# shoeffner/ann3depth

Hardware: AMD Instinct MI355X
Metric: images/sec (640x480->55x74 MSDN train step) (higher is better)
Workload: dtype f32

## Files before the change

ann3depth_amd/_lib.py:

```python
import ctypes
import os
from ctypes import c_char_p, c_float, c_int, c_int32, c_int64, c_size_t, c_uint8, c_uint32, c_void_p, POINTER

LIB_PATH = os.environ.get('A3D_LIB') or os.path.join(os.path.dirname(os.path.abspath(__file__)), 'liba3d.so')


class A3dError(RuntimeError):
    pass


class ConvDesc(ctypes.Structure):
    _fields_ = [(n, c_int32) for n in ('n', 'h', 'w', 'c', 'k', 'r', 's', 'stride', 'pad_t', 'pad_l', 'ho', 'wo',
                                       'ldx', 'ldy', 'precision', 'storage', 'hints')]


class SecondOutput(ctypes.Structure):
    _fields_ = [('ptr', c_void_p), ('ld', c_int32), ('step', c_int32), ('offset', c_int32), ('bf16', c_int32), ('cols', c_int32)]


class ExampleView(ctypes.Structure):
    _fields_ = [('image_height', c_int64), ('image_width', c_int64), ('image_channels', c_int64),
                ('depth_height', c_int64), ('depth_width', c_int64), ('depth_channels', c_int64),
                ('image', c_void_p), ('image_bytes', c_size_t), ('depth', c_void_p), ('depth_bytes', c_size_t)]


class TimingRecord(ctypes.Structure):
    _fields_ = [(n, c_int32) for n in ('mode', 'bm', 'bn', 'waves_m', 'nwaves', 'bk', 'avec', 'bvec', 'prec', 'lds_dma', 'splitk', 'm', 'n', 'k')] + \
               [('ms', c_float), ('flops', ctypes.c_double)]


_P = c_void_p
_D = POINTER(ConvDesc)

SIGNATURES = {
    'a3d_version': (c_char_p, []),
    'a3d_last_error': (c_int, [c_char_p, c_size_t]),
    'a3d_conv2d_fwd_ws_bytes': (c_size_t, [_D]),
    'a3d_conv2d_fwd': (c_int, [_D, _P, _P, _P, _P, c_int, _P, c_size_t, _P]),
    'a3d_conv2d_bwd_data_ws_bytes': (c_size_t, [_D]),
    'a3d_conv2d_bwd_data': (c_int, [_D, _P, _P, _P, _P, _P, c_size_t, _P]),
    'a3d_conv2d_bwd_filter_ws_bytes': (c_size_t, [_D]),
    'a3d_conv2d_bwd_filter': (c_int, [_D, _P, _P, _P, _P, _P, c_size_t, _P]),
    'a3d_conv2d_fwd_prepared_filter_bytes': (c_size_t, [_D]),
    'a3d_conv2d_fwd_prepare_filter': (c_int, [_D, _P, _P, c_size_t, _P]),
    'a3d_conv2d_bwd_filter_pooled_ws_bytes': (c_size_t, [_D]),
    'a3d_conv2d_bwd_filter_pooled': (c_int, [_D, _P, _P, c_int, _P, _P, c_int, c_int, _P, _P, _P, c_size_t, _P]),
    'a3d_conv2d_bwd_both_supported': (c_int, [_D]),
    'a3d_conv2d_bwd_both_ws_bytes': (c_size_t, [_D]),
    'a3d_conv2d_bwd_both': (c_int, [_D, _P, _P, _P, _P, _P, _P, c_int, c_int, c_int, _P, _P, c_size_t, _P]),
    'a3d_dense_fwd_ws_bytes': (c_size_t, [c_int, c_int, c_int]),
    'a3d_dense_fwd': (c_int, [c_int, c_int, c_int, _P, _P, _P, _P, c_int, _P, _P, c_size_t, _P]),
    'a3d_dense_bwd_data_ws_bytes': (c_size_t, [c_int, c_int, c_int]),
    'a3d_dense_bwd_data': (c_int, [c_int, c_int, c_int, _P, _P, _P, _P, c_int, c_float, _P, c_size_t, _P]),
    'a3d_dense_bwd_filter_ws_bytes': (c_size_t, [c_int, c_int, c_int]),
    'a3d_dense_bwd_filter': (c_int, [c_int, c_int, c_int, _P, _P, _P, _P, _P, c_size_t, _P]),
    'a3d_maxpool2x2_fwd': (c_int, [c_int, c_int, c_int, c_int, _P, _P, c_int, _P, _P]),
    'a3d_maxpool2x2_bwd': (c_int, [c_int, c_int, c_int, c_int, _P, _P, c_int, _P, c_int, _P]),
    'a3d_resize_bilinear_tf1': (c_int, [c_int, c_int, c_int, c_int, _P, c_int, c_int, _P, _P]),
    'a3d_resize_bilinear_tf1_pair': (c_int, [c_int, c_int, c_int, c_int, _P, c_int, c_int, _P, c_int, _P, c_int, c_int, _P, _P]),
    'a3d_resize_bilinear_tf1_ex': (c_int, [c_int, c_int, c_int, c_int, _P, c_int, c_int, c_int, _P, c_int, _P, c_int, c_int, c_int,
                                           _P, _P]),
    'a3d_warp_bilinear_pair': (c_int, [c_int, c_int, c_int, c_int, _P, c_int, c_int, c_int, _P, c_int, _P, c_int, c_int, c_int,
                                       _P, _P, _P]),
    'a3d_extract_patches': (c_int, [c_int, c_int, c_int, c_int, _P, c_int, c_int, _P, _P]),
    'a3d_silog_loss_fwd': (c_int, [c_int, c_int, _P, _P, _P, _P, _P]),
    'a3d_silog_loss_bwd': (c_int, [c_int, c_int, _P, _P, _P, _P, _P]),
    'a3d_dropout_keep_mask': (c_int, [c_size_t, ctypes.c_uint64, ctypes.c_uint64, c_float, _P, _P]),
    'a3d_adam_apply_tf1': (c_int, [c_size_t, _P, _P, _P, _P, c_float, c_float, c_float, c_float, c_float, c_float,
                                   c_float, _P]),
    'a3d_adam_apply_tf1_flag': (c_int, [c_size_t, _P, _P, _P, _P, c_float, c_float, c_float, c_float, c_float, c_float,
                                        c_float, _P, _P]),
    'a3d_dense_fwd_ex': (c_int, [c_int, c_int, c_int, _P, _P, _P, _P, c_int, _P, c_int, c_int, _P, c_size_t, _P]),
    'a3d_dense_bwd_data_ex': (c_int, [c_int, c_int, c_int, _P, _P, _P, _P, c_int, c_float, c_int, c_int, _P, c_size_t, _P]),
    'a3d_dense_fwd_ex2': (c_int, [c_int, c_int, c_int, _P, _P, _P, _P, c_int, c_int, c_int, _P, c_int, c_int, POINTER(SecondOutput), _P,
                                  c_size_t, _P]),
    'a3d_dense_bwd_data_ex2': (c_int, [c_int, c_int, c_int, _P, _P, _P, _P, c_int, c_float, c_int, c_int, POINTER(SecondOutput), _P,
                                       c_size_t, _P]),
    'a3d_conv2d_fwd_ex2': (c_int, [_D, _P, _P, _P, _P, c_int, POINTER(SecondOutput), _P, c_size_t, _P]),
    'a3d_silog_loss_bwd_ex': (c_int, [c_int, c_int, _P, _P, _P, _P, _P, c_int, _P]),
    'a3d_depth_metrics_ws_bytes': (c_size_t, [c_int, c_int, c_int]),
    'a3d_depth_metrics': (c_int, [c_int, c_int, c_int, _P, c_int, c_int, _P, c_int, c_float, c_float, c_float, c_float, _P, _P,
                                  c_size_t, _P]),
    'a3d_cast_bf16': (c_int, [c_size_t, _P, _P, c_int, _P]),
    'a3d_cast_rows': (c_int, [c_size_t, c_int, _P, c_int, c_int, _P, c_int, c_int, _P]),
    'a3d_pad_channels_bf16': (c_int, [c_size_t, c_int, _P, c_int, _P, _P]),
    'a3d_stream_create': (c_int, [c_int, ctypes.POINTER(ctypes.c_void_p)]),
    'a3d_stream_destroy': (c_int, [_P]),
    'a3d_maxpool2x2_fwd_bf16': (c_int, [c_int, c_int, c_int, c_int, _P, c_int, _P, c_int, _P, _P]),
    'a3d_maxpool2x2_bwd_bf16': (c_int, [c_int, c_int, c_int, c_int, _P, c_int, _P, c_int, _P, c_int, _P]),
    'a3d_copy_channel_bf16': (c_int, [c_size_t, _P, c_int, c_int, _P, c_int, c_int, _P]),
    'a3d_maxpool2x2_bwd_idx_bf16': (c_int, [c_int, c_int, c_int, c_int, _P, _P, c_int, _P, c_int, _P, c_int, _P]),
    'a3d_maxpool2x2_bwd_idx_bf16s': (c_int, [c_int, c_int, c_int, c_int, _P, _P, c_int, _P, c_int, _P, c_int, _P]),
    'a3d_dense_bwd_filter_adam_tf1': (c_int, [c_int, c_int, c_int, _P, _P, _P, _P, _P, _P, _P, _P, c_float, c_float, c_float,
                                              c_float, c_float, c_float, _P]),
    'a3d_dense_bwd_filter_adam_tf1_ex': (c_int, [c_int, c_int, c_int, _P, _P, _P, _P, _P, _P, _P, _P, c_float, c_float, c_float,
                                                 c_float, c_float, c_float, c_int, _P]),
    'a3d_superpixel_mean': (c_int, [c_int, c_int, c_int, c_int, _P, c_int, _P, _P]),
    'a3d_superpixel_hist': (c_int, [c_int, c_int, c_int, _P, c_int, _P, _P]),
    'a3d_pair_similarity': (c_int, [c_int, c_int, c_int, _P, c_int, _P, _P, _P, c_int, _P, _P, c_float, _P, _P, _P]),
    'a3d_crf_loss': (c_int, [c_int, c_int, _P, _P, _P, _P, _P, c_int, c_float, _P, _P, _P, _P]),
    'a3d_crf_map': (c_int, [c_int, c_int, _P, _P, _P, _P, c_int, _P, _P, _P]),
    'a3d_sgd_apply': (c_int, [c_size_t, _P, _P, c_float, _P]),
    'a3d_conv2d_pool_fwd': (c_int, [_D, _P, _P, _P, _P, c_int, _P, c_int, _P, c_size_t, _P]),
    'a3d_maxpool2x2_bwd_idx': (c_int, [c_int, c_int, c_int, c_int, _P, _P, c_int, _P, c_int, _P, c_int, _P]),
    'a3d_copy_channel': (c_int, [c_size_t, _P, c_int, c_int, _P, c_int, c_int, _P]),
    'a3d_comm_standin': (c_int, [_P, c_size_t, _P, c_size_t, c_int, c_float, _P]),
    'a3d_timing_enable': (c_int, [c_int]),
    'a3d_timing_collect': (c_int, [POINTER(TimingRecord), c_int]),
    'a3d_timing_select': (c_int, [POINTER(TimingRecord)]),
    'a3d_crc32c': (c_uint32, [_P, c_size_t]),
    'a3d_masked_crc32c': (c_uint32, [_P, c_size_t]),
    'a3d_tfrecord_next': (c_int, [_P, c_size_t, c_int, POINTER(c_size_t), POINTER(c_size_t), POINTER(c_size_t)]),
    'a3d_example_parse': (c_int, [_P, c_size_t, POINTER(ExampleView)]),
    'a3d_decode_raw_plus_half': (c_int, [_P, c_size_t, _P]),
    'a3d_record_decode': (c_int, [_P, c_size_t, c_int, _P, c_size_t, _P, c_size_t, POINTER(ExampleView)]),
    'a3d_record_decode_u8': (c_int, [_P, c_size_t, c_int, _P, _P, c_size_t, _P, _P, c_size_t, POINTER(ExampleView),
                                     POINTER(c_int)]),
    'a3d_records_decode': (c_int, [POINTER(c_void_p), POINTER(c_size_t), c_int, c_int, POINTER(c_int64), _P, _P, _P, _P,
                                   POINTER(c_int32), c_int, POINTER(c_int32)]),
    'a3d_h2d_gather': (c_int, [_P, _P, POINTER(c_int32), c_int, c_int, c_size_t, _P]),
    'a3d_sizeof_conv_desc': (c_size_t, []),
    'a3d_example_write': (c_int64, [_P, c_int, c_int, c_int, _P, c_int, c_int, c_int, _P, c_size_t]),
}

EXT_SIGNATURES = {
    'a3dx_resize_bilinear_tf1_valid': (c_int, [c_int, c_int, c_int, c_int, _P, c_int, c_int, c_int, _P, c_int, _P, c_int, c_int,
                                               c_int, _P, c_float, c_float, _P]),
    'a3dx_warp_bilinear_pair_valid': (c_int, [c_int, c_int, c_int, c_int, _P, c_int, c_int, c_int, _P, c_int, _P, c_int, c_int,
                                              c_int, _P, _P, c_float, c_float, _P]),
    'a3dx_silog_masked_loss_fwd': (c_int, [c_int, c_int, _P, _P, _P, _P, _P]),
    'a3dx_silog_masked_loss_bwd_ex': (c_int, [c_int, c_int, _P, _P, _P, _P, _P, c_int, _P]),
}

PAIR_SIGNATURES = {
    'a3dp_crf_loss_grad': (c_int, [c_int, c_int, _P, _P, _P, _P, _P, c_int, c_float, _P, _P, _P, _P, _P]),
    'a3dp_pair_dense_bwd': (c_int, [c_int, c_int, c_int, _P, _P, _P, _P, _P]),
    'a3dp_sgd_apply_floor': (c_int, [c_size_t, _P, _P, c_float, c_float, _P]),
}

TEXTURE_SIGNATURES = {
    'a3dt_superpixel_lbp_hist': (c_int, [c_int, c_int, c_int, _P, c_int, _P, _P]),
    'a3dt_pair_similarity3': (c_int, [c_int, c_int, c_int, _P, c_int, _P, _P, _P, _P, c_int, _P, _P, c_float, _P, _P, _P]),
}

GRADLOSS_SIGNATURES = {
    'a3dg_silog_grad_loss_fwd': (c_int, [c_int, c_int, c_int, _P, _P, c_int, c_float, _P, _P, _P]),
    'a3dg_silog_grad_loss_bwd_ex': (c_int, [c_int, c_int, c_int, _P, _P, c_int, c_float, _P, _P, _P, c_int, _P]),
}

CRF_VALID_SIGNATURES = {
    'a3dv_superpixel_mean_valid': (c_int, [c_int, c_int, c_int, _P, c_int, c_int, _P, _P, _P]),
    'a3dv_crf_loss_observed': (c_int, [c_int, c_int, _P, _P, _P, _P, _P, c_int, _P, _P, _P, _P, _P, _P, _P]),
}

FCSP_SIGNATURES = {
    'a3df_superpixel_pool_fwd': (c_int, [c_int, c_int, c_int, c_int, _P, c_int, c_int, c_int, c_int, _P, _P, _P, c_int, _P]),
    'a3df_superpixel_pool_bwd': (c_int, [c_int, c_int, c_int, c_int, _P, c_int, c_int, c_int, c_int, _P, _P, _P, c_int, _P]),
}

CRF_BAND_SIGNATURES = {
    'a3db_crf_band_nll': (c_int, [c_int, c_int, c_int, _P, _P, _P, _P, _P, c_int, _P, _P, _P, _P, _P, _P, _P]),
    'a3db_crf_band_map': (c_int, [c_int, c_int, c_int, _P, _P, _P, _P, c_int, _P, _P, _P]),
}

WINO_SIGNATURES = {
    'a3dw_conv2d_bwd_data_prepared_filter_bytes': (c_size_t, [_D]),
    'a3dw_conv2d_bwd_data_prepare_filter': (c_int, [_D, _P, _P, c_size_t, _P]),
}

WINO_GRAD_SIGNATURES = {
    'a3dwg_conv2d_bwd_filter_ws_bytes': (c_size_t, [_D]),
    'a3dwg_conv2d_bwd_filter': (c_int, [_D, _P, _P, _P, _P, _P, c_size_t, _P]),
}

UPSAMPLE_SIGNATURES = {
    'a3du_joint_bilateral_upsample': (c_int, [c_int, c_int, c_int, _P, c_int, c_int, _P, c_int, _P, _P, _P, _P, c_int, c_float,
                                              c_float, _P, _P]),
}

POSTERIOR_SIGNATURES = {
    'a3dc_crf_band_posterior': (c_int, [c_int, c_int, c_int, _P, _P, _P, _P, _P, c_int, _P, _P, _P, _P, _P]),
}

SLIC_SIGNATURES = {
    'a3ds_label_mean': (c_int, [c_int, c_int, c_int, c_int, _P, c_int, _P, _P, _P, _P]),
    'a3ds_label_hist': (c_int, [c_int, c_int, c_int, _P, c_int, _P, _P, _P]),
    'a3ds_slic_update': (c_int, [c_int, c_int, c_int, _P, c_int, _P, _P, _P, _P]),
    'a3ds_slic_assign': (c_int, [c_int, c_int, c_int, _P, c_int, _P, c_float, _P, _P]),
    'a3ds_slic_segment': (c_int, [c_int, c_int, c_int, _P, c_int, c_int, c_float, _P, _P, _P, _P]),
    'a3ds_pair_similarity': (c_int, [c_int, c_int, _P, _P, _P, _P, _P, c_int, _P, _P, c_float, _P, _P, _P]),
    'a3ds_label_pool_fwd': (c_int, [c_int, c_int, c_int, c_int, _P, c_int, c_int, c_int, c_int, _P, _P, _P, _P, _P, c_int, _P]),
    'a3ds_label_pool_bwd': (c_int, [c_int, c_int, c_int, c_int, _P, c_int, c_int, c_int, c_int, _P, _P, _P, _P, _P, c_int, _P]),
}

_lib = None


def load():
    global _lib
    if _lib is not None:
        return _lib
    if not os.path.exists(LIB_PATH):
        raise A3dError(f'{LIB_PATH} not found: build it with `python -c "import __graft_entry__ as g; g.build()"` '
                       f'or `make -C ann3depth_amd/csrc` (there is no fallback path)')
    import torch
    lib = ctypes.CDLL(LIB_PATH)
    for name, (res, args) in (list(SIGNATURES.items()) + list(EXT_SIGNATURES.items()) + list(PAIR_SIGNATURES.items())
                              + list(TEXTURE_SIGNATURES.items()) + list(GRADLOSS_SIGNATURES.items())
                              + list(CRF_VALID_SIGNATURES.items()) + list(FCSP_SIGNATURES.items())
                              + list(CRF_BAND_SIGNATURES.items()) + list(WINO_SIGNATURES.items())
                              + list(UPSAMPLE_SIGNATURES.items()) + list(POSTERIOR_SIGNATURES.items())
                              + list(WINO_GRAD_SIGNATURES.items()) + list(SLIC_SIGNATURES.items())):
        try:
            fn = getattr(lib, name)
        except AttributeError as e:
            raise A3dError(f'liba3d.so lacks symbol {name}: stale build?') from e
        fn.restype = res
        fn.argtypes = args
    if lib.a3d_sizeof_conv_desc() != ctypes.sizeof(ConvDesc):
        raise A3dError(f'liba3d.so reads a {lib.a3d_sizeof_conv_desc()}-byte a3d_conv_desc, this binding passes '
                       f'{ctypes.sizeof(ConvDesc)} bytes: stale build?')
    _lib = lib
    return lib


def last_error():
    buf = ctypes.create_string_buffer(512)
    load().a3d_last_error(buf, 512)
    return buf.value.decode(errors='replace')


def check(rc, what):
    if rc != 0:
        raise A3dError(f'{what} failed ({rc}): {last_error()}')
```

ann3depth_amd/csrc/a3d_internal.h:

```cpp
#pragma once
#include <hip/hip_runtime.h>
#include <stddef.h>
#include <stdint.h>

#include <algorithm>

#include "../../include/a3d.h"
#include "igemm_plan.h"

namespace a3d {

int set_error(int code, const char* fmt, ...);

#define A3D_CHECK_ARG(cond, ...)                                 \
  do {                                                           \
    if (!(cond)) return ::a3d::set_error(A3D_EINVAL, __VA_ARGS__); \
  } while (0)

inline void clear_stale_error() { (void)hipGetLastError(); }

inline int check_launch(const char* what) {
  hipError_t e = hipGetLastError();
  if (e != hipSuccess) return set_error(A3D_ELAUNCH, "%s: %s", what, hipGetErrorString(e));
  return A3D_OK;
}

inline unsigned grid_for(size_t total, int per_block = 256, unsigned cap = 8192) {
  size_t g = (total + per_block - 1) / per_block;
  return (unsigned)std::min<size_t>(std::max<size_t>(g, 1), cap);
}

inline bool aligned16(const void* p) { return (reinterpret_cast<uintptr_t>(p) & 15) == 0; }

struct IgemmParams;
int launch_igemm(int mode, const GemmPlan& plan, int avec, int bvec, IgemmParams& p, void* ws, hipStream_t st);
int take_second_output(IgemmParams& p, const a3d_second_output* o);

struct TimingSlot {
  hipEvent_t start, stop;
  a3d_timing_record rec;
};
bool timing_wanted(const a3d_timing_record& r);
int timing_begin(TimingSlot& slot, hipStream_t st);
void timing_end(TimingSlot& slot, hipStream_t st);
a3d_timing_record timing_record(int mode, int prec, int bm, int bn, int waves_m, int nwaves, int bk, int avec, int bvec, int lds_dma,
                                int m, int n, int k);
template <typename Launch>
int timed_launch(const a3d_timing_record& rec, hipStream_t st, Launch&& launch) {
  if (!timing_wanted(rec)) return launch();
  TimingSlot slot{};
  slot.rec = rec;
  int rc = timing_begin(slot, st);
  if (rc != A3D_OK) return rc;
  rc = launch();
  timing_end(slot, st);
  return rc;
}

bool dense_dw_applicable(int m, int k, int n);
bool dense_stream_applicable(int m, int k, int n);
size_t dense_stream_ws_bytes(int m, int k, int n);
int dense_fwd_stream(int m, int k, int n, const float* x, const float* w, const float* bias, float* y, int act,
                     const uint8_t* keep, float keep_scale, void* ws, size_t ws_bytes, hipStream_t st);
struct ReduceParams;
int launch_splitk_reduce(const ReduceParams& r, hipStream_t st);
int dense_dw_launch(int m, int k, int n, const float* x, const float* dz, float* dw, float* db, hipStream_t st);

size_t colsum_bf16_ws_bytes(int n);
bool colsum_bf16_ok(int n);
int colsum_bf16(const void* dz, int rows, int n, int ld, float* out, void* ws, int* nparts, hipStream_t st);

bool stencil1_applicable(const a3d_conv_desc* d);
size_t stencil1_bwdf_ws_bytes(const a3d_conv_desc* d);
int stencil1_fwd(const a3d_conv_desc* d, const float* x, const float* w, const float* bias, float* y, int act,
                 hipStream_t st);
int stencil1_bwd_filter(const a3d_conv_desc* d, const float* x, const float* dz, float* dw, float* db, void* ws,
                        hipStream_t st);
bool stencil1_bwd_both_applicable(const a3d_conv_desc* d);
size_t stencil1_bwd_both_ws_bytes(const a3d_conv_desc* d);
int stencil1_bwd_both(const a3d_conv_desc* d, const float* x, const float* dz, const float* w, float* dw, float* db,
                      void* dx, int lddx, int dx_bf16, int relu_mask, unsigned* state, void* ws, hipStream_t st);

bool fewch_bwdf_applicable(const a3d_conv_desc* d, bool pooled);
size_t fewch_bwdf_ws_bytes(const a3d_conv_desc* d, bool pooled);
bool fewch_extents_ok(const a3d_conv_desc* d, bool pooled, int ldz, int esz, int ld_arg);
int fewch_bwd_filter(const a3d_conv_desc* d, const float* x, int src, const void* dz, int ldz, const void* pooled_act,
                     const uint8_t* argmax, int ld_arg, float* dw, float* db, void* ws, hipStream_t st);

int fewch_reduce_launch(const float* slabs, int splits, int Mp, int NP, int M, int N, float* dw, float* db, hipStream_t st);
bool fewch16_bwdf_applicable(const a3d_conv_desc* d, bool pooled);
size_t fewch16_bwdf_ws_bytes(const a3d_conv_desc* d, bool pooled);
int fewch16_bwd_filter(const a3d_conv_desc* d, const float* x, bool pooled, const void* dz, int ldz, const void* pooled_act,
                       const uint8_t* argmax, int ld_arg, float* dw, float* db, void* ws, hipStream_t st);

bool conv3_applicable(const a3d_conv_desc* d, unsigned x_off);
size_t conv3_ws_bytes(const a3d_conv_desc* d);
int conv3_pack(const a3d_conv_desc* d, const float* w, float* wp, hipStream_t st);
int conv3_fwd(const a3d_conv_desc* d, const float* x, const float* w, const float* bias, float* y, int act, int pool,
              int ld_out, uint8_t* argmax, void* ws, size_t ws_bytes, hipStream_t st, bool prepared = false);

bool conv3b_applicable(const a3d_conv_desc* d);
size_t conv3b_filter_bytes(const a3d_conv_desc* d);
int conv3b_pack(const a3d_conv_desc* d, const float* w, void* wp, hipStream_t st);
int conv3b_fwd(const a3d_conv_desc* d, const void* x, const float* w, const float* bias, void* y, int act, int pool, int ld_out,
               uint8_t* argmax, void* ws, size_t ws_bytes, hipStream_t st, bool prepared);

struct WinoGeom {
  int oh, ow, th, tw;
  size_t T;
  int K, N, Kp, Np;
  size_t v_bytes, m_bytes, u_bytes;
};
WinoGeom wino_geom(const a3d_conv_desc* d, bool bwd);
bool wino_applicable(const a3d_conv_desc* d);
int wino_filter(const a3d_conv_desc* d, bool bwd, const float* w, float* U, hipStream_t st);
int wino_input(const a3d_conv_desc* d, bool bwd, const float* src, float* V, hipStream_t st);
int wino_output(const a3d_conv_desc* d, bool bwd, const float* M, float* out, const float* bias, const float* mask, int act,
                hipStream_t st);
a3d_timing_record wino_record(int mode, const WinoGeom& g);
int wino_gemm(IgemmParams& p, const WinoGeom& g, hipStream_t st);

struct WinoGradGeom {
  size_t T;
  int Cp, Kp;
  int splits;
  size_t v_bytes, z_bytes;
  size_t slab_bytes, bias_bytes;
};
int wino_grad_splits(int C, int K, size_t T);
WinoGradGeom wino_grad_geom(const a3d_conv_desc* d);
bool wino_grad_applicable(const a3d_conv_desc* d);
int wino_dz(const a3d_conv_desc* d, const float* dz, float* Z, hipStream_t st);
int wino_dw(const a3d_conv_desc* d, const WinoGradGeom& g, const float* slabs, const float* bparts, float* dw, float* db, hipStream_t st);
a3d_timing_record wino_grad_record(const a3d_conv_desc* d, const WinoGradGeom& g);
int wino_grad_gemm(IgemmParams& p, const WinoGradGeom& g, hipStream_t st);

}
```

ann3depth_amd/csrc/igemm_host.hip:

```cpp
#include <algorithm>

#include "../../include/a3d_wino.h"
#include "../../include/a3d_wino_grad.h"
#include "a3d_internal.h"
#include "igemm.h"
#include "igemm_cfgs.h"

namespace a3d {

int launch_igemm_multi_bwd_d(int avec, int bvec, IgemmMulti& ps, unsigned grid_x, unsigned count, hipStream_t st);
int launch_igemm_bf16_multi_bwd_d(int bn, IgemmMulti& ps, unsigned grid_x, unsigned count, hipStream_t st);


struct RunForm {
  int vec;
  int rl, rlp;
  int kp;
  int np;
  size_t bytes;
};
static bool run_form_ok(const a3d_conv_desc* d, unsigned x_off, RunForm* rf, bool bwd_filter = false) {
  if (d->pad_t || d->pad_l || d->ldx != d->c || d->c % 4 == 0 || d->c > 4) return false;
  const int step = d->stride * d->c, row = d->w * d->c;
  int vec = 0;
  bool anywhere = false;
  if (step % 4 == 0 && row % 4 == 0 && x_off == 0) vec = 4;
  else if (step % 2 == 0 && row % 2 == 0 && (x_off & 7) == 0) vec = 2;
  else if (bwd_filter && d->precision == A3D_PREC_F32 && !d->storage && (x_off & 3) == 0) {
    vec = 2;
    anywhere = true;
  }
  if (vec == 4 && d->precision == A3D_PREC_F32) {
    const int rl = d->s * d->c;
    const int kp4 = d->r * ((rl + 3) / 4 * 4), kp2 = d->r * ((rl + 1) / 2 * 2);
    if ((kp2 + 127) / 128 < (kp4 + 127) / 128) vec = 2;
  }
  if (!vec) return false;
  rf->vec = vec;
  rf->rl = d->s * d->c;
  rf->rlp = (rf->rl + vec - 1) / vec * vec;
  rf->kp = d->r * rf->rlp;
  rf->np = (d->k + 3) / 4 * 4;
  rf->bytes = ((size_t)rf->kp * rf->np * 4 + 255) / 256 * 256;
  if (anywhere) return (d->wo - 1) * step + rf->rl <= row && (d->ho - 1) * d->stride + d->r <= d->h;
  return (d->wo - 1) * step + rf->rlp <= row;
}

__global__ __launch_bounds__(256) void pad_filter_kernel(const float* w, float* wp, int r, int rl, int rlp, int n, int np) {
  const int total = r * rlp * np;
  for (int i = blockIdx.x * 256 + threadIdx.x; i < total; i += gridDim.x * 256) {
    const int col = i % np, row = i / np;
    const int q = row % rlp, rr = row / rlp;
    wp[i] = (q < rl && col < n) ? w[(size_t)(rr * rl + q) * n + col] : 0.f;
  }
}
__global__ __launch_bounds__(256) void unpad_filter_kernel(const float* wp, float* w, int r, int rl, int rlp, int n) {
  const int total = r * rl * n;
  for (int i = blockIdx.x * 256 + threadIdx.x; i < total; i += gridDim.x * 256) {
    const int col = i % n, row = i / n;
    const int q = row % rl, rr = row / rl;
    w[i] = wp[(size_t)(rr * rlp + q) * n + col];
  }
}

struct Operands {
  bool known = false;
  unsigned x = 0, w = 0, y = 0;
  unsigned aux = 0;
  int act = A3D_ACT_NONE, pool = 0, ld_out = 0;
  bool argmax = false, prepared = false;
  bool db = true;
};
static const Operands kOnGrid{};
static Operands launch_operands(const void* x, const void* w, const void* y, const void* aux) {
  auto off16 = [](const void* p) { return (unsigned)(reinterpret_cast<uintptr_t>(p) & 15); };
  Operands o;
  o.known = true;
  o.x = off16(x); o.w = off16(w); o.y = off16(y); o.aux = off16(aux);
  return o;
}

enum GemmForm { kAsStored, kLdsDma, kRunForm, kBf16Image };
struct Route {
  bool ok = false;
  RunForm rf{};
  GemmProblem g{};
  GemmPlan plan{};
  size_t repack = 0;
  size_t bytes = 0;
};
static size_t upto(size_t need, const Route& r) { return r.ok ? std::max(need, r.bytes) : need; }
static void fit_workspace(Route& r, const Operands& o, size_t ws_bytes, size_t per_split = 0) {
  if (r.bytes <= ws_bytes || !(o.x | o.w | o.y | o.aux) || r.repack > ws_bytes) return;
  r.plan = plan_within(r.g, r.plan, ws_bytes - r.repack, per_split);
  r.bytes = r.repack + r.plan.ws_bytes + (r.plan.splitk > 1 ? (size_t)r.plan.splitk * per_split : 0);
}
#define A3D_CHECK_WS(ws, who) A3D_CHECK_ARG(aligned16(ws), who ": ws must be 16-byte aligned")

static const int kAll16 = A3D_STORE_X_BF16 | A3D_STORE_W_BF16 | A3D_STORE_Y_BF16;
static bool stored16(const a3d_conv_desc* d, int bits) { return (d->storage & bits) == bits; }
static bool ring_ok(const a3d_conv_desc* d, const Operands& o, int both, unsigned out_off, int taps) {
  if (d->precision != A3D_PREC_BF16 || !stored16(d, both) || d->c % 8 || d->k % 8) return false;
  return !o.known || (d->ldx % 8 == 0 && d->ldy % 8 == 0 && taps <= 128 && !out_off);
}

static int ilog2_exact(int v) {
  for (int l = 0; l < 8; ++l)
    if ((1 << l) == v) return l;
  return -1;
}

static int check_desc(const a3d_conv_desc* d) {
  A3D_CHECK_ARG(d != nullptr, "conv: null descriptor");
  A3D_CHECK_ARG(d->n > 0 && d->h > 0 && d->w > 0 && d->c > 0 && d->k > 0 && d->r > 0 && d->s > 0, "conv: bad dims");
  A3D_CHECK_ARG(ilog2_exact(d->stride) >= 0 && d->stride <= 4, "conv: stride %d unsupported (1, 2 or 4)", d->stride);
  A3D_CHECK_ARG(d->pad_t >= 0 && d->pad_l >= 0 && d->pad_t < d->r && d->pad_l < d->s, "conv: bad padding");
  A3D_CHECK_ARG(d->ho > 0 && d->wo > 0, "conv: bad output size");
  A3D_CHECK_ARG((d->ho - 1) * d->stride - d->pad_t < d->h && (d->wo - 1) * d->stride - d->pad_l < d->w,
                "conv: output size inconsistent with input");
  A3D_CHECK_ARG(d->ldx >= d->c && d->ldy >= d->k, "conv: pixel strides smaller than channel counts");
  A3D_CHECK_ARG(d->precision >= A3D_PREC_F32 && d->precision <= A3D_PREC_F32_WINOGRAD, "conv: unknown precision %d", d->precision);
  const double lim = 2147483647.0;
  A3D_CHECK_ARG((double)d->n * d->h * d->w * d->ldx < lim && (double)d->n * d->ho * d->wo * d->ldy < lim &&
                    (double)d->r * d->s * d->c * d->k < lim,
                "conv: tensor too large for 31-bit indexing");
  return A3D_OK;
}

#define A3D_AS_F32(d)                                          \
  a3d_conv_desc d##_f32;                                       \
  if ((d) && (d)->precision == A3D_PREC_F32_WINOGRAD) {        \
    d##_f32 = *(d);                                            \
    d##_f32.precision = A3D_PREC_F32;                          \
    (d) = &d##_f32;                                            \
  }

static GemmProblem fwd_problem(const a3d_conv_desc* d) {
  GemmProblem g;
  g.mode = MODE_FWD;
  g.M = d->n * d->ho * d->wo; g.N = d->k; g.K = d->r * d->s * d->c;
  g.avec = (d->c % 4 == 0 && d->ldx % 4 == 0) ? 4 : 1;
  g.bvec = (d->k % 4 == 0) ? 4 : 1;
  return g;
}
static GemmProblem bwd_d_problem(const a3d_conv_desc* d) {
  GemmProblem g;
  g.mode = MODE_BWD_D;
  g.M = d->n * d->h * d->w; g.N = d->c; g.K = d->r * d->s * d->k;
  g.avec = (d->k % 4 == 0 && d->ldy % 4 == 0) ? 4 : 1;
  g.bvec = (d->k % 4 == 0) ? 4 : 1;
  return g;
}
static GemmProblem bwd_f_problem(const a3d_conv_desc* d) {
  GemmProblem g;
  g.mode = MODE_BWD_F;
  g.M = d->r * d->s * d->c; g.N = d->k; g.K = d->n * d->ho * d->wo;
  g.avec = (d->c % 4 == 0 && d->ldx % 4 == 0) ? 4 : 1;
  g.bvec = (d->k % 4 == 0 && d->ldy % 4 == 0) ? 4 : 1;
  return g;
}

static void storage_vecs(GemmProblem& g, bool a16, bool b16, bool c16) {
  if (c16) g.no_glds = 1;
  if (a16) g.avec = 4;
  if (b16) g.bvec = 4;
}
static int apply_storage(IgemmParams& p, int precision, bool a16, bool b16, bool c16, int a_c, int a_ld, int b_c, int b_ld,
                         const void* a, const void* b, const void* c, const char* an, const char* bn, const char* cn) {
  if (!a16 && !b16 && !c16) return A3D_OK;
  A3D_CHECK_ARG(precision == A3D_PREC_BF16 || (precision == A3D_PREC_F32 && !a16 && !b16),
                "bf16 operands need precision A3D_PREC_BF16");
  A3D_CHECK_ARG(!a16 || (a_c % 8 == 0 && a_ld % 8 == 0 && aligned16(a)), "bf16 %s: channels / stride must be multiples of 8, base 16-byte aligned", an);
  A3D_CHECK_ARG(!b16 || ((b_c < 0 || b_c % 8 == 0) && b_ld % 8 == 0 && aligned16(b)), "bf16 %s: channels / stride must be multiples of 8, base 16-byte aligned", bn);
  A3D_CHECK_ARG(!c16 || aligned16(c), "bf16 %s: base must be 16-byte aligned", cn);
  p.a16 = a16; p.b16 = b16; p.c16 = c16;
  return A3D_OK;
}

static void fill_common(IgemmParams& p, const GemmProblem& g) {
  p = IgemmParams{};
  p.M = g.M; p.N = g.N; p.K = g.K;
  p.mask_scale = 1.f;
  p.mask_act = EPI_RELU;
  p.sub_step = 1;
}

static void fill_staging(IgemmParams& p, int mode, unsigned long long a_elems, unsigned long long b_elems, int taps_r,
                         int taps_s) {
  p.a_elems = a_elems;
  p.b_elems = b_elems;
  p.ntaps = std::max(1, taps_r * taps_s);
  p.cpt = std::max(1, p.Cg / 32);
  p.uni = (mode != MODE_BWD_F) && p.Cg % 32 == 0 && p.K == p.ntaps * p.Cg;
  p.kperm = p.uni && p.ntaps > 1 && p.cpt > 1;
  p.div_cpt = make_fastdiv(p.cpt);
  p.div_taps = make_fastdiv(p.ntaps);
  p.cpt64 = std::max(1, p.Cg / 64);
  p.uni64 = p.uni && p.Cg % 64 == 0;
  p.kperm64 = p.uni64 && p.ntaps > 1 && p.cpt64 > 1;
  p.div_cpt64 = make_fastdiv(p.cpt64);
}

static void fill_gather(IgemmParams& p, const a3d_conv_desc* d, int ld, int S, int Cg) {
  p.H = d->h; p.W = d->w; p.ld = ld; p.pHW = d->h * d->w;
  p.stride = d->stride; p.lstride = ilog2_exact(d->stride); p.pad_t = d->pad_t; p.pad_l = d->pad_l;
  p.S = S; p.Cg = Cg;
  p.div_phw = make_fastdiv(d->ho * d->wo); p.div_pw = make_fastdiv(d->wo);
  p.div_c = make_fastdiv(Cg); p.div_s = make_fastdiv(S);
  p.div_c_half = make_fastdiv(std::max(1, Cg / 2));
}
static void fill_pool(IgemmParams& p, const a3d_conv_desc* d, uint8_t* argmax, int ld_out) {
  const int ph = d->ho / 2, pw = d->wo / 2;
  p.pool = 1;
  p.argmax = argmax;
  p.div_phw = make_fastdiv(ph * pw * 4); p.div_pw = make_fastdiv(pw);
  p.ldc = ld_out;
}

static int fwd_rows(const a3d_conv_desc* d, int pool) {
  return pool ? d->n * (d->ho / 2) * (d->wo / 2) * 4 : d->n * d->ho * d->wo;
}

static a3d_timing_record conv3_record(const a3d_conv_desc* d, int m) {
  return timing_record(MODE_FWD, A3D_PREC_F32, 64, d->k > 64 ? 96 : 64, 1, 1, 8, 4, 4, 2, m, d->k, d->r * d->s * d->c);
}
static a3d_timing_record conv3b_record(const a3d_conv_desc* d, int m) {
  return timing_record(MODE_FWD, A3D_PREC_BF16, 64, d->k > 64 ? 96 : 64, 1, 1, 16, 4, 4, 2, m, d->k, d->r * d->s * 3);
}
static a3d_timing_record fewch_record(const a3d_conv_desc* d) {
  return timing_record(MODE_BWD_F, A3D_PREC_F32, 128, (d->k + 31) / 32 * 32, 4, 4, 2, 1, 1, 4, d->r * d->s * d->c, d->k, d->n * d->ho * d->wo);
}
static a3d_timing_record fewch16_record(const a3d_conv_desc* d) {
  return timing_record(MODE_BWD_F, A3D_PREC_BF16, 128, (d->k + 31) / 32 * 32, 4, 4, 16, 1, 1, 4, d->r * d->s * d->c, d->k, d->n * d->ho * d->wo);
}

static bool bf16_image_form_ok(const a3d_conv_desc* d, const Operands& o, RunForm* rf) {
  rf->vec = 4;
  rf->rl = d->s * 4;
  rf->rlp = (d->s * 2 + 3) / 4 * 4 * 2;
  rf->kp = d->r * rf->rlp;
  rf->np = (d->k + 7) / 8 * 8;
  rf->bytes = ((size_t)rf->kp * rf->np * 2 + 255) / 256 * 256;
  if (!(d->storage & A3D_STORE_X_BF16) || d->c != 4 || d->ldx != 4) return false;
  if (!o.known) return true;
  if ((d->storage & A3D_STORE_W_BF16) || d->precision != A3D_PREC_BF16) return false;
  if (d->pad_t || d->pad_l || d->stride % 2 || (d->w * 2) % 4 || o.x) return false;
  return (d->wo - 1) * d->stride * 2 + rf->rlp / 2 <= d->w * 2;
}
__global__ __launch_bounds__(256) void pad_filter_bf16_kernel(const float* w, __bf16* wp, int r, int rl, int rlp, int n, int np) {
  const int total = r * rlp * np;
  for (int i = blockIdx.x * 256 + threadIdx.x; i < total; i += gridDim.x * 256) {
    const int col = i % np, row = i / np;
    const int q = row % rlp, rr = row / rlp;
    wp[i] = (__bf16)((q < rl && col < n) ? w[(size_t)(rr * rl + q) * n + col] : 0.f);
  }
}
static int pad_filter(const a3d_conv_desc* d, const RunForm& rf, bool bf16, const float* w, void* wp, hipStream_t st) {
  const dim3 grid((rf.kp * rf.np + 255) / 256), block(256);
  clear_stale_error();
  if (bf16)
    hipLaunchKernelGGL(pad_filter_bf16_kernel, grid, block, 0, st, w, static_cast<__bf16*>(wp), d->r, rf.rl, rf.rlp, d->k, rf.np);
  else
    hipLaunchKernelGGL(pad_filter_kernel, grid, block, 0, st, w, static_cast<float*>(wp), d->r, rf.rl, rf.rlp, d->k, rf.np);
  return check_launch(bf16 ? "pad_filter_bf16" : "pad_filter");
}

static bool fwd_form_ok(const a3d_conv_desc* d, const Operands& o, GemmForm form, RunForm* rf) {
  if (form == kRunForm) return run_form_ok(d, o.x, rf);
  if (form == kBf16Image) return bf16_image_form_ok(d, o, rf);
  if (form == kAsStored || !ring_ok(d, o, A3D_STORE_X_BF16 | A3D_STORE_W_BF16, o.y, d->r * d->s)) return form == kAsStored;
  return !o.known || (o.act != A3D_ACT_SIGMOID && (!o.pool || ((d->storage & A3D_STORE_Y_BF16) && o.ld_out % 8 == 0 &&
                                                               (!o.argmax || (d->k % 16 == 0 && !o.aux)))));
}
static Route fwd_gemm(const a3d_conv_desc* d, const Operands& o, GemmForm form) {
  Route r;
  if (!(r.ok = fwd_form_ok(d, o, form, &r.rf))) return r;
  GemmProblem& g = r.g;
  g = fwd_problem(d);
  g.M = fwd_rows(d, o.pool); g.plain = o.pool ? 1 : 0;
  if (o.x) g.avec = 1;
  if (o.w) g.bvec = 1;
  if (form == kRunForm || form == kBf16Image) {
    g.K = r.rf.kp; g.avec = r.rf.vec;
    if (!o.prepared) r.repack = r.rf.bytes;
  }
  if (form == kBf16Image) { g.bvec = 4; g.no_glds = 1; }
  if (form == kLdsDma) { g.ring_ok = 1; g.avec = g.bvec = 4; }
  if (o.known) {
    if (d->hints & A3D_HINT_SHARE_CU) g.no_glds = 1;
    if (form == kRunForm) g.bvec = 4;
    storage_vecs(g, d->storage & A3D_STORE_X_BF16, d->storage & A3D_STORE_W_BF16, d->storage & A3D_STORE_Y_BF16);
  }
  r.plan = plan_gemm(g, d->precision);
  r.bytes = r.repack + r.plan.ws_bytes;
  return r;
}

}

using namespace a3d;

extern "C" {

static size_t wino_bytes(const a3d_conv_desc* d, bool bwd, bool prepared) {
  const WinoGeom g = wino_geom(d, bwd);
  return (prepared ? 0 : g.u_bytes) + g.v_bytes + g.m_bytes;
}
static int wino_conv(const a3d_conv_desc* d, bool bwd, const float* src, const float* w, float* out, const float* bias, const float* mask,
                     int act, bool prepared, void* ws, size_t ws_bytes, hipStream_t st) {
  const WinoGeom g = wino_geom(d, bwd);
  const size_t need = wino_bytes(d, bwd, prepared);
  if (!ws || need > ws_bytes) return set_error(A3D_EWORKSPACE, "conv2d (Winograd): need %zu workspace bytes", need);
  A3D_CHECK_ARG(!prepared || aligned16(w), "conv2d (Winograd): the prepared filter must be 16-byte aligned");
  char* base = static_cast<char*>(ws);
  const float* U = w;
  int rc;
  if (!prepared) {
    rc = wino_filter(d, bwd, w, reinterpret_cast<float*>(base), st);
    if (rc != A3D_OK) return rc;
    U = reinterpret_cast<const float*>(base);
    base += g.u_bytes;
  }
  float* V = reinterpret_cast<float*>(base);
  float* M = reinterpret_cast<float*>(base + g.v_bytes);
  rc = wino_input(d, bwd, src, V, st);
  if (rc != A3D_OK) return rc;
  a3d_conv_desc e{};
  e.n = (int)g.T; e.h = e.w = e.ho = e.wo = 1; e.c = g.Kp; e.k = g.Np; e.r = e.s = 1; e.stride = 1; e.ldx = g.Kp; e.ldy = g.Np;
  GemmProblem gp = fwd_problem(&e);
  IgemmParams p;
  fill_common(p, gp);
  p.A = V; p.B = U; p.C = M;
  p.npix = gp.M; p.nrsc = gp.K;
  fill_gather(p, &e, g.Kp, 1, g.Kp);
  p.ldb = g.Np; p.ldc = g.Np;
  fill_staging(p, MODE_FWD, (unsigned long long)g.T * g.Kp, (unsigned long long)g.Kp * g.Np, 1, 1);
  rc = timed_launch(wino_record(bwd ? MODE_BWD_D : MODE_FWD, g), st, [&] { return wino_gemm(p, g, st); });
  if (rc != A3D_OK) return rc;
  return wino_output(d, bwd, M, out, bias, mask, act, st);
}

size_t a3d_conv2d_fwd_ws_bytes(const a3d_conv_desc* d) {
  if (check_desc(d) != A3D_OK) return 0;
  const size_t wino = wino_applicable(d) ? wino_bytes(d, false, (d->hints & A3D_HINT_W_PREPARED) != 0) : 0;
  A3D_AS_F32(d);
  if (stencil1_applicable(d)) return 0;
  if (wino) return std::max(wino, a3d_conv2d_fwd_ws_bytes(d));
  size_t need = 0;
  for (GemmForm form : {kAsStored, kLdsDma, kRunForm, kBf16Image}) need = upto(need, fwd_gemm(d, kOnGrid, form));
  RunForm rf;
  if (bf16_image_form_ok(d, kOnGrid, &rf)) need = std::max(need, conv3b_filter_bytes(d));
  if (conv3_applicable(d, kOnGrid.x)) need = std::max(need, conv3_ws_bytes(d));
  return need;
}

static int conv_fwd_impl(const a3d_conv_desc* d, const float* x, const float* w, const float* bias, float* y, int act,
                         int pool, int ld_out, uint8_t* argmax, void* ws, size_t ws_bytes, void* stream,
                         const a3d_second_output* out2 = nullptr) {
  int rc = check_desc(d);
  if (rc != A3D_OK) return rc;
  if (!ws) ws_bytes = 0;
  if (wino_applicable(d) && !pool && !(out2 && out2->ptr)) {
    A3D_CHECK_ARG(x && w && y, "conv2d_fwd: null tensor");
    A3D_CHECK_WS(ws, "conv2d_fwd");
    A3D_CHECK_ARG(act == A3D_ACT_NONE || act == A3D_ACT_RELU || act == A3D_ACT_SIGMOID, "conv2d_fwd: bad act");
    return wino_conv(d, false, x, w, y, bias, nullptr, act, (d->hints & A3D_HINT_W_PREPARED) != 0, ws, ws_bytes,
                     static_cast<hipStream_t>(stream));
  }
  A3D_CHECK_ARG(!(wino_applicable(d) && (d->hints & A3D_HINT_W_PREPARED)),
                "conv2d_fwd: A3D_HINT_W_PREPARED with A3D_PREC_F32_WINOGRAD is for the plain forward only (no fused pool, no second output)");
  A3D_AS_F32(d);
  Operands o = launch_operands(x, w, y, argmax);
  o.act = act; o.pool = pool; o.ld_out = ld_out; o.argmax = argmax != nullptr;
  o.prepared = (d->hints & A3D_HINT_W_PREPARED) != 0;
  RunForm rf;
  const bool image = fwd_form_ok(d, o, kBf16Image, &rf);
  A3D_CHECK_ARG(!(out2 && out2->ptr) || (!pool && !stencil1_applicable(d) && !image && !conv3_applicable(d, o.x)),
                "conv2d_fwd_ex2: a second output on the implicit-GEMM forwards only (no fused pool, no few-channel / one-filter kernels)");
  A3D_CHECK_ARG(x && w && y, "conv2d_fwd: null tensor");
  A3D_CHECK_WS(ws, "conv2d_fwd");
  A3D_CHECK_ARG(act == A3D_ACT_NONE || act == A3D_ACT_RELU || act == A3D_ACT_SIGMOID, "conv2d_fwd: bad act");
  if (pool) {
    A3D_CHECK_ARG(d->precision == A3D_PREC_F32 || image ||
                      (d->precision == A3D_PREC_BF16 && (stored16(d, kAll16) || d->storage == A3D_STORE_Y_BF16)),
                  "conv2d_pool_fwd: fp32, the bf16 image form (4-channel bf16 image, a3d_pad_channels_bf16), or bf16 arithmetic on "
                  "bf16 x, w and y (LDS-DMA kernel)");
    A3D_CHECK_ARG(d->ho >= 2 && d->wo >= 2 && ld_out >= d->k, "conv2d_pool_fwd: output smaller than one pool window");
    A3D_CHECK_ARG(!stencil1_applicable(d), "conv2d_pool_fwd: single-output-channel convs are not supported");
  } else if (stencil1_applicable(d)) {
    A3D_CHECK_ARG(!d->storage, "conv2d_fwd: single-output-channel convs take float32 tensors");
    return stencil1_fwd(d, x, w, bias, y, act, static_cast<hipStream_t>(stream));
  }
  hipStream_t st = static_cast<hipStream_t>(stream);
  if (image && conv3b_applicable(d))
    return timed_launch(conv3b_record(d, fwd_rows(d, pool)), st,
                        [&] { return conv3b_fwd(d, x, w, bias, y, act, pool, ld_out, argmax, ws, ws_bytes, st, o.prepared); });
  if (!image && conv3_applicable(d, o.x))
    return timed_launch(conv3_record(d, fwd_rows(d, pool)), st,
                        [&] { return conv3_fwd(d, x, w, bias, y, act, pool, ld_out, argmax, ws, ws_bytes, st, o.prepared); });
  const bool run = !image && fwd_form_ok(d, o, kRunForm, &rf) && (o.prepared || rf.bytes <= ws_bytes), padded = run || image;
  Route r = fwd_gemm(d, o, image ? kBf16Image : run ? kRunForm : fwd_form_ok(d, o, kLdsDma, &rf) ? kLdsDma : kAsStored);
  fit_workspace(r, o, ws_bytes);
  A3D_CHECK_ARG(!o.prepared || (padded && !o.w && !o.x),
                "conv2d_fwd: A3D_HINT_W_PREPARED on a launch that reads the filter as stored, or with x off the 16-byte grid");
  IgemmParams p;
  fill_common(p, r.g);
  const int sb = d->storage;
  if (image) {
    p.a16 = 1; p.b16 = 1; p.c16 = (sb & A3D_STORE_Y_BF16) ? 1 : 0;
  } else {
    A3D_CHECK_ARG(!sb || ((!pool || sb == A3D_STORE_Y_BF16 || (sb == kAll16 && d->precision == A3D_PREC_BF16)) &&
                          !(run && (sb & A3D_STORE_W_BF16))),
                  "conv2d_fwd: the fused pool takes float32 inputs (its output may be bf16) or bf16 x, w and y; 3-channel filters stay float32");
    rc = apply_storage(p, d->precision, sb & A3D_STORE_X_BF16, sb & A3D_STORE_W_BF16, sb & A3D_STORE_Y_BF16, d->c, d->ldx, d->k, d->k,
                       x, w, y, "x", "w", "y");
    if (rc != A3D_OK) return rc;
    A3D_CHECK_ARG(!(pool && (p.a16 || p.b16)) || r.plan.ring,
                  "conv2d_pool_fwd: on bf16 inputs the fused pool is the LDS-DMA kernel's (channels and strides in whole 16-byte pieces, k %% 16 == 0)");
  }
  if (r.bytes > ws_bytes) return set_error(A3D_EWORKSPACE, "conv2d_fwd: need %zu workspace bytes", r.bytes);
  A3D_CHECK_ARG(!image || (r.plan.prec == A3D_PREC_BF16 && !o.y), "conv2d_fwd: bf16 image form needs the bf16 kernel");
  A3D_CHECK_ARG(!(p.a16 || p.b16) || r.plan.prec == A3D_PREC_BF16, "conv2d_fwd: bf16 operands need vectorisable tensors");
  A3D_CHECK_ARG(!p.c16 || r.plan.prec == A3D_PREC_BF16 || !is_glds_cfg(r.plan.cfg), "conv2d_fwd: no bf16 output from the LDS-DMA kernels");
  const float* filter = w;
  if (padded && !o.prepared) {
    rc = pad_filter(d, r.rf, image, w, ws, st);
    if (rc != A3D_OK) return rc;
    filter = static_cast<const float*>(ws);
  }
  const int ldb = padded ? r.rf.np : d->k;
  p.A = x; p.B = filter; p.C = y; p.bias = bias; p.act = act;
  p.share = (d->hints & A3D_HINT_SHARE_CU) ? 1 : 0;
  p.npix = r.g.M; p.nrsc = r.g.K;
  fill_gather(p, d, d->ldx, padded ? 1 : d->s, padded ? r.rf.rlp : d->c);
  p.ldb = ldb; p.ldc = d->ldy;
  if (pool) fill_pool(p, d, argmax, ld_out);
  fill_staging(p, MODE_FWD, (unsigned long long)d->n * d->h * d->w * d->ldx, (unsigned long long)r.g.K * ldb, d->r, padded ? 1 : d->s);
  rc = take_second_output(p, out2);
  if (rc != A3D_OK) return rc;
  return launch_igemm(MODE_FWD, r.plan, r.g.avec, r.g.bvec, p, static_cast<char*>(ws) + r.repack, st);
}

int a3d_conv2d_fwd(const a3d_conv_desc* d, const float* x, const float* w, const float* bias, float* y, int act,
                   void* ws, size_t ws_bytes, void* stream) {
  return conv_fwd_impl(d, x, w, bias, y, act, 0, 0, nullptr, ws, ws_bytes, stream);
}

static int fwd_filter_form(const a3d_conv_desc* d, RunForm* rf) {
  if (check_desc(d) != A3D_OK || stencil1_applicable(d)) return 0;
  const Operands o = launch_operands(nullptr, nullptr, nullptr, nullptr);
  if (bf16_image_form_ok(d, o, rf)) return 1;
  if (conv3_applicable(d, o.x)) return 2;
  if (run_form_ok(d, o.x, rf)) return 3;
  return 0;
}

size_t a3d_conv2d_fwd_prepared_filter_bytes(const a3d_conv_desc* d) {
  if (check_desc(d) == A3D_OK && wino_applicable(d)) return wino_geom(d, false).u_bytes;
  A3D_AS_F32(d);
  RunForm rf{};
  switch (fwd_filter_form(d, &rf)) {
    case 1: return conv3b_applicable(d) ? conv3b_filter_bytes(d) : rf.bytes;
    case 2: return conv3_ws_bytes(d);
    case 3: return rf.bytes;
    default: return 0;
  }
}

int a3d_conv2d_fwd_prepare_filter(const a3d_conv_desc* d, const float* w, void* prepared, size_t prepared_bytes, void* stream) {
  int rc = check_desc(d);
  if (rc != A3D_OK) return rc;
  A3D_CHECK_ARG(w && prepared && aligned16(prepared), "conv2d_fwd_prepare_filter: null or misaligned buffer");
  const size_t need = a3d_conv2d_fwd_prepared_filter_bytes(d);
  A3D_CHECK_ARG(need > 0, "conv2d_fwd_prepare_filter: this forward reads the filter as stored");
  if (prepared_bytes < need) return set_error(A3D_EWORKSPACE, "conv2d_fwd_prepare_filter: need %zu bytes", need);
  hipStream_t st = static_cast<hipStream_t>(stream);
  if (wino_applicable(d)) return wino_filter(d, false, w, static_cast<float*>(prepared), st);
  A3D_AS_F32(d);
  RunForm rf{};
  switch (fwd_filter_form(d, &rf)) {
    case 1: return conv3b_applicable(d) ? conv3b_pack(d, w, prepared, st) : pad_filter(d, rf, true, w, prepared, st);
    case 2: return conv3_pack(d, w, static_cast<float*>(prepared), st);
    default: return pad_filter(d, rf, false, w, prepared, st);
  }
}

int a3d_conv2d_fwd_ex2(const a3d_conv_desc* d, const float* x, const float* w, const float* bias, float* y, int act,
                       const a3d_second_output* out2, void* ws, size_t ws_bytes, void* stream) {
  return conv_fwd_impl(d, x, w, bias, y, act, 0, 0, nullptr, ws, ws_bytes, stream, out2);
// ... 182 lines not shown
  r.plan = plan_gemm(g, d->precision);
  if (r.plan.ring) r.bytes = r.plan.ws_bytes + (o.db ? colsum_bf16_ws_bytes(d->k) : 0);
  else r.bytes = r.repack + r.plan.ws_bytes + (r.plan.splitk > 1 && o.db ? (size_t)r.plan.splitk * g.N * 4 : 0);
  return r;
}

int a3d_conv2d_bwd_both_supported(const a3d_conv_desc* d) {
  A3D_AS_F32(d);
  return check_desc(d) == A3D_OK && !d->storage && stencil1_bwd_both_applicable(d);
}

size_t a3d_conv2d_bwd_both_ws_bytes(const a3d_conv_desc* d) {
  return a3d_conv2d_bwd_both_supported(d) ? stencil1_bwd_both_ws_bytes(d) : 0;
}

int a3d_conv2d_bwd_both(const a3d_conv_desc* d, const float* x, const float* dz, const float* w, float* dw, float* db,
                        void* dx, int lddx, int dx_bf16, int relu_mask, uint32_t* state, void* ws, size_t ws_bytes,
                        void* stream) {
  A3D_AS_F32(d);
  int rc = check_desc(d);
  if (rc != A3D_OK) return rc;
  A3D_CHECK_ARG(x && dz && w && dw && dx && state, "conv2d_bwd_both: null tensor");
  A3D_CHECK_ARG(a3d_conv2d_bwd_both_supported(d),
                "conv2d_bwd_both: one output channel, 5x5, stride 1, an even channel count <= 64, float32 tensors, x below 1 GiB");
  A3D_CHECK_ARG(lddx >= d->c && lddx % 2 == 0, "conv2d_bwd_both: lddx must be even and >= c");
  A3D_CHECK_ARG((reinterpret_cast<uintptr_t>(x) & 7) == 0 && (reinterpret_cast<uintptr_t>(w) & 7) == 0 &&
                    (reinterpret_cast<uintptr_t>(dx) & (dx_bf16 ? 3 : 7)) == 0 && (reinterpret_cast<uintptr_t>(ws) & 3) == 0,
                "conv2d_bwd_both: x, w and dx must be aligned to a channel pair");
  if (stencil1_bwd_both_ws_bytes(d) > ws_bytes) return set_error(A3D_EWORKSPACE, "conv2d_bwd_both: workspace too small");
  return stencil1_bwd_both(d, x, dz, w, dw, db, dx, lddx, dx_bf16, relu_mask, state, ws, static_cast<hipStream_t>(stream));
}

static bool fewch_wanted(const a3d_conv_desc* d, bool pooled) {
  return !d->storage && fewch_bwdf_applicable(d, pooled) && tune_int("A3D_FEWCH", 1) != 0;
}

static int fewch_timed(const a3d_conv_desc* d, const float* x, int src, const void* dz, int ldz, const void* pooled_act,
                       const uint8_t* argmax, int ld_arg, float* dw, float* db, void* ws, hipStream_t st) {
  return timed_launch(fewch_record(d), st, [&] { return fewch_bwd_filter(d, x, src, dz, ldz, pooled_act, argmax, ld_arg, dw, db, ws, st); });
}

static bool fewch16_wanted(const a3d_conv_desc* d, bool pooled) {
  return !d->storage && fewch16_bwdf_applicable(d, pooled) && tune_int("A3D_FEWCH16", 1) != 0;
}

static bool fewch_pooled_ok(const a3d_conv_desc* d) { return !d->storage && fewch_bwdf_applicable(d, true); }

size_t a3d_conv2d_bwd_filter_pooled_ws_bytes(const a3d_conv_desc* d) {
  A3D_AS_F32(d);
  if (check_desc(d) != A3D_OK) return 0;
  if (fewch16_wanted(d, true)) return fewch16_bwdf_ws_bytes(d, true);
  return fewch_pooled_ok(d) ? fewch_bwdf_ws_bytes(d, true) : 0;
}

int a3d_conv2d_bwd_filter_pooled(const a3d_conv_desc* d, const float* x, const void* dpool, int ld_dpool, const void* pooled,
                                 const uint8_t* argmax, int ld_argmax, int pooled_bf16, float* dw, float* db, void* ws,
                                 size_t ws_bytes, void* stream) {
  A3D_AS_F32(d);
  int rc = check_desc(d);
  if (rc != A3D_OK) return rc;
  A3D_CHECK_ARG(x && dpool && argmax && dw, "conv2d_bwd_filter_pooled: null tensor");
  A3D_CHECK_WS(ws, "conv2d_bwd_filter_pooled");
  if (fewch16_wanted(d, true)) {
    A3D_CHECK_ARG(pooled_bf16 && ld_dpool >= d->k && ld_argmax >= d->k && ld_dpool % 4 == 0 &&
                      (reinterpret_cast<uintptr_t>(dpool) & 7) == 0 && (reinterpret_cast<uintptr_t>(pooled) & 7) == 0 &&
                      (reinterpret_cast<uintptr_t>(x) & 15) == 0,
                  "conv2d_bwd_filter_pooled: bf16 arithmetic takes bf16 pooled tensors in whole aligned 4-channel groups");
    A3D_CHECK_ARG(fewch_extents_ok(d, true, ld_dpool, 2, ld_argmax), "conv2d_bwd_filter_pooled: pooled tensors of 2 GiB or more");
    if (fewch16_bwdf_ws_bytes(d, true) > ws_bytes) return set_error(A3D_EWORKSPACE, "conv2d_bwd_filter_pooled: workspace too small");
    hipStream_t st = static_cast<hipStream_t>(stream);
    return timed_launch(fewch16_record(d), st,
                        [&] { return fewch16_bwd_filter(d, x, true, dpool, ld_dpool, pooled, argmax, ld_argmax, dw, db, ws, st); });
  }
  A3D_CHECK_ARG(fewch_pooled_ok(d),
                "conv2d_bwd_filter_pooled: an unpadded conv of <= 4 densely packed float32 input channels and 33..96 filters (fp32 "
                "arithmetic; or bf16 arithmetic with bf16 pooled tensors)");
  A3D_CHECK_ARG(ld_dpool >= d->k && ld_argmax >= d->k, "conv2d_bwd_filter_pooled: pixel strides below the filter count");
  A3D_CHECK_ARG(ld_dpool % 4 == 0 && aligned16(x) && (reinterpret_cast<uintptr_t>(dpool) & (pooled_bf16 ? 7 : 15)) == 0 &&
                    (reinterpret_cast<uintptr_t>(pooled) & (pooled_bf16 ? 7 : 15)) == 0,
                "conv2d_bwd_filter_pooled: x, dpool and pooled in whole aligned 4-channel groups (ld_dpool % 4 == 0)");
  A3D_CHECK_ARG(fewch_extents_ok(d, true, ld_dpool, pooled_bf16 ? 2 : 4, ld_argmax), "conv2d_bwd_filter_pooled: pooled tensors of 2 GiB or more");
  if (fewch_bwdf_ws_bytes(d, true) > ws_bytes) return set_error(A3D_EWORKSPACE, "conv2d_bwd_filter_pooled: workspace too small");
  return fewch_timed(d, x, pooled_bf16 ? 2 : 1, dpool, ld_dpool, pooled, argmax, ld_argmax, dw, db, ws,
                     static_cast<hipStream_t>(stream));
}

size_t a3d_conv2d_bwd_filter_ws_bytes(const a3d_conv_desc* d) {
  A3D_AS_F32(d);
  if (check_desc(d) != A3D_OK) return 0;
  if (stencil1_applicable(d)) return stencil1_bwdf_ws_bytes(d);
  size_t need = fewch_wanted(d, false) ? fewch_bwdf_ws_bytes(d, false) : 0;
  for (GemmForm form : {kAsStored, kLdsDma, kRunForm}) need = upto(need, bwd_f_gemm(d, kOnGrid, form));
  return need;
}

int a3d_conv2d_bwd_filter(const a3d_conv_desc* d, const float* x, const float* dz, float* dw, float* db, void* ws,
                          size_t ws_bytes, void* stream) {
  A3D_AS_F32(d);
  int rc = check_desc(d);
  if (rc != A3D_OK) return rc;
  A3D_CHECK_ARG(x && dz && dw, "conv2d_bwd_filter: null tensor");
  A3D_CHECK_WS(ws, "conv2d_bwd_filter");
  if (!ws) ws_bytes = 0;
  if (stencil1_applicable(d)) {
    A3D_CHECK_ARG(!d->storage, "conv2d_bwd_filter: single-output-channel convs take float32 tensors");
    if (stencil1_bwdf_ws_bytes(d) > ws_bytes) return set_error(A3D_EWORKSPACE, "conv2d_bwd_filter: workspace too small");
    return stencil1_bwd_filter(d, x, dz, dw, db, ws, static_cast<hipStream_t>(stream));
  }
  if (fewch_wanted(d, false) && aligned16(x) && fewch_extents_ok(d, false, d->ldy, 4, 0)) {
    if (fewch_bwdf_ws_bytes(d, false) > ws_bytes) return set_error(A3D_EWORKSPACE, "conv2d_bwd_filter: workspace too small");
    return fewch_timed(d, x, 0, dz, d->ldy, nullptr, nullptr, 0, dw, db, ws, static_cast<hipStream_t>(stream));
  }
  Operands o = launch_operands(x, dw, dz, nullptr);
  o.db = db != nullptr;
  RunForm rf;
  const bool run = run_form_ok(d, o.x, &rf, true) && rf.bytes <= ws_bytes;
  Route r = bwd_f_gemm(d, o, run ? kRunForm : bwd_f_ring_ok(d, o) ? kLdsDma : kAsStored);
  fit_workspace(r, o, ws_bytes, o.db ? (size_t)r.g.N * 4 : 0);
  const GemmPlan& plan = r.plan;
  float* out = run ? static_cast<float*>(ws) : dw;
  IgemmParams p;
  fill_common(p, r.g);
  rc = apply_storage(p, d->precision, d->storage & A3D_STORE_X_BF16, d->storage & A3D_STORE_Y_BF16, false, d->c, d->ldx, -1, d->ldy,
                     x, dz, dw, "x", "dz", "dw");
  if (rc != A3D_OK) return rc;
  A3D_CHECK_ARG(!d->storage || plan.prec == A3D_PREC_BF16, "conv2d_bwd_filter: bf16 storage needs vectorisable operands");
  if (r.bytes > ws_bytes) return set_error(A3D_EWORKSPACE, "conv2d_bwd_filter: need %zu workspace bytes", r.bytes);
  hipStream_t st = static_cast<hipStream_t>(stream);
  if (plan.ring && db) {
    float* parts = reinterpret_cast<float*>(static_cast<char*>(ws) + plan.ws_bytes);
    int nparts = 0;
    rc = colsum_bf16(dz, r.g.K, d->k, d->ldy, plan.splitk > 1 ? nullptr : db, parts, &nparts, st);
    if (rc != A3D_OK) return rc;
    if (plan.splitk > 1) { p.dbias_parts = parts; p.dbias_parts_out = db; p.dbias_parts_n = nparts; }
    db = nullptr;
  }
  p.A = x; p.B = dz; p.C = out; p.dbias = db;
  p.npix = r.g.K; p.nrsc = r.g.M;
  fill_gather(p, d, d->ldx, run ? 1 : d->s, run ? rf.rlp : d->c);
  p.ldb = d->ldy; p.ldc = d->k;
  fill_staging(p, MODE_BWD_F, (unsigned long long)d->n * d->h * d->w * d->ldx, (unsigned long long)d->n * d->ho * d->wo * d->ldy, d->r,
               run ? 1 : d->s);
  if (run) { p.unpad_dst = dw; p.unpad_rl = rf.rl; p.unpad_rlp = rf.rlp; }
  rc = launch_igemm(MODE_BWD_F, plan, r.g.avec, r.g.bvec, p, static_cast<char*>(ws) + r.repack, st);
  if (rc != A3D_OK || !run || p.unpad_done) return rc;
  clear_stale_error();
  hipLaunchKernelGGL(unpad_filter_kernel, dim3((d->r * rf.rl * d->k + 255) / 256), dim3(256), 0, st, out, dw, d->r,
                     rf.rl, rf.rlp, d->k);
  return check_launch("unpad_filter");
}

static bool wino_grad_takes(const a3d_conv_desc* d) { return check_desc(d) == A3D_OK && wino_grad_applicable(d); }

size_t a3dwg_conv2d_bwd_filter_ws_bytes(const a3d_conv_desc* d) {
  if (!wino_grad_takes(d)) return a3d_conv2d_bwd_filter_ws_bytes(d);
  const WinoGradGeom g = wino_grad_geom(d);
  return g.v_bytes + g.z_bytes + g.slab_bytes + g.bias_bytes;
}

int a3dwg_conv2d_bwd_filter(const a3d_conv_desc* d, const float* x, const float* dz, float* dw, float* db, void* ws,
                            size_t ws_bytes, void* stream) {
  if (!wino_grad_takes(d)) return a3d_conv2d_bwd_filter(d, x, dz, dw, db, ws, ws_bytes, stream);
  A3D_CHECK_ARG(x && dz && dw, "conv2d_bwd_filter (Winograd): null tensor");
  A3D_CHECK_WS(ws, "conv2d_bwd_filter (Winograd)");
  const WinoGradGeom g = wino_grad_geom(d);
  const size_t need = g.v_bytes + g.z_bytes + g.slab_bytes + g.bias_bytes;
  if (!ws || need > ws_bytes) return set_error(A3D_EWORKSPACE, "conv2d_bwd_filter (Winograd): need %zu workspace bytes", need);
  hipStream_t st = static_cast<hipStream_t>(stream);
  char* base = static_cast<char*>(ws);
  float* V = reinterpret_cast<float*>(base);
  float* Z = reinterpret_cast<float*>(base + g.v_bytes);
  float* slabs = reinterpret_cast<float*>(base + g.v_bytes + g.z_bytes);
  float* bparts = reinterpret_cast<float*>(base + g.v_bytes + g.z_bytes + g.slab_bytes);
  int rc = wino_input(d, false, x, V, st);
  if (rc != A3D_OK) return rc;
  rc = wino_dz(d, dz, Z, st);
  if (rc != A3D_OK) return rc;
  a3d_conv_desc e{};
  e.n = (int)g.T; e.h = e.w = e.ho = e.wo = 1; e.c = g.Cp; e.k = g.Kp; e.r = e.s = 1; e.stride = 1; e.ldx = g.Cp; e.ldy = g.Kp;
  GemmProblem gp = bwd_f_problem(&e);
  IgemmParams p;
  fill_common(p, gp);
  p.A = V; p.B = Z; p.C = slabs; p.dbias = db ? bparts : nullptr;
  p.npix = gp.K; p.nrsc = gp.M;
  fill_gather(p, &e, g.Cp, 1, g.Cp);
  p.ldb = g.Kp; p.ldc = g.Kp;
  fill_staging(p, MODE_BWD_F, (unsigned long long)g.T * g.Cp, (unsigned long long)g.T * g.Kp, 1, 1);
  rc = timed_launch(wino_grad_record(d, g), st, [&] { return wino_grad_gemm(p, g, st); });
  if (rc != A3D_OK) return rc;
  return wino_dw(d, g, slabs, bparts, dw, db, st);
}

static a3d_conv_desc dense_desc(int m, int k, int n) {
  a3d_conv_desc d{};
  d.n = m; d.h = 1; d.w = 1; d.c = k; d.k = n; d.r = 1; d.s = 1; d.stride = 1; d.ho = 1; d.wo = 1;
  d.ldx = k; d.ldy = n;
  return d;
}

size_t a3d_dense_fwd_ws_bytes(int m, int k, int n) {
  a3d_conv_desc d = dense_desc(m, k, n);
  if (check_desc(&d) != A3D_OK) return 0;
  return std::max(plan_gemm(fwd_problem(&d), A3D_PREC_F32).ws_bytes, dense_stream_ws_bytes(m, k, n));
}

int a3d_dense_fwd(int m, int k, int n, const float* x, const float* w, const float* bias, float* y, int act,
                  const uint8_t* drop_keep, void* ws, size_t ws_bytes, void* stream) {
  return a3d_dense_fwd_ex(m, k, n, x, w, bias, y, act, drop_keep, A3D_PREC_F32, 0, ws, ws_bytes, stream);
}

int a3d_dense_fwd_ex(int m, int k, int n, const float* x, const float* w, const float* bias, float* y, int act,
                     const uint8_t* drop_keep, int precision, int storage, void* ws, size_t ws_bytes, void* stream) {
  return a3d_dense_fwd_ex2(m, k, n, x, w, bias, y, n, n, act, drop_keep, precision, storage, nullptr, ws, ws_bytes, stream);
}

int a3d_dense_fwd_ex2(int m, int k, int n, const float* x, const float* w, const float* bias, float* y, int ldy, int ncols_y, int act,
                      const uint8_t* drop_keep, int precision, int storage, const a3d_second_output* out2, void* ws,
                      size_t ws_bytes, void* stream) {
  A3D_CHECK_ARG(m > 0 && k > 0 && n > 0, "dense_fwd: bad dims");
  A3D_CHECK_ARG(ncols_y > 0 && ncols_y <= n && ldy >= ncols_y, "dense_fwd: y rows of %d columns at pitch %d from a GEMM of %d", ncols_y, ldy, n);
  A3D_CHECK_ARG((storage & ~(A3D_STORE_W_BF16 | A3D_STORE_X_BF16)) == 0, "dense_fwd: the weights and x may be bf16, y is float32");
  if (precision == A3D_PREC_F32_WINOGRAD) precision = A3D_PREC_F32;
  a3d_conv_desc d = dense_desc(m, k, n);
  d.precision = precision;
  int rc = check_desc(&d);
  if (rc != A3D_OK) return rc;
  A3D_CHECK_ARG(x && w && y, "dense_fwd: null tensor");
  A3D_CHECK_WS(ws, "dense_fwd");
  if (precision == A3D_PREC_F32 && !storage && dense_stream_applicable(m, k, n) && aligned16(x) && !out2 && ldy == n && ncols_y == n &&
      !tune_int("A3D_NO_DENSE_KERNELS", 0))
    return dense_fwd_stream(m, k, n, x, w, bias, y, act, drop_keep, 2.f, ws, ws_bytes, static_cast<hipStream_t>(stream));
  GemmProblem g = fwd_problem(&d);
  if (!aligned16(x)) g.avec = 1;
  if (!aligned16(w)) g.bvec = 1;
  IgemmParams p;
  fill_common(p, g);
  rc = apply_storage(p, precision, storage & A3D_STORE_X_BF16, storage & A3D_STORE_W_BF16, false, k, k, n, n, x, w, y, "x", "w", "y");
  if (rc != A3D_OK) return rc;
  A3D_CHECK_ARG(!p.a16 || aligned16(y), "dense_fwd: beside a bf16 x, y must be 16-byte aligned (the LDS-DMA kernel alone reads a bf16 x)");
  storage_vecs(g, p.a16, p.b16, p.c16);
  g.ring_ok = p.a16 && p.b16 && precision == A3D_PREC_BF16 && k % 8 == 0 && n % 8 == 0 && aligned16(y) && act != A3D_ACT_SIGMOID;
  g.need_reduce = ncols_y != n;
  GemmPlan plan = plan_gemm(g, precision);
  if (!aligned16(x) || !aligned16(w) || !aligned16(y)) plan = plan_within(g, plan, ws ? ws_bytes : 0, 0);
  A3D_CHECK_ARG(!storage || plan.prec == A3D_PREC_BF16, "dense_fwd: bf16 weights need vectorisable operands");
  A3D_CHECK_ARG(!p.a16 || plan.ring, "dense_fwd: a bf16 x is taken by the LDS-DMA kernel only (bf16 weights, k and n multiples of 8)");
  if (plan.ws_bytes > ws_bytes) return set_error(A3D_EWORKSPACE, "dense_fwd: need %zu workspace bytes", plan.ws_bytes);
  p.A = x; p.B = w; p.C = y; p.bias = bias; p.act = act; p.keep = drop_keep; p.mask_scale = 2.f;
  p.npix = m; p.nrsc = k;
  fill_gather(p, &d, k, 1, k);
  p.ldb = n; p.ldc = ldy; p.c_cols = ncols_y == n ? 0 : ncols_y;
  rc = take_second_output(p, out2);
  if (rc != A3D_OK) return rc;
  fill_staging(p, MODE_FWD, (unsigned long long)m * k, (unsigned long long)k * n, 1, 1);
  return launch_igemm(MODE_FWD, plan, g.avec, g.bvec, p, ws, static_cast<hipStream_t>(stream));
}

size_t a3d_dense_bwd_data_ws_bytes(int m, int k, int n) {
  a3d_conv_desc d = dense_desc(m, k, n);
  return a3d_conv2d_bwd_data_ws_bytes(&d);
}

int a3d_dense_bwd_data(int m, int k, int n, const float* dz, const float* w, float* dx, const float* mask,
                       int mask_act, float scale, void* ws, size_t ws_bytes, void* stream) {
  return a3d_dense_bwd_data_ex(m, k, n, dz, w, dx, mask, mask_act, scale, A3D_PREC_F32, 0, ws, ws_bytes, stream);
}

int a3d_dense_bwd_data_ex(int m, int k, int n, const float* dz, const float* w, float* dx, const float* mask, int mask_act,
                          float scale, int precision, int storage, void* ws, size_t ws_bytes, void* stream) {
  return a3d_dense_bwd_data_ex2(m, k, n, dz, w, dx, mask, mask_act, scale, precision, storage, nullptr, ws, ws_bytes, stream);
}

int a3d_dense_bwd_data_ex2(int m, int k, int n, const float* dz, const float* w, float* dx, const float* mask, int mask_act,
                           float scale, int precision, int storage, const a3d_second_output* out2, void* ws, size_t ws_bytes,
                           void* stream) {
  A3D_CHECK_ARG(m > 0 && k > 0 && n > 0, "dense_bwd_data: bad dims");
  if (precision == A3D_PREC_F32_WINOGRAD) precision = A3D_PREC_F32;
  A3D_CHECK_ARG(precision >= A3D_PREC_F32 && precision <= A3D_PREC_BF16, "dense_bwd_data: unknown precision %d", precision);
  A3D_CHECK_ARG(!mask || mask_act == A3D_ACT_RELU || mask_act == A3D_ACT_SIGMOID, "dense_bwd_data: bad mask_act");
  a3d_conv_desc d = dense_desc(m, k, n);
  int rc = check_desc(&d);
  if (rc != A3D_OK) return rc;
  A3D_CHECK_ARG(dz && w && dx, "dense_bwd_data: null tensor");
  A3D_CHECK_WS(ws, "dense_bwd_data");
  GemmProblem g = bwd_d_problem(&d);
  if (!aligned16(dz)) g.avec = 1;
  if (!aligned16(w)) g.bvec = 1;
  IgemmParams p;
  fill_common(p, g);
  rc = apply_storage(p, precision, storage & A3D_STORE_Y_BF16, storage & A3D_STORE_W_BF16, storage & A3D_STORE_X_BF16, n, n, n, n, dz, w,
                     dx, "dz", "w", "dx");
  if (rc != A3D_OK) return rc;
  A3D_CHECK_ARG(!p.c16 || aligned16(mask), "dense_bwd_data: bf16 mask must be 16-byte aligned");
  storage_vecs(g, p.a16, p.b16, p.c16);
  g.ring_ok = p.a16 && p.b16 && precision == A3D_PREC_BF16 && k % 8 == 0 && n % 8 == 0 && aligned16(dx) &&
              (!mask || (aligned16(mask) && mask_act == A3D_ACT_RELU));
  GemmPlan plan = plan_gemm(g, precision);
  if (!aligned16(dz) || !aligned16(w) || !aligned16(dx) || !aligned16(mask)) plan = plan_within(g, plan, ws ? ws_bytes : 0, 0);
  A3D_CHECK_ARG(!storage || plan.prec == A3D_PREC_BF16, "dense_bwd_data: bf16 weights need vectorisable operands");
  A3D_CHECK_ARG(!(p.a16 || p.c16) || plan.ring, "dense_bwd_data: bf16 dz / dx are taken by the LDS-DMA kernel only (bf16 weights, k and n multiples of 8, ReLU mask)");
  if (plan.ws_bytes > ws_bytes) return set_error(A3D_EWORKSPACE, "dense_bwd_data: need %zu workspace bytes", plan.ws_bytes);
  p.A = dz; p.B = w; p.C = dx; p.mask = mask; p.mask_scale = scale; p.mask_act = mask_act;
  p.npix = m; p.nrsc = n;
  fill_gather(p, &d, n, 1, n);
  p.Cn = k;
  p.ldc = k;
  p.S_full = 1;
  rc = take_second_output(p, out2);
  if (rc != A3D_OK) return rc;
  fill_staging(p, MODE_BWD_D, (unsigned long long)m * n, (unsigned long long)k * n, 1, 1);
  return launch_igemm(MODE_BWD_D, plan, g.avec, g.bvec, p, ws, static_cast<hipStream_t>(stream));
}

size_t a3d_dense_bwd_filter_ws_bytes(int m, int k, int n) {
  a3d_conv_desc d = dense_desc(m, k, n);
  return a3d_conv2d_bwd_filter_ws_bytes(&d);
}

int a3d_dense_bwd_filter(int m, int k, int n, const float* x, const float* dz, float* dw, float* db, void* ws,
                         size_t ws_bytes, void* stream) {
  A3D_CHECK_ARG(m > 0 && k > 0 && n > 0, "dense_bwd_filter: bad dims");
  A3D_CHECK_WS(ws, "dense_bwd_filter");
  if (dense_dw_applicable(m, k, n) && (long)k * n >= (1L << 16) && !tune_int("A3D_NO_DENSE_KERNELS", 0)) {
    A3D_CHECK_ARG(x && dz && dw, "dense_bwd_filter: null tensor");
    return dense_dw_launch(m, k, n, x, dz, dw, db, static_cast<hipStream_t>(stream));
  }
  a3d_conv_desc d = dense_desc(m, k, n);
  return a3d_conv2d_bwd_filter(&d, x, dz, dw, db, ws, ws_bytes, stream);
}

}
```

ann3depth_amd/csrc/wino.hip:

```cpp
#include "a3d_internal.h"
#include "igemm.h"
#include "igemm_cfgs.h"

namespace a3d {

typedef float f4 __attribute__((ext_vector_type(4)));

__global__ __launch_bounds__(256) void wino_filter_kernel(const float* w, float* U, int c, int k, int Rp, int Cp, int bwd) {
  const int total = Rp * Cp;
  for (int i = blockIdx.x * 256 + threadIdx.x; i < total; i += gridDim.x * 256) {
    const int col = i % Cp, row = i / Cp;
    const int rows = bwd ? k : c, cols = bwd ? c : k;
    float g[3][3];
#pragma unroll
    for (int r = 0; r < 3; ++r)
#pragma unroll
      for (int s = 0; s < 3; ++s) {
        float v = 0.f;
        if (row < rows && col < cols)
          v = bwd ? w[((size_t)((2 - r) * 3 + (2 - s)) * c + col) * k + row] : w[((size_t)(r * 3 + s) * c + row) * k + col];
        g[r][s] = v;
      }
    float t[4][3];
#pragma unroll
    for (int s = 0; s < 3; ++s) {
      const float a = g[0][s] + g[2][s];
      t[0][s] = g[0][s];
      t[1][s] = (a + g[1][s]) * 0.5f;
      t[2][s] = (a - g[1][s]) * 0.5f;
      t[3][s] = g[2][s];
    }
#pragma unroll
    for (int a4 = 0; a4 < 4; ++a4) {
      const float a = t[a4][0] + t[a4][2];
      const float u[4] = {t[a4][0], (a + t[a4][1]) * 0.5f, (a - t[a4][1]) * 0.5f, t[a4][2]};
#pragma unroll
      for (int b4 = 0; b4 < 4; ++b4) U[(size_t)(a4 * 4 + b4) * total + i] = u[b4];
    }
  }
}

template <bool VEC>
__global__ __launch_bounds__(256) void wino_input_kernel(const float* __restrict__ x, float* __restrict__ V, int h, int w, int c, int ld,
                                                         int th, int tw, int pad_t, int pad_l, int Cp, size_t T) {
  const int cqn = Cp / 4;
  const size_t total = T * (size_t)cqn;
  for (size_t i = (size_t)blockIdx.x * 256 + threadIdx.x; i < total; i += (size_t)gridDim.x * 256) {
    const int cq = (int)(i % cqn);
    const size_t t = i / cqn;
    const int tj = (int)(t % tw), ti = (int)((t / tw) % th);
    const size_t img = t / ((size_t)tw * th);
    const int y0 = 2 * ti - pad_t, x0 = 2 * tj - pad_l;
    f4 d[4][4];
#pragma unroll
    for (int a = 0; a < 4; ++a)
#pragma unroll
      for (int b = 0; b < 4; ++b) {
        f4 v = f4(0.f);
        const int yy = y0 + a, xx = x0 + b;
        if (yy >= 0 && yy < h && xx >= 0 && xx < w) {
          const float* src = x + ((img * h + yy) * w + xx) * (size_t)ld + cq * 4;
          if (VEC) {
            v = *reinterpret_cast<const f4*>(src);
          } else {
#pragma unroll
            for (int e = 0; e < 4; ++e)
              if (cq * 4 + e < c) v[e] = src[e];
          }
        }
        d[a][b] = v;
      }
    f4 r[4][4];
#pragma unroll
    for (int b = 0; b < 4; ++b) {
      r[0][b] = d[0][b] - d[2][b];
      r[1][b] = d[1][b] + d[2][b];
      r[2][b] = d[2][b] - d[1][b];
      r[3][b] = d[1][b] - d[3][b];
    }
#pragma unroll
    for (int a = 0; a < 4; ++a) {
      const f4 v[4] = {r[a][0] - r[a][2], r[a][1] + r[a][2], r[a][2] - r[a][1], r[a][1] - r[a][3]};
#pragma unroll
      for (int b = 0; b < 4; ++b) *reinterpret_cast<f4*>(V + ((size_t)(a * 4 + b) * T + t) * Cp + cq * 4) = v[b];
    }
  }
}

template <bool VEC>
__global__ __launch_bounds__(256) void wino_output_kernel(const float* __restrict__ M, float* __restrict__ out, const float* __restrict__ bias,
                                                          const float* __restrict__ mask, int act, int oh, int ow, int ncols, int ld,
                                                          int th, int tw, int Np, size_t T) {
  const int cqn = Np / 4;
  const size_t total = T * (size_t)cqn;
  for (size_t i = (size_t)blockIdx.x * 256 + threadIdx.x; i < total; i += (size_t)gridDim.x * 256) {
    const int cq = (int)(i % cqn);
    const size_t t = i / cqn;
    const int tj = (int)(t % tw), ti = (int)((t / tw) % th);
    const size_t img = t / ((size_t)tw * th);
    f4 m[4][4];
#pragma unroll
    for (int a = 0; a < 4; ++a)
#pragma unroll
      for (int b = 0; b < 4; ++b) m[a][b] = *reinterpret_cast<const f4*>(M + ((size_t)(a * 4 + b) * T + t) * Np + cq * 4);
    f4 r[2][4];
#pragma unroll
    for (int b = 0; b < 4; ++b) {
      r[0][b] = (m[0][b] + m[1][b]) + m[2][b];
      r[1][b] = (m[1][b] - m[2][b]) - m[3][b];
    }
    f4 bv = f4(0.f);
    if (bias) {
#pragma unroll
      for (int e = 0; e < 4; ++e)
        if (cq * 4 + e < ncols) bv[e] = bias[cq * 4 + e];
    }
#pragma unroll
    for (int a = 0; a < 2; ++a) {
      const f4 y2[2] = {(r[a][0] + r[a][1]) + r[a][2], (r[a][1] - r[a][2]) - r[a][3]};
#pragma unroll
      for (int b = 0; b < 2; ++b) {
        const int oy = 2 * ti + a, ox = 2 * tj + b;
        if (oy >= oh || ox >= ow) continue;
        const size_t o = ((img * oh + oy) * ow + ox) * (size_t)ld + cq * 4;
        f4 v = y2[b] + bv;
        if (act == EPI_RELU) {
#pragma unroll
          for (int e = 0; e < 4; ++e) v[e] = fmaxf(v[e], 0.f);
        } else if (act == EPI_SIGMOID) {
#pragma unroll
          for (int e = 0; e < 4; ++e) v[e] = 1.f / (1.f + expf(-v[e]));
        }
        if (VEC) {
          if (mask) {
            const f4 y = *reinterpret_cast<const f4*>(mask + o);
#pragma unroll
            for (int e = 0; e < 4; ++e) v[e] = apply_act_grad(v[e], y[e], EPI_RELU, 1.f);
          }
          *reinterpret_cast<f4*>(out + o) = v;
        } else {
#pragma unroll
          for (int e = 0; e < 4; ++e)
            if (cq * 4 + e < ncols) out[o + e] = mask ? apply_act_grad(v[e], mask[o + e], EPI_RELU, 1.f) : v[e];
        }
      }
    }
  }
}

constexpr int kBM = 128, kBN = 128, kWavesM = 4, kNWaves = 8, kBK = 32;
__global__ __launch_bounds__(64 * kNWaves, 2 * kNWaves / 4) void wino_gemm_kernel(const IgemmParams p, const size_t batch_a,
                                                                                   const size_t batch_b, const size_t batch_c) {
  IgemmParams q = p;
  q.A = p.A + (size_t)blockIdx.y * batch_a;
  q.B = p.B + (size_t)blockIdx.y * batch_b;
  q.C = p.C + (size_t)blockIdx.y * batch_c;
  igemm_body<MODE_FWD, kBM, kBN, kWavesM, kNWaves, kBK, 4, 4>(q, gridDim.x, blockIdx.x);
}

WinoGeom wino_geom(const a3d_conv_desc* d, bool bwd) {
  WinoGeom g{};
  g.oh = bwd ? d->h : d->ho;
  g.ow = bwd ? d->w : d->wo;
  g.th = (g.oh + 1) / 2;
  g.tw = (g.ow + 1) / 2;
  g.T = (size_t)d->n * g.th * g.tw;
  g.K = bwd ? d->k : d->c;
  g.N = bwd ? d->c : d->k;
  g.Kp = (g.K + 3) / 4 * 4;
  g.Np = (g.N + 3) / 4 * 4;
  auto up = [](size_t b) { return (b + 255) / 256 * 256; };
  g.v_bytes = up((size_t)16 * g.T * g.Kp * 4);
  g.m_bytes = up((size_t)16 * g.T * g.Np * 4);
  g.u_bytes = up((size_t)16 * g.Kp * g.Np * 4);
  return g;
}

bool wino_applicable(const a3d_conv_desc* d) {
  if (d->precision != A3D_PREC_F32_WINOGRAD || d->storage || d->r != 3 || d->s != 3 || d->stride != 1 || d->pad_t > 1 || d->pad_l > 1)
    return false;
  for (bool bwd : {false, true}) {
    const WinoGeom g = wino_geom(d, bwd);
    if ((double)g.T * std::max(g.Kp, g.Np) * 4.0 >= 2147483647.0 || g.T >= ((size_t)1 << 30)) return false;
  }
  return true;
}

int wino_filter(const a3d_conv_desc* d, bool bwd, const float* w, float* U, hipStream_t st) {
  const WinoGeom g = wino_geom(d, bwd);
  clear_stale_error();
  hipLaunchKernelGGL(wino_filter_kernel, dim3(grid_for((size_t)g.Kp * g.Np)), dim3(256), 0, st, w, U, d->c, d->k, g.Kp, g.Np, bwd ? 1 : 0);
  return check_launch("wino_filter");
}

int wino_input(const a3d_conv_desc* d, bool bwd, const float* src, float* V, hipStream_t st) {
  const WinoGeom g = wino_geom(d, bwd);
  const int h = bwd ? d->ho : d->h, w = bwd ? d->wo : d->w, ld = bwd ? d->ldy : d->ldx;
  const int pad_t = bwd ? 2 - d->pad_t : d->pad_t, pad_l = bwd ? 2 - d->pad_l : d->pad_l;
  const bool vec = g.K % 4 == 0 && ld % 4 == 0 && aligned16(src);
  const dim3 grid(grid_for(g.T * (size_t)(g.Kp / 4), 256, 1u << 20)), block(256);
  clear_stale_error();
  if (vec) hipLaunchKernelGGL(wino_input_kernel<true>, grid, block, 0, st, src, V, h, w, g.K, ld, g.th, g.tw, pad_t, pad_l, g.Kp, g.T);
  else hipLaunchKernelGGL(wino_input_kernel<false>, grid, block, 0, st, src, V, h, w, g.K, ld, g.th, g.tw, pad_t, pad_l, g.Kp, g.T);
  return check_launch("wino_input");
}

int wino_output(const a3d_conv_desc* d, bool bwd, const float* M, float* out, const float* bias, const float* mask, int act,
                hipStream_t st) {
  const WinoGeom g = wino_geom(d, bwd);
  const int ld = bwd ? d->ldx : d->ldy;
  const bool vec = g.N % 4 == 0 && ld % 4 == 0 && aligned16(out) && aligned16(mask);
  const dim3 grid(grid_for(g.T * (size_t)(g.Np / 4), 256, 1u << 20)), block(256);
  clear_stale_error();
  if (vec) hipLaunchKernelGGL(wino_output_kernel<true>, grid, block, 0, st, M, out, bias, mask, act, g.oh, g.ow, g.N, ld, g.th, g.tw, g.Np, g.T);
  else hipLaunchKernelGGL(wino_output_kernel<false>, grid, block, 0, st, M, out, bias, mask, act, g.oh, g.ow, g.N, ld, g.th, g.tw, g.Np, g.T);
  return check_launch("wino_output");
}

a3d_timing_record wino_record(int mode, const WinoGeom& g) {
  return timing_record(mode, A3D_PREC_F32, kBM, kBN, kWavesM, kNWaves, kBK, 4, 4, 0, (int)(16 * g.T), g.N, g.K);
}

int wino_gemm(IgemmParams& p, const WinoGeom& g, hipStream_t st) {
  using Cfg = IgemmCfg<MODE_FWD, kBM, kBN, kWavesM, kNWaves, kBK, 4, 4>;
  static bool attr_done[64] = {};
  int dev = 0;
  (void)hipGetDevice(&dev);
  if (dev < 0 || dev >= 64 || !attr_done[dev]) {
    hipError_t e = hipFuncSetAttribute(reinterpret_cast<const void*>(wino_gemm_kernel), hipFuncAttributeMaxDynamicSharedMemorySize,
                                       (int)Cfg::LDS_BYTES);
    if (e != hipSuccess) return set_error(A3D_ELAUNCH, "hipFuncSetAttribute: %s", hipGetErrorString(e));
    if (dev >= 0 && dev < 64) attr_done[dev] = true;
  }
  p.splitk = 1;
  p.ktiles_per_split = (p.K + kBK - 1) / kBK;
  p.tiles_m = (p.M + kBM - 1) / kBM;
  p.tiles_n = (p.N + kBN - 1) / kBN;
  p.slab = (size_t)p.M * p.N;
  clear_stale_error();
  hipLaunchKernelGGL(wino_gemm_kernel, dim3((unsigned)(p.tiles_m * p.tiles_n), 16), dim3(Cfg::NT), Cfg::LDS_BYTES, st, p,
                     g.T * (size_t)g.Kp, (size_t)g.Kp * g.Np, g.T * (size_t)g.Np);
  return check_launch("wino_gemm");
}


template <bool VEC>
__global__ __launch_bounds__(256) void wino_dz_kernel(const float* __restrict__ dz, float* __restrict__ Z, int ho, int wo, int k, int ld,
                                                      int th, int tw, int Kp, size_t T) {
  const int cqn = Kp / 4;
  const size_t total = T * (size_t)cqn;
  for (size_t i = (size_t)blockIdx.x * 256 + threadIdx.x; i < total; i += (size_t)gridDim.x * 256) {
    const int cq = (int)(i % cqn);
    const size_t t = i / cqn;
    const int tj = (int)(t % tw), ti = (int)((t / tw) % th);
    const size_t img = t / ((size_t)tw * th);
    f4 y[2][2];
#pragma unroll
    for (int a = 0; a < 2; ++a)
#pragma unroll
      for (int b = 0; b < 2; ++b) {
        f4 v = f4(0.f);
        const int yy = 2 * ti + a, xx = 2 * tj + b;
        if (yy < ho && xx < wo) {
          const float* src = dz + ((img * ho + yy) * wo + xx) * (size_t)ld + cq * 4;
          if (VEC) {
            v = *reinterpret_cast<const f4*>(src);
          } else {
#pragma unroll
            for (int e = 0; e < 4; ++e)
              if (cq * 4 + e < k) v[e] = src[e];
          }
        }
        y[a][b] = v;
      }
    const f4 r[4][2] = {{y[0][0], y[0][1]}, {y[0][0] + y[1][0], y[0][1] + y[1][1]}, {y[0][0] - y[1][0], y[0][1] - y[1][1]},
                        {-y[1][0], -y[1][1]}};
#pragma unroll
    for (int a = 0; a < 4; ++a) {
      const f4 z[4] = {r[a][0], r[a][0] + r[a][1], r[a][0] - r[a][1], -r[a][1]};
#pragma unroll
      for (int b = 0; b < 4; ++b) *reinterpret_cast<f4*>(Z + ((size_t)(a * 4 + b) * T + t) * Kp + cq * 4) = z[b];
    }
  }
}

__global__ __launch_bounds__(256) void wino_dw_kernel(const float* __restrict__ slabs, const float* __restrict__ bparts, float* __restrict__ dw,
                                                      float* __restrict__ db, int c, int k, int Cp, int Kp, int splits) {
  const size_t total = (size_t)c * k, plane = (size_t)Cp * Kp;
  for (size_t i = (size_t)blockIdx.x * 256 + threadIdx.x; i < total; i += (size_t)gridDim.x * 256) {
    const int col = (int)(i % k), row = (int)(i / k);
    const size_t at = (size_t)row * Kp + col;
    float m[4][4];
#pragma unroll
    for (int xi = 0; xi < 16; ++xi) m[xi / 4][xi % 4] = slabs[(size_t)xi * splits * plane + at];
    for (int z = 1; z < splits; ++z) {
      float v[16];
#pragma unroll
      for (int xi = 0; xi < 16; ++xi) v[xi] = slabs[((size_t)xi * splits + z) * plane + at];
#pragma unroll
      for (int xi = 0; xi < 16; ++xi) m[xi / 4][xi % 4] += v[xi];
    }
    float t[3][4];
#pragma unroll
    for (int b = 0; b < 4; ++b) {
      const float hs = (m[1][b] + m[2][b]) * 0.5f;
      t[0][b] = m[0][b] + hs;
      t[1][b] = (m[1][b] - m[2][b]) * 0.5f;
      t[2][b] = hs + m[3][b];
    }
#pragma unroll
    for (int a = 0; a < 3; ++a) {
      const float hs = (t[a][1] + t[a][2]) * 0.5f;
      const float g[3] = {t[a][0] + hs, (t[a][1] - t[a][2]) * 0.5f, hs + t[a][3]};
#pragma unroll
      for (int b = 0; b < 3; ++b) dw[((size_t)(a * 3 + b) * c + row) * k + col] = g[b];
    }
    if (db && row == 0) {
      float s = bparts[col];
      for (int z = 1; z < splits; ++z) s += bparts[(size_t)z * Kp + col];
      db[col] = s;
    }
  }
}

constexpr int kBiasPlane = 1 * 4 + 1;
__global__ __launch_bounds__(64 * kNWaves, 2 * kNWaves / 4) void wino_grad_gemm_kernel(const IgemmParams p, const size_t batch_a,
                                                                                        const size_t batch_b, const size_t batch_c) {
  IgemmParams q = p;
  q.A = p.A + (size_t)blockIdx.y * batch_a;
  q.B = p.B + (size_t)blockIdx.y * batch_b;
  q.C = p.C + (size_t)blockIdx.y * batch_c;
  if (blockIdx.y != kBiasPlane) q.dbias = nullptr;
  igemm_body<MODE_BWD_F, kBM, kBN, kWavesM, kNWaves, kBK, 4, 4>(q, gridDim.x, blockIdx.x);
}

constexpr int kBlockSlots = 512, kCUs = 256, kMinKTiles = 5;
int wino_grad_splits(int C, int K, size_t T) {
  const long blocks1 = 16L * ((C + kBM - 1) / kBM) * ((K + kBN - 1) / kBN);
  const long nk = (long)((T + kBK - 1) / kBK);
  const long smax = std::max(1L, std::min(kBlockSlots / blocks1, nk / kMinKTiles));
  long s = 1, load = (blocks1 + kCUs - 1) / kCUs;
  for (long t = 2; t <= smax; ++t) {
    const long l = (blocks1 * t + kCUs - 1) / kCUs;
    if (l * s < load * t) { s = t; load = l; }
  }
  const int forced = tune_int("A3D_WINO_GRAD_SPLIT", 0);
  if (forced > 0) s = std::min((long)forced, nk);
  const long per = (nk + s - 1) / s;
  return (int)((nk + per - 1) / per);
}

WinoGradGeom wino_grad_geom(const a3d_conv_desc* d) {
  const WinoGeom w = wino_geom(d, false);
  WinoGradGeom g{};
  g.T = w.T; g.Cp = w.Kp; g.Kp = w.Np;
  g.splits = wino_grad_splits(d->c, d->k, w.T);
  auto up = [](size_t b) { return (b + 255) / 256 * 256; };
  g.v_bytes = w.v_bytes;
  g.z_bytes = w.m_bytes;
  g.slab_bytes = up((size_t)16 * g.splits * g.Cp * g.Kp * 4);
  g.bias_bytes = up((size_t)g.splits * g.Kp * 4);
  return g;
}

bool wino_grad_applicable(const a3d_conv_desc* d) {
  if (d->precision != A3D_PREC_F32 && d->precision != A3D_PREC_F32_WINOGRAD) return false;
  a3d_conv_desc e = *d;
  e.precision = A3D_PREC_F32_WINOGRAD;
  return wino_applicable(&e);
}

int wino_dz(const a3d_conv_desc* d, const float* dz, float* Z, hipStream_t st) {
  const WinoGeom g = wino_geom(d, false);
  const bool vec = d->k % 4 == 0 && d->ldy % 4 == 0 && aligned16(dz);
  const dim3 grid(grid_for(g.T * (size_t)(g.Np / 4), 256, 1u << 20)), block(256);
  clear_stale_error();
  if (vec) hipLaunchKernelGGL(wino_dz_kernel<true>, grid, block, 0, st, dz, Z, d->ho, d->wo, d->k, d->ldy, g.th, g.tw, g.Np, g.T);
  else hipLaunchKernelGGL(wino_dz_kernel<false>, grid, block, 0, st, dz, Z, d->ho, d->wo, d->k, d->ldy, g.th, g.tw, g.Np, g.T);
  return check_launch("wino_dz");
}

int wino_dw(const a3d_conv_desc* d, const WinoGradGeom& g, const float* slabs, const float* bparts, float* dw, float* db, hipStream_t st) {
  clear_stale_error();
  hipLaunchKernelGGL(wino_dw_kernel, dim3(grid_for((size_t)d->c * d->k, 256, 1u << 20)), dim3(256), 0, st, slabs, bparts, dw, db, d->c, d->k,
                     g.Cp, g.Kp, g.splits);
  return check_launch("wino_dw");
}

a3d_timing_record wino_grad_record(const a3d_conv_desc* d, const WinoGradGeom& g) {
  a3d_timing_record r = timing_record(MODE_BWD_F, A3D_PREC_F32, kBM, kBN, kWavesM, kNWaves, kBK, 4, 4, 0, d->c, d->k, (int)(16 * g.T));
  r.splitk = g.splits;
  return r;
}

int wino_grad_gemm(IgemmParams& p, const WinoGradGeom& g, hipStream_t st) {
  using Cfg = IgemmCfg<MODE_BWD_F, kBM, kBN, kWavesM, kNWaves, kBK, 4, 4>;
  static bool attr_done[64] = {};
  int dev = 0;
  (void)hipGetDevice(&dev);
  if (dev < 0 || dev >= 64 || !attr_done[dev]) {
    hipError_t e = hipFuncSetAttribute(reinterpret_cast<const void*>(wino_grad_gemm_kernel), hipFuncAttributeMaxDynamicSharedMemorySize,
                                       (int)Cfg::LDS_BYTES);
    if (e != hipSuccess) return set_error(A3D_ELAUNCH, "hipFuncSetAttribute: %s", hipGetErrorString(e));
    if (dev >= 0 && dev < 64) attr_done[dev] = true;
  }
  const int nk = (p.K + kBK - 1) / kBK;
  p.splitk = g.splits;
  p.ktiles_per_split = (nk + g.splits - 1) / g.splits;
  p.tiles_m = (p.M + kBM - 1) / kBM;
  p.tiles_n = (p.N + kBN - 1) / kBN;
  p.slab = (size_t)p.M * p.N;
  clear_stale_error();
  hipLaunchKernelGGL(wino_grad_gemm_kernel, dim3((unsigned)(p.tiles_m * p.tiles_n * p.splitk), 16), dim3(Cfg::NT), Cfg::LDS_BYTES, st, p,
                     g.T * (size_t)g.Cp, g.T * (size_t)g.Kp, (size_t)g.splits * g.Cp * g.Kp);
  return check_launch("wino_grad_gemm");
}

}
```

ann3depth_amd/models.py:

```python
import collections
import contextlib
import ctypes
import math
import os

import numpy as np
import torch

from . import _lib, augment as augment_, ops
from ._lib import ConvDesc
from .feed import DeviceFeed

NET_H, NET_W = 228, 304
OUT_H, OUT_W = 55, 74
SAMPLES_COARSE = 2000000
SAMPLES_FINE = 1500000

ConvSpec = collections.namedtuple('ConvSpec', 'name cin cout k stride padding relu')

MSDN_CONVS = [
    ConvSpec('coarse/conv/conv2d_0', 3, 96, 11, 4, 'VALID', True),
    ConvSpec('coarse/conv/conv2d_1', 96, 256, 5, 1, 'SAME', True),
    ConvSpec('coarse/conv/conv2d_2', 256, 384, 3, 1, 'SAME', True),
    ConvSpec('coarse/conv/conv2d_3', 384, 384, 3, 1, 'SAME', True),
# ... 146 lines not shown
        self._poison_seen = []
        self.fuse_pool = precision == 'fp32'
        self.side = None
        if self.overlap and dev.type == 'cuda':
            handle = ctypes.c_void_p()
            with torch.cuda.device(dev):
                ops.check(_lib.load().a3d_stream_create(1, ctypes.byref(handle)), 'a3d_stream_create')
            self.side = torch.cuda.ExternalStream(handle.value, device=dev)
            self._side_handle = handle.value
        shapes = collections.OrderedDict()
        for c in MSDN_CONVS:
            shapes[c.name + '/kernel'] = (c.k, c.k, c.cin, c.cout)
            shapes[c.name + '/bias'] = (c.cout,)
        for n, i, o in MSDN_DENSES:
            shapes[n + '/kernel'] = (i, o)
            shapes[n + '/bias'] = (o,)
        self.shapes = shapes
        self.groups = collections.OrderedDict()
        self.group_of = {}
        for gname, (lr, scopes) in MSDN_OPTIMIZERS.items():
            gshapes = collections.OrderedDict((n, s) for n, s in shapes.items()
                                              if any(n.startswith(sc + '/') for sc in scopes))
            world = reducer.world_size if (reducer is not None and gname == 'CoarseDense') else 1
            self.groups[gname] = ParamGroup(gname, lr, gshapes, dev, beta2=beta2, multiple=world)
            for n in gshapes:
                self.group_of[n] = gname
        if params is None:
            rng = np.random.default_rng(seed)
            params = {n: (glorot_uniform(rng, s) if n.endswith('/kernel') else np.zeros(s, np.float32))
                      for n, s in shapes.items()}
        self.load_params(params)

        def buf(*shape):
            return torch.empty(shape, device=dev)

        def abuf(*shape):
            return torch.empty(shape, device=dev, dtype=torch.bfloat16 if self.bf16s else torch.float32)
        self.conv = {c.name: c for c in MSDN_CONVS}
        self.x = buf(B, NET_H, NET_W, 3)
        self.t = buf(B, OUT_H, OUT_W, 1)
        self.c0 = None if self.bf16s else buf(B, 55, 74, 96)
        self.c1 = None if self.bf16s else buf(B, 27, 37, 256)
        self.p0 = abuf(B, 27, 37, 96); self.p1 = abuf(B, 13, 18, 256)
        self.c2 = abuf(B, 13, 18, 384); self.c3 = abuf(B, 13, 18, 384); self.c4 = abuf(B, 6, 8, 256)
        self.drop = buf(B, 4096)
        self.coarse = buf(B, OUT_H, OUT_W, 1)
        self.f1 = buf(B, 110, 148, 63) if not self.bf16s else None
        self.cat = abuf(B, OUT_H, OUT_W, 64)
        self.f2 = buf(B, OUT_H, OUT_W, 64)
        self.fine = buf(B, OUT_H, OUT_W, 1)
        self.loss_coarse = buf(1); self.loss_fine = buf(1)
        if grad_weight > 0:
            self.loss_quad_c = buf(4); self.loss_quad_f = buf(4)
            self.loss_pair_c = self.loss_quad_c[:2]; self.loss_pair_f = self.loss_quad_f[:2]
            self.loss_coarse = self.loss_pair_c[:1]; self.loss_fine = self.loss_pair_f[:1]
        elif valid_range is not None:
            self.loss_pair_c = buf(2); self.loss_pair_f = buf(2)
            self.loss_coarse = self.loss_pair_c[:1]; self.loss_fine = self.loss_pair_f[:1]
        self.loss_out_c, self.loss_out_f = ((self.loss_quad_c, self.loss_quad_f) if grad_weight > 0 else
                                            (self.loss_pair_c, self.loss_pair_f) if valid_range is not None else
                                            (self.loss_coarse, self.loss_fine))
        self.a0 = torch.empty((B, 27, 37, 96), dtype=torch.uint8, device=dev)
        self.a1 = torch.empty((B, 13, 18, 256), dtype=torch.uint8, device=dev)
        self.af1 = torch.empty((B, OUT_H, OUT_W, 63), dtype=torch.uint8, device=dev)
        self.pooled_fwd = None
        silog_ws = ops.silog_grad_ws if grad_weight > 0 else ops.silog_ws if valid_range is None else ops.silog_masked_ws
        self.ws_c = silog_ws(B, dev); self.ws_f = silog_ws(B, dev)
        self.t_one = buf(B, 1, 1, 1) if valid_range is not None else None
        self.dz1 = buf(B, OUT_H * OUT_W); self.dz0 = buf(B, 4096)
        self.dc4 = abuf(B, 6, 8, 256); self.dc3 = abuf(B, 13, 18, 384); self.dc2 = abuf(B, 13, 18, 384)
        self.dp1 = abuf(B, 13, 18, 256); self.dc1 = abuf(B, 27, 37, 256)
        self.dp0 = abuf(B, 27, 37, 96); self.dc0 = None
        self.dfine = buf(B, OUT_H, OUT_W, 1); self.df2 = abuf(B, OUT_H, OUT_W, 64)
        self.dcat = abuf(B, OUT_H, OUT_W, 64); self.df1 = None
        if self.bf16s:
            self.c4_32 = buf(B, 6, 8, 256)
            self.dz0_16 = torch.empty((B, 4096), device=dev, dtype=torch.bfloat16)
            self.dense_bf16_x = B <= 64
            if not self.dense_bf16_x:
                self.dc4_32 = buf(B, 6, 8, 256)
            NP = (OUT_H * OUT_W + 7) // 8 * 8
            self.w1pad = torch.zeros((4096, NP), device=dev, dtype=torch.bfloat16)
            self.b1pad = torch.zeros((1, NP), device=dev)
            self.drop16 = torch.empty((B, 4096), device=dev, dtype=torch.bfloat16)
            self.dz1_16 = torch.zeros((B, NP), device=dev, dtype=torch.bfloat16)
        def D(*a):
            return ops.conv_desc(*a, precision=precision)
        self.d = {
            'coarse/conv/conv2d_0': D(B, NET_H, NET_W, 3, 96, 11, 11, 4, 'VALID'),
            'coarse/conv/conv2d_1': D(B, 27, 37, 96, 256, 5, 5, 1, 'SAME'),
            'coarse/conv/conv2d_2': D(B, 13, 18, 256, 384, 3, 3, 1, 'SAME'),
            'coarse/conv/conv2d_3': D(B, 13, 18, 384, 384, 3, 3, 1, 'SAME'),
            'coarse/conv/conv2d_4': D(B, 13, 18, 384, 256, 3, 3, 2, 'VALID'),
            'fine/first/conv2d': D(B, NET_H, NET_W, 3, 63, 9, 9, 2, 'VALID'),
            'fine/second/conv2d': D(B, OUT_H, OUT_W, 64, 64, 5, 5, 1, 'SAME'),
            'fine/third': D(B, OUT_H, OUT_W, 64, 1, 5, 5, 1, 'SAME'),
        }
        self.d_wino = {}
        if precision == 'fp32' and dev.type == 'cuda':
            for n in self.WINO_LAYERS:
                d = self.d[n]
                if d.n * -(-d.ho // 2) * -(-d.wo // 2) >= self.WINO_MIN_TILES:
                    e = self.d_wino[n] = ConvDesc.from_buffer_copy(d)
                    e.precision = ops.PREC['fp32w']
        self.wino_grad = set()
        if precision == 'fp32' and dev.type == 'cuda':
            for n in self.WINO_GRAD_LAYERS:
                d = self.d[n]
                if d.n * -(-d.ho // 2) * -(-d.wo // 2) >= self.WINO_GRAD_MIN_TILES:
                    self.wino_grad.add(n)
        self.d_few = {}
        if dev.type == 'cuda':
            few_prec = 'bf16' if self.bf16s else 'fp32'
            for n, dd in (('coarse/conv/conv2d_0', ops.conv_desc(B, NET_H, NET_W, 3, 96, 11, 11, 4, 'VALID', precision=few_prec)),
                          ('fine/first/conv2d', ops.conv_desc(B, NET_H, NET_W, 3, 63, 9, 9, 2, 'VALID', precision=few_prec))):
                if ops.conv2d_bwd_filter_pooled_supported(dd):
                    self.d_few[n] = dd
        self.store = {}
        self.wcopy = {}
        if self.bf16s:
            X, W, Y = ops.STORE_X, ops.STORE_W, ops.STORE_Y
            for n in ('coarse/conv/conv2d_1', 'coarse/conv/conv2d_2', 'coarse/conv/conv2d_3', 'coarse/conv/conv2d_4'):
                self.store[n] = {'fwd': X | W | Y, 'bwd_d': X | W | Y, 'bwd_f': X | Y}
            self.store['coarse/conv/conv2d_0'] = {'bwd_f': Y}
            self.d['fine/first/conv2d'].precision = ops.PREC['fp32']
            self.store['fine/second/conv2d'] = {'fwd': X | W, 'bwd_d': W | X | Y, 'bwd_f': X | Y}
            self.x4 = torch.empty((B, NET_H, NET_W, 4), device=dev, dtype=torch.bfloat16)
            self.w0_4 = torch.zeros((11, 11, 4, 96), device=dev)
            self.d0_4 = ops.with_storage(ops.conv_desc(B, NET_H, NET_W, 4, 96, 11, 11, 4, 'VALID', ldy=96, precision='bf16'),
                                         X | Y)
            self.w4 = torch.zeros((9, 9, 4, 63), device=dev)
            self.d4 = ops.with_storage(ops.conv_desc(B, NET_H, NET_W, 4, 63, 9, 9, 2, 'VALID', ldy=64, precision='bf16'),
                                       X | Y)
            for n in list(self.store) + ['coarse/dense/dense_0']:
                if n == 'coarse/dense/dense_0' or self.store[n].get('fwd', 0) & W:
                    self.wcopy[n] = torch.empty(self.shapes[n + '/kernel'], device=dev, dtype=torch.bfloat16)
            self.refresh_weight_copies()

    def __del__(self):
        handle, self._side_handle = getattr(self, '_side_handle', None), None
        if handle:
            try:
                torch.cuda.synchronize(self.device)
                ops.drop_workspace(handle)
                _lib.load().a3d_stream_destroy(handle)
            except Exception:
                pass

    SHARE_CU = ('fine/first/conv2d', 'fine/second/conv2d')
    WINO_LAYERS = ('coarse/conv/conv2d_2', 'coarse/conv/conv2d_3')
    WINO_MIN_TILES = 504
    WINO_GRAD_LAYERS = WINO_LAYERS
    WINO_GRAD_MIN_TILES = 504

    def _desc(self, name, which):
        d = self.d[name]
        bits = self.store.get(name, {}).get(which, 0)
        if which == 'fwd' and self.side is not None and name in self.SHARE_CU and name not in self._alone:
            key = (name, bits)
            if key not in self._shared_desc:
                e = ops.with_storage(d, bits)
                e.hints = ops.HINT_SHARE_CU
                self._shared_desc[key] = e
            return self._shared_desc[key]
        return ops.with_storage(d, bits) if bits else d

    def _w(self, name, which='fwd'):
        if name in self.wcopy and (name not in self.store or self.store[name][which] & ops.STORE_W):
            return self.wcopy[name]
        return self._v(name + '/kernel')

    def _prepared(self, key, desc, w, which='fwd'):
        if self.device.type != 'cuda':
            return desc, w
        pf = self._prep.get(key)
        if pf is None:
            pf = self._prep[key] = ops.PreparedFilter(desc, self.device, which)
            pf.source = w
            if pf.ok:
                pf.refresh(w)
        return (pf.desc_prepared, pf.buf) if pf.ok else (desc, w)

    def _refresh_prepared(self):
        for pf in self._prep.values():
            if pf.ok:
                pf.refresh(pf.source)

    def refresh_weight_copies(self):
        for n, c in self.wcopy.items():
            ops.cast_bf16(self._v(n + '/kernel'), c)
        if self.bf16s:
            self.w4[:, :, :3, :] = self._v('fine/first/conv2d/kernel')
            self.w0_4[:, :, :3, :] = self._v('coarse/conv/conv2d_0/kernel')
            n = 'coarse/dense/dense_1'
            ops.cast_rows(self._v(n + '/kernel'), self.w1pad)
            ops.cast_rows(self._v(n + '/bias').view(1, -1), self.b1pad)

    def _weights_moved(self, *groups):
        if not all(g.frozen() for g in groups):
            if self.wcopy:
                self.refresh_weight_copies()
            self._refresh_prepared()

    def settle(self):
        if self._deferred is not None:
            works, group, scale = self._deferred
            self._deferred = None
            if works and isinstance(works[0], tuple):
                self._poll_poison()
                for work, a, b in works:
                    self.reducer.wait(work)
                    group.apply_slice(a, b, scale, poisoned=self._poison)
                group.advance()
                self._m_sharded = True
                self._watch_poison()
                return
            for work in works:
                self.reducer.wait(work)
            group.apply(scale)
            self._weights_moved(group)

    def _dense_buckets(self):
        if self._dense_pieces is None:
            gd = self.groups['CoarseDense']
            q = self.reducer.world_size * ParamGroup.ALIGN
            c = -(-gd.offsets['coarse/dense/dense_1/kernel'][0] // q) * q
            third = -(-(c // 3) // q) * q
            self._dense_pieces = ([(c, gd.count)], [(0, third), (third, 2 * third), (2 * third, c)])
        return self._dense_pieces

    def _my_slice(self, a, b):
        n = (b - a) // self.reducer.world_size
        return a + self.reducer.rank * n, a + (self.reducer.rank + 1) * n

    def _watch_poison(self):
        red = self.reducer
        work = red.any(self._poison)
        red.wait(work)
        if not hasattr(self, '_poison_ring'):
            ring = torch.empty(4, dtype=torch.int32)
            self._poison_ring = (ring.pin_memory() if self.device.type == 'cuda' else ring, 0)
        ring, nxt = self._poison_ring
        self._poison_ring = (ring, (nxt + 1) % 4)
        host = ring[nxt:nxt + 1]
        host.copy_(self._poison, non_blocking=True)
        ev = None
        if self.device.type == 'cuda':
            ev = torch.cuda.Event()
            ev.record()
        self._poison_seen.append((ev, host))

    def _poll_poison(self, block=False):
        while self._poison_seen and (block or len(self._poison_seen) >= 2):
            ev, host = self._poison_seen.pop(0)
            if ev is not None:
                ev.synchronize()
            if int(host.item()):
                self._resync()

    def _resync(self):
        gd = self.groups['CoarseDense']
        early, late = self._dense_buckets()
        for a, b in early + late:
            for buf in (gd.var, gd.v, gd.m):
                self.reducer.all_gather(buf[a:b])
        self._poison.zero_()
        self._poison_seen = []
        self._m_sharded = False

    def gather_state(self):
        self.settle()
        if self._m_sharded:
            self._poll_poison(block=True)
        if self._m_sharded:
            gd = self.groups['CoarseDense']
            early, late = self._dense_buckets()
            for a, b in early + late:
                self.reducer.all_gather(gd.m[a:b])
            self._m_sharded = False

    def load_params(self, params):
        self.settle()
        for n, shp in self.shapes.items():
            g = self.groups[self.group_of[n]]
            a = np.asarray(params[n], np.float32)
            assert a.shape == tuple(shp), (n, a.shape, shp)
            g.view(g.var, n).copy_(torch.from_numpy(np.ascontiguousarray(a)))
        if getattr(self, 'wcopy', None):
            self.refresh_weight_copies()
        if getattr(self, '_prep', None):
            self._refresh_prepared()

    def _v(self, name):
        g = self.groups[self.group_of[name]]
        return g.view(g.var, name)

    def _g(self, name):
        g = self.groups[self.group_of[name]]
        return g.view(g.grad, name)

    def var(self, name):
        self.settle()
        return self._v(name)

    def grad(self, name):
        self.settle()
# ... 128 lines not shown
        pooled = pooled.float()
        c = arg.shape[-1]
        out = torch.zeros_like(full)
        ph, pw = arg.shape[1], arg.shape[2]
        win = out[:, :2 * ph, :2 * pw, :].reshape(full.shape[0], ph, 2, pw, 2, c)
        a = arg.long()
        for pos in range(4):
            win[:, :, pos >> 1, :, pos & 1, :] = torch.where(a == pos, pooled[..., :c], torch.zeros_like(pooled[..., :c]))
        return out

    def _conv_pool(self, name, x, y_pooled, argmax=None):
        d, w = self._fwd_operands(name)
        ops.conv2d_pool_fwd(d, x, w, self._v(name + '/bias'), y_pooled, 'relu', argmax)

    def _fine_first_image_form(self, argmax=None):
        d, w = self._prepared(('fine/first/image', 0, 0, 0), self.d4, self.w4)
        ops.conv2d_pool_fwd(d, self.x4, w, self._v('fine/first/conv2d/bias'), self.cat, 'relu', argmax)

    def forward(self, images, depths, keep_mask, join=True, phase=None, warp=None):
        if depths is None:
            pass
        elif self.valid_range is not None:
            lo, hi = self.valid_range
            if warp is not None:
                ops.warp_bilinear_pair_valid(images, self.x, depths, self.t, warp, lo, hi)
            elif images.shape[:3] == depths.shape[:3]:
                ops.resize_bilinear_tf1_pair_valid(images, self.x, depths, self.t, lo, hi)
            else:
                ops.resize_bilinear_tf1(images, self.x)
                ops.resize_bilinear_tf1_valid(depths, self.t, lo, hi, scratch=self.t_one)
        elif warp is not None:
            ops.warp_bilinear_pair(images, self.x, depths, self.t, warp)
        elif images.shape[:3] == depths.shape[:3]:
            ops.resize_bilinear_tf1_pair(images, self.x, depths, self.t)
        else:
            ops.resize_bilinear_tf1(images, self.x)
            ops.resize_bilinear_tf1(depths, self.t)
        B = self.B
        self.dropout_on = keep_mask is not None
        self._alone = ('fine/second/conv2d',) if phase == 2 else ()
        if self.bf16s:
            ops.pad_channels_bf16(self.x, self.x4)
        fused = self.fuse_pool and phase in (1, 2, 3)
        self.pooled_fwd = phase if fused else None
        lean_fine = fused
        if fused:
            train = phase == 1
            self._conv_pool('coarse/conv/conv2d_0', self.x, self.p0, self.a0 if train else None)
            self._conv_pool('coarse/conv/conv2d_1', self.p0, self.p1, self.a1 if train else None)
        elif self.bf16s:
            d, w = self._prepared(('conv2d_0/image', 0, 0, 0), self.d0_4, self.w0_4)
            ops.conv2d_pool_fwd(d, self.x4, w, self._v('coarse/conv/conv2d_0/bias'), self.p0, 'relu', self.a0)
            self._conv_pool('coarse/conv/conv2d_1', self.p0, self.p1, self.a1)
        else:
            self._conv('coarse/conv/conv2d_0', self.x, self.c0)
            ops.maxpool2x2_fwd(self.c0, self.p0)
            self._conv('coarse/conv/conv2d_1', self.p0, self.c1)
            ops.maxpool2x2_fwd(self.c1, self.p1)
        def fine_first():
            with self._beside():
                if lean_fine:
                    self._conv_pool('fine/first/conv2d', self.x, self.cat, self.af1 if phase == 2 else None)
                elif self.bf16s:
                    self._fine_first_image_form(None if phase in (1, 3) else self.af1)
                else:
                    self._conv('fine/first/conv2d', self.x, self.f1)
        self._conv('coarse/conv/conv2d_2', self.p1, self.c2)
        self._conv('coarse/conv/conv2d_3', self.c2, self.c3)
        fine_first()
        self._c4_32_fresh = False
        if self.bf16s and self.dense_bf16_x and phase == 1:
            n4 = 'coarse/conv/conv2d_4'
            ops.conv2d_fwd(self._desc(n4, 'fwd'), self.c3, self._w(n4), self._v(n4 + '/bias'), self.c4, 'relu',
                           out2=ops.second_output(self.c4_32.view(-1, 256)))
            self._c4_32_fresh = True
        else:
            self._conv('coarse/conv/conv2d_4', self.c3, self.c4)
        if not self._sharded_in_flight():
            self.settle()
        w, b = self._kb('coarse/dense/dense_0')
        if self.bf16s and self.dense_bf16_x:
            ops.dense_fwd_ex(self.c4.view(B, -1), self.wcopy['coarse/dense/dense_0'], b, self.drop, 'relu',
                             drop_keep=keep_mask, precision='bf16', storage=ops.STORE_W | ops.STORE_X,
                             out2=ops.second_output(self.drop16))
        elif self.bf16s:
            ops.cast_bf16(self.c4, self.c4_32)
            ops.dense_fwd_ex(self.c4_32.view(B, -1), self.wcopy['coarse/dense/dense_0'], b, self.drop, 'relu',
                             drop_keep=keep_mask, precision='bf16', storage=ops.STORE_W)
        else:
            ops.dense_fwd(self.c4.view(B, -1), w, b, self.drop, 'relu', drop_keep=keep_mask)
        w, b = self._kb('coarse/dense/dense_1')
        cat_done = self.bf16s and self.dense_bf16_x
        if cat_done:
            ops.dense_fwd_ex(self.drop16, self.w1pad, self.b1pad, self.coarse.view(B, -1), None, precision='bf16',
                             storage=ops.STORE_W | ops.STORE_X, n=self.w1pad.shape[1],
                             out2=ops.second_output(self.cat, cols=OUT_H * OUT_W, step=64, offset=63, ld=OUT_H * OUT_W))
        else:
            ops.dense_fwd(self.drop, w, b, self.coarse.view(B, -1))
        with self._beside():
            if cat_done:
                pass
            elif lean_fine or self.bf16s:
                ops.copy_channel(self.coarse, 0, self.cat, 63)
            else:
                ops.maxpool2x2_fwd(self.f1, self.cat, extra=self.coarse)
            self._conv('fine/second/conv2d', self.cat, self.f2)
            self._conv('fine/third', self.f2, self.fine)
            if depths is not None:
                self._loss_fwd(self.fine, self.loss_out_f, self.ws_f)
        if depths is not None:
            self._loss_fwd(self.coarse, self.loss_out_c, self.ws_c)
        if join:
            self._join()

    def predict(self, images, n=None):
        B = self.B
        n = images.shape[0] if n is None else int(n)
        check_rows('predict', n, B, f'a batch of {images.shape[0]} images', images.shape[0])
        ops.resize_bilinear_tf1(images[:n], self.x[:n])
        if n < B:
            self.x[n:].zero_()
        self.forward(images, None, None, join=True, phase=3)
        return self.coarse.view(B, OUT_H, OUT_W), self.fine.view(B, OUT_H, OUT_W)

    def _loss_fwd(self, out, loss, ws):
        if self.grad_weight > 0:
            ops.silog_grad_loss_fwd(out, self.t, OUT_H, OUT_W, self.valid_range is not None, self.grad_weight, loss, ws)
        elif self.valid_range is None:
            ops.silog_loss_fwd(out, self.t, loss, ws)
        else:
            ops.silog_masked_loss_fwd(out, self.t, loss, ws)

    def _loss_bwd(self, out, ws, dout, dout16=None):
        if self.grad_weight > 0:
            ops.silog_grad_loss_bwd(out, self.t, OUT_H, OUT_W, self.valid_range is not None, self.grad_weight, ws, dout, dout16)
        elif self.valid_range is None:
            ops.silog_loss_bwd(out, self.t, ws, dout, dout16)
        else:
            ops.silog_masked_loss_bwd(out, self.t, ws, dout, dout16)

    def _sharded_in_flight(self):
        d = self._deferred
        return d is not None and bool(d[0]) and isinstance(d[0][0], tuple)

    def _fused_dense_adam(self):
        return not self.keep_dense_grads and self.groups['CoarseDense'].frozen()

    def _bwd_data(self, name, dz, dx, relu_mask=None):
        d, w = self._desc(name, 'bwd_d'), self._w(name, 'bwd_d')
        if name in self.d_wino:
            d, w = self._prepared((name, 'bwd_d', 'fp32w'), self.d_wino[name], w, 'bwd_d')
        ops.conv2d_bwd_data(d, dz, w, dx, relu_mask=relu_mask)

    def _bwd_filter(self, name, x, dz):
        if name in self.d:
            call = ops.conv2d_bwd_filter_wino if name in self.wino_grad else ops.conv2d_bwd_filter
            call(self._desc(name, 'bwd_f'), x, dz, self._g(name + '/kernel'), self._g(name + '/bias'))
        elif self._fused_dense_adam():
            g = self.groups[self.group_of[name + '/kernel']]
            kw = [g.view(buf, name + '/kernel') for buf in (g.var, g.m, g.v)]
            kb = [g.view(buf, name + '/bias') for buf in (g.var, g.m, g.v)]
            ops.dense_bwd_filter_adam_tf1(x, dz, *kw, *kb, g.lr, g.beta1, g.beta2, float(g.beta1_power),
                                          float(g.beta2_power), 1.0, precision='bf16' if self.bf16s else 'fp32')
        else:
            ops.dense_bwd_filter(x, dz, self._g(name + '/kernel'), self._g(name + '/bias'))

    def backward_coarse(self, after_dense=None, after_conv2=None, after_dense1=None):
        B = self.B
        bf16_x = self.bf16s and self.dense_bf16_x
        self._loss_bwd(self.coarse, self.ws_c, self.dz1.view(B, OUT_H, OUT_W, 1),
                       dout16=self.dz1_16 if bf16_x else None)
        self.settle()
        n = 'coarse/dense/dense_1'
        self._bwd_filter(n, self.drop, self.dz1)
        if after_dense1 is not None:
            after_dense1()
        if bf16_x:
            ops.dense_bwd_data_ex(self.dz1_16, self.w1pad, self.dz0, mask=self.drop, scale=2.0 if self.dropout_on else 1.0,
                                  precision='bf16', storage=ops.STORE_W | ops.STORE_Y,
                                  out2=ops.second_output(self.dz0_16))
        else:
            ops.dense_bwd_data(self.dz1, self._v(n + '/kernel'), self.dz0, mask=self.drop, scale=2.0 if self.dropout_on else 1.0)
        n = 'coarse/dense/dense_0'
        if bf16_x and not self._c4_32_fresh:
            ops.cast_bf16(self.c4, self.c4_32)
        flat = (self.c4_32 if self.bf16s else self.c4).view(B, -1)
        self._bwd_filter(n, flat, self.dz0)
        if bf16_x:
            ops.dense_bwd_data_ex(self.dz0_16, self.wcopy[n], self.dc4.view(B, -1), mask=self.c4.view(B, -1), scale=1.0,
                                  precision='bf16', storage=ops.STORE_W | ops.STORE_X | ops.STORE_Y)
        elif self.bf16s:
            ops.dense_bwd_data_ex(self.dz0, self.wcopy[n], self.dc4_32.view(B, -1), mask=flat, scale=1.0, precision='bf16',
                                  storage=ops.STORE_W)
            ops.cast_bf16(self.dc4_32, self.dc4)
        else:
            ops.dense_bwd_data(self.dz0, self._v(n + '/kernel'), self.dc4.view(B, -1), mask=flat, scale=1.0)
        if after_dense is not None:
            after_dense()
        n = 'coarse/conv/conv2d_4'
        self._bwd_filter(n, self.c3, self.dc4)
        self._bwd_data(n, self.dc4, self.dc3, relu_mask=self.c3)
        self._join()
        dw = self._bwd_filter
        n = 'coarse/conv/conv2d_3'
        dw(n, self.c2, self.dc3)
        self._bwd_data(n, self.dc3, self.dc2, relu_mask=self.c2)
        n = 'coarse/conv/conv2d_2'
        dw(n, self.p1, self.dc2)
        if after_conv2 is not None:
            after_conv2()
        self._bwd_data(n, self.dc2, self.dp1)
        pooled = self.pooled_fwd == 1 or self.bf16s
        if pooled:
            ops.maxpool2x2_bwd_idx(self.a1, self.p1, self.dp1, self.dc1, relu_mask=True)
        else:
            ops.maxpool2x2_bwd(self.c1, self.dp1, self.dc1, relu_mask=True)
        n = 'coarse/conv/conv2d_1'
        dw(n, self.p0, self.dc1)
        self._bwd_data(n, self.dc1, self.dp0)
        n = 'coarse/conv/conv2d_0'
        if pooled and n in self.d_few:
            ops.conv2d_bwd_filter_pooled(self.d_few[n], self.x, self.dp0, self.p0, self.a0, self._g(n + '/kernel'),
                                         self._g(n + '/bias'))
            return
        if self.dc0 is None:
            self.dc0 = torch.empty((self.B, 55, 74, 96), device=self.device, dtype=self.dp0.dtype)
        if pooled:
            ops.maxpool2x2_bwd_idx(self.a0, self.p0, self.dp0, self.dc0, relu_mask=True)
        else:
            ops.maxpool2x2_bwd(self.c0, self.dp0, self.dc0, relu_mask=True)
        dw(n, self.x, self.dc0)

    def backward_fine(self):
        self._join()
        self._loss_bwd(self.fine, self.ws_f, self.dfine)
        n = 'fine/third'
        if ops.conv2d_bwd_both_supported(self.d[n]):
            ops.conv2d_bwd_both(self.d[n], self.f2, self.dfine, self._v(n + '/kernel'), self._g(n + '/kernel'),
                                self._g(n + '/bias'), self.df2, relu_mask=True)
        else:
            assert not self.bf16s, 'bf16 storage: df2 is a bf16 tensor only the fused backward writes'
            self._bwd_filter(n, self.f2, self.dfine)
            self._bwd_data(n, self.dfine, self.df2, relu_mask=self.f2)
        n = 'fine/second/conv2d'
        self._bwd_filter(n, self.cat, self.df2)
        self._bwd_data(n, self.df2, self.dcat)
        n = 'fine/first/conv2d'
        if (self.pooled_fwd == 2 or self.bf16s) and n in self.d_few:
            ops.conv2d_bwd_filter_pooled(self.d_few[n], self.x, self.dcat, self.cat, self.af1, self._g(n + '/kernel'),
                                         self._g(n + '/bias'))
            return
        if self.df1 is None:
            self.df1 = torch.empty((self.B, 110, 148, 63), device=self.device)
        if self.pooled_fwd == 2 or self.bf16s:
            ops.maxpool2x2_bwd_idx(self.af1, self.cat, self.dcat, self.df1, relu_mask=True)
        else:
            ops.maxpool2x2_bwd(self.f1, self.dcat, self.df1, relu_mask=True)
        self._bwd_filter(n, self.x, self.df1)

    def step(self, images, depths, keep_mask, warp=None):
        if keep_mask is not None and keep_mask.dtype != torch.uint8:
            keep_mask = keep_mask.to(torch.uint8)
        phase = phase_of(self.global_step, self.B)
        self.forward(images, depths, keep_mask, join=False, phase=phase, warp=warp)
        red = self.reducer
        scale = 1.0 / red.world_size if red is not None else 1.0
        if phase == 1:
            gc, gd = self.groups['CoarseConv'], self.groups['CoarseDense']
            if red is None:
                fused = self._fused_dense_adam()
                self.backward_coarse()
                gc.apply(scale)
                if fused:
                    gd.advance()
                else:
                    gd.apply(scale)
                self._weights_moved(gc, gd)
            else:
                handle, tail = [], []
                cut = gc.offsets['coarse/conv/conv2d_2/kernel'][0]
                if gd.frozen() and self.dense_exchange == 'reduce_scatter':
                    early, late = self._dense_buckets()
                    if self._poison is None:
                        self._poison = torch.zeros(1, dtype=torch.int32, device=self.device)

                    def scatter(pieces):
                        for a, b in pieces:
                            work, _ = red.reduce_scatter(gd.grad[a:b])
                            handle.append((work,) + self._my_slice(a, b))
                    after_dense1, after_dense = (lambda: scatter(early)), (lambda: scatter(late))
                else:
                    d1 = gd.offsets['coarse/dense/dense_1/kernel'][0]
                    third = -(-(d1 // 3) // ParamGroup.ALIGN) * ParamGroup.ALIGN
                    pieces0 = [(0, third), (third, 2 * third), (2 * third, d1)]
                    after_dense1 = lambda: handle.append(red.start(gd.grad[d1:]))
                    after_dense = lambda: handle.extend(red.start(gd.grad[a:b]) for a, b in pieces0)
                self.backward_coarse(after_dense1=after_dense1, after_dense=after_dense,
                                     after_conv2=lambda: tail.append(red.start(gc.grad[cut:], urgent=True)))
                head = red.start(gc.grad[:cut], urgent=True)
                red.wait(tail[0])
                red.wait(head)
                gc.apply(scale)
                self._weights_moved(gc)
                self._deferred = (handle, gd, scale)
        elif phase == 2:
            ga, gb = self.groups['FineA'], self.groups['FineB']
            self.backward_fine()
            if red is not None:
                red.start(ga.grad)
                red.start(gb.grad)
                red.finish()
            ga.apply(scale)
            gb.apply(scale)
            self._weights_moved(ga, gb)
        self._join()
        self.global_step += 1
        return {'coarse_loss': self.loss_coarse, 'fine_loss': self.loss_fine, 'phase': phase}


DCNF_IMG_H, DCNF_IMG_W = 240, 320
DCNF_PATCH, DCNF_SP = 100, 40
DCNF_PREFIX = 'unary/unary_layers/'
DCNF_CONVS = [('conv2d', 3, 64, 11), ('conv2d_1', 64, 256, 5), ('conv2d_2', 256, 256, 3),
              ('conv2d_3', 256, 256, 3), ('conv2d_4', 256, 256, 3)]
DCNF_POOL_AFTER = ('conv2d', 'conv2d_1', 'conv2d_4')
DCNF_DENSES = [('dense', 12544, 128, 'relu'), ('dense_1', 128, 16, 'sigmoid'), ('dense_2', 16, 1, None)]


class DCNFUnary:

    def __init__(self, batchsize, device='cuda', params=None, seed=3000, precision='fp32'):
        self.B = batchsize
        self.device = dev = torch.device(device)
        self.rows, _ = ops.same_pad(DCNF_IMG_H, DCNF_PATCH, DCNF_SP)
        self.cols, _ = ops.same_pad(DCNF_IMG_W, DCNF_PATCH, DCNF_SP)
        self.P = P = batchsize * self.rows * self.cols
        shapes = collections.OrderedDict()
        for n, ci, co, k in DCNF_CONVS:
            shapes[DCNF_PREFIX + n + '/kernel'] = (k, k, ci, co)
            shapes[DCNF_PREFIX + n + '/bias'] = (co,)
        for n, i, o, _ in DCNF_DENSES:
            shapes[DCNF_PREFIX + n + '/kernel'] = (i, o)
            shapes[DCNF_PREFIX + n + '/bias'] = (o,)
        self.shapes = shapes
        self.group = ParamGroup('unary', 0.1, shapes, dev, slots=False)
        if params is None:
            rng = np.random.default_rng(seed)
            params = {n: (glorot_uniform(rng, s) if n.endswith('/kernel') else np.zeros(s, np.float32))
                      for n, s in shapes.items()}
        for n, s in shapes.items():
            self.group.view(self.group.var, n).copy_(torch.from_numpy(np.ascontiguousarray(params[n], np.float32)))

        def buf(*shape):
            return torch.empty(shape, device=dev)
        self.resized = buf(batchsize, DCNF_IMG_H, DCNF_IMG_W, 3)
        self.act = collections.OrderedDict()
        self.dact = {}
        self.desc = {}
        self.fuse_pool = precision == 'fp32'
        self.argmax, self.conv_hw = {}, {}
        self.few_pooled = False
        self.act['x'] = buf(P, DCNF_PATCH, DCNF_PATCH, 3)
        h = DCNF_PATCH
        for n, ci, co, k in DCNF_CONVS:
            self.desc[n] = ops.conv_desc(P, h, h, ci, co, k, k, 1, 'VALID', precision=precision)
            h = h - k + 1
            self.conv_hw[n] = h
            if not (self.fuse_pool and n in DCNF_POOL_AFTER):
                self.act[n] = buf(P, h, h, co)
# ... 721 lines not shown
```

ann3depth_amd/ops.py:

```python
import ctypes

import torch

from . import _lib
from ._lib import ConvDesc, check

ACT = {None: 0, 'relu': 1, 'sigmoid': 2}
PREC = {'fp32': 0, 'f32': 0, 'bf16x3': 1, 'bf16': 2, 'fp32w': 3}


def _ptr(t):
    return None if t is None else ctypes.c_void_p(t.data_ptr())


def _stream():
    return ctypes.c_void_p(torch.cuda.current_stream().cuda_stream)


class Workspace:

    def __init__(self):
        self.buf = None

    def reserve(self, nbytes, device):
        if self.buf is None or self.buf.numel() < nbytes or self.buf.device != device:
            if torch.cuda.is_current_stream_capturing():
                raise RuntimeError(f'workspace of {nbytes} bytes must be reserved before graph capture')
            self.buf = torch.empty(max(nbytes, 1 << 20), dtype=torch.uint8, device=device)
        return self.buf

    def get(self, nbytes, device):
        buf = self.reserve(nbytes, device)
        return ctypes.c_void_p(buf.data_ptr()), buf.numel()


_WS = {}


def _ws():
    key = torch.cuda.current_stream().cuda_stream
    w = _WS.get(key)
    if w is None:
        w = _WS[key] = Workspace()
    return w


def drop_workspace(stream_handle):
    _WS.pop(stream_handle, None)


def same_pad(in_size, k, stride):
    out = -(-in_size // stride)
    pad = max((out - 1) * stride + k - in_size, 0)
    return out, pad // 2


STORE_X, STORE_W, STORE_Y = 1, 2, 4


HINT_SHARE_CU = 1
HINT_W_PREPARED = 2


class PreparedFilter:

    def __init__(self, desc, device, which='fwd'):
        lib = _lib.load()
        self.stem = {'fwd': 'a3d_conv2d_fwd', 'bwd_d': 'a3dw_conv2d_bwd_data'}[which]
        nbytes = getattr(lib, self.stem + '_prepared_filter_bytes')(ctypes.byref(desc))
        self.ok = nbytes > 0
        self.desc = desc
        if self.ok:
            self.buf = torch.empty(nbytes, dtype=torch.uint8, device=device)
            self.desc_prepared = ConvDesc.from_buffer_copy(desc)
            self.desc_prepared.hints = desc.hints | HINT_W_PREPARED

    def refresh(self, w):
        name = self.stem + '_prepare_filter'
        check(getattr(_lib.load(), name)(ctypes.byref(self.desc), _ptr(w), _ptr(self.buf), self.buf.numel(), _stream()), name)


def conv_desc(n, h, w, c, k, r, s, stride, padding, ldx=None, ldy=None, precision='fp32', storage=0, hints=0):
    padding = padding.upper()
    if padding == 'SAME':
        ho, pt = same_pad(h, r, stride)
        wo, pl = same_pad(w, s, stride)
    elif padding == 'VALID':
        ho, pt = (h - r) // stride + 1, 0
        wo, pl = (w - s) // stride + 1, 0
    else:
        raise ValueError(padding)
    return ConvDesc(n=n, h=h, w=w, c=c, k=k, r=r, s=s, stride=stride, pad_t=pt, pad_l=pl, ho=ho, wo=wo,
                    ldx=ldx or c, ldy=ldy or k, precision=PREC[precision], storage=storage, hints=hints)


def second_output(t, cols=None, step=1, offset=0, ld=None):
    if t is None:
        return None
    ld = t.shape[-1] if ld is None else ld
    o = _lib.SecondOutput(t.data_ptr(), ld, step, offset, int(t.dtype == torch.bfloat16), ld if cols is None else cols)
    o._keep = t
    return o


def _o2(out2):
    return None if out2 is None else ctypes.byref(out2)


def conv2d_fwd(d, x, w, bias, y, act=None, out2=None):
    lib = _lib.load()
    ws, n = _ws().get(lib.a3d_conv2d_fwd_ws_bytes(ctypes.byref(d)), x.device)
    if out2 is not None:
        check(lib.a3d_conv2d_fwd_ex2(ctypes.byref(d), _ptr(x), _ptr(w), _ptr(bias), _ptr(y), ACT[act], _o2(out2), ws, n, _stream()),
              'a3d_conv2d_fwd_ex2')
        return y
    check(lib.a3d_conv2d_fwd(ctypes.byref(d), _ptr(x), _ptr(w), _ptr(bias), _ptr(y), ACT[act], ws, n, _stream()),
          'a3d_conv2d_fwd')
    return y


def conv2d_pool_fwd(d, x, w, bias, y_pooled, act='relu', argmax=None):
    lib = _lib.load()
    ws, n = _ws().get(lib.a3d_conv2d_fwd_ws_bytes(ctypes.byref(d)), x.device)
    check(lib.a3d_conv2d_pool_fwd(ctypes.byref(d), _ptr(x), _ptr(w), _ptr(bias), _ptr(y_pooled), y_pooled.shape[-1],
                                  _ptr(argmax), ACT[act], ws, n, _stream()), 'a3d_conv2d_pool_fwd')
    return y_pooled


def maxpool2x2_bwd_idx(argmax, y_pooled, dy, dx, relu_mask=True):
    n, h, w, c = dx.shape
    if y_pooled.dtype == torch.bfloat16 and dx.dtype == torch.bfloat16:
        assert dy.dtype == torch.bfloat16
        name = 'a3d_maxpool2x2_bwd_idx_bf16s'
    elif y_pooled.dtype == torch.bfloat16:
        assert dy.dtype == torch.bfloat16 and dx.dtype == torch.float32
        name = 'a3d_maxpool2x2_bwd_idx_bf16'
    else:
        name = 'a3d_maxpool2x2_bwd_idx'
    check(getattr(_lib.load(), name)(n, h, w, c, _ptr(argmax), _ptr(y_pooled), y_pooled.shape[-1], _ptr(dy), dy.shape[-1],
                                     _ptr(dx), int(relu_mask), _stream()), name)
    return dx


def copy_channel(src, c_src, dst, c_dst):
    npix = src.numel() // src.shape[-1]
    assert dst.numel() // dst.shape[-1] == npix
    fn = _lib.load().a3d_copy_channel_bf16 if dst.dtype == torch.bfloat16 else _lib.load().a3d_copy_channel
    check(fn(npix, _ptr(src), src.shape[-1], c_src, _ptr(dst), dst.shape[-1], c_dst, _stream()), 'a3d_copy_channel')
    return dst


def conv2d_bwd_data(d, dz, w, dx, relu_mask=None):
    lib = _lib.load()
    ws, n = _ws().get(lib.a3d_conv2d_bwd_data_ws_bytes(ctypes.byref(d)), dz.device)
    check(lib.a3d_conv2d_bwd_data(ctypes.byref(d), _ptr(dz), _ptr(w), _ptr(dx), _ptr(relu_mask), ws, n, _stream()),
          'a3d_conv2d_bwd_data')
    return dx


def conv2d_bwd_filter(d, x, dz, dw, db=None):
    lib = _lib.load()
    ws, n = _ws().get(lib.a3d_conv2d_bwd_filter_ws_bytes(ctypes.byref(d)), x.device)
    check(lib.a3d_conv2d_bwd_filter(ctypes.byref(d), _ptr(x), _ptr(dz), _ptr(dw), _ptr(db), ws, n, _stream()),
          'a3d_conv2d_bwd_filter')
    return dw, db


def conv2d_bwd_filter_wino(d, x, dz, dw, db=None):
    lib = _lib.load()
    ws, n = _ws().get(lib.a3dwg_conv2d_bwd_filter_ws_bytes(ctypes.byref(d)), x.device)
    check(lib.a3dwg_conv2d_bwd_filter(ctypes.byref(d), _ptr(x), _ptr(dz), _ptr(dw), _ptr(db), ws, n, _stream()),
          'a3dwg_conv2d_bwd_filter')
    return dw, db


def conv2d_bwd_filter_pooled_supported(d):
    return _lib.load().a3d_conv2d_bwd_filter_pooled_ws_bytes(ctypes.byref(d)) > 0


def conv2d_bwd_filter_pooled(d, x, dpool, pooled, argmax, dw, db=None):
    lib = _lib.load()
    ws, n = _ws().get(lib.a3d_conv2d_bwd_filter_pooled_ws_bytes(ctypes.byref(d)), x.device)
    assert pooled is None or (pooled.dtype == dpool.dtype and pooled.shape[-1] == dpool.shape[-1])
    check(lib.a3d_conv2d_bwd_filter_pooled(ctypes.byref(d), _ptr(x), _ptr(dpool), dpool.shape[-1], _ptr(pooled), _ptr(argmax),
                                           argmax.shape[-1], int(dpool.dtype == torch.bfloat16), _ptr(dw), _ptr(db), ws, n,
                                           _stream()), 'a3d_conv2d_bwd_filter_pooled')
    return dw, db


_BOTH_STATE = {}


def conv2d_bwd_both_supported(d):
    return bool(_lib.load().a3d_conv2d_bwd_both_supported(ctypes.byref(d)))


def conv2d_bwd_both(d, x, dz, w, dw, db, dx, relu_mask=True):
    lib = _lib.load()
    key = (torch.cuda.current_stream().cuda_stream, x.device)
    state = _BOTH_STATE.get(key)
    if state is None:
        state = _BOTH_STATE[key] = torch.zeros(64, dtype=torch.int32, device=x.device)
    ws, n = _ws().get(lib.a3d_conv2d_bwd_both_ws_bytes(ctypes.byref(d)), x.device)
    check(lib.a3d_conv2d_bwd_both(ctypes.byref(d), _ptr(x), _ptr(dz), _ptr(w), _ptr(dw), _ptr(db), _ptr(dx), dx.shape[-1],
                                  int(dx.dtype == torch.bfloat16), int(bool(relu_mask)), _ptr(state), ws, n, _stream()),
          'a3d_conv2d_bwd_both')
    return dw, db, dx


def dense_fwd(x, w, bias, y, act=None, drop_keep=None):
    m, k = x.shape
    n = w.shape[1]
    lib = _lib.load()
    ws, nb = _ws().get(lib.a3d_dense_fwd_ws_bytes(m, k, n), x.device)
    check(lib.a3d_dense_fwd(m, k, n, _ptr(x), _ptr(w), _ptr(bias), _ptr(y), ACT[act], _ptr(drop_keep), ws, nb,
                            _stream()), 'a3d_dense_fwd')
    return y


def dense_bwd_data(dz, w, dx, mask=None, scale=1.0, mask_act='relu'):
    m, n = dz.shape
    k = w.shape[0]
    lib = _lib.load()
    ws, nb = _ws().get(lib.a3d_dense_bwd_data_ws_bytes(m, k, n), dz.device)
    check(lib.a3d_dense_bwd_data(m, k, n, _ptr(dz), _ptr(w), _ptr(dx), _ptr(mask), ACT[mask_act], scale, ws, nb,
                                 _stream()),
          'a3d_dense_bwd_data')
    return dx


def dense_bwd_filter(x, dz, dw, db=None):
    m, k = x.shape
    n = dz.shape[1]
    lib = _lib.load()
    ws, nb = _ws().get(lib.a3d_dense_bwd_filter_ws_bytes(m, k, n), x.device)
    check(lib.a3d_dense_bwd_filter(m, k, n, _ptr(x), _ptr(dz), _ptr(dw), _ptr(db), ws, nb, _stream()),
          'a3d_dense_bwd_filter')
    return dw, db


def maxpool2x2_fwd(x, y, extra=None):
    n, h, w, c = x.shape
    check(_lib.load().a3d_maxpool2x2_fwd(n, h, w, c, _ptr(x), _ptr(y), y.shape[-1], _ptr(extra), _stream()),
          'a3d_maxpool2x2_fwd')
    return y


def maxpool2x2_bwd(x, dy, dx, relu_mask=True):
    n, h, w, c = x.shape
    check(_lib.load().a3d_maxpool2x2_bwd(n, h, w, c, _ptr(x), _ptr(dy), dy.shape[-1], _ptr(dx), int(relu_mask),
                                         _stream()), 'a3d_maxpool2x2_bwd')
    return dx


def _pair_args(x0, y0, x1=None, y1=None):
    def one(x, y):
        if x is None:
            return 0, None, 0, 0, 0, None
        return x.shape[3], _ptr(x), int(x.dtype == torch.uint8), y.shape[1], y.shape[2], _ptr(y)
    return tuple(x0.shape[:3]) + one(x0, y0) + one(x1, y1)


def resize_bilinear_tf1(x, y):
    n, h, w, c = x.shape
    if x.dtype == torch.uint8:
        check(_lib.load().a3d_resize_bilinear_tf1_ex(*_pair_args(x, y), _stream()), 'a3d_resize_bilinear_tf1_ex')
        return y
    check(_lib.load().a3d_resize_bilinear_tf1(n, h, w, c, _ptr(x), y.shape[1], y.shape[2], _ptr(y), _stream()),
          'a3d_resize_bilinear_tf1')
    return y


def resize_bilinear_tf1_pair(x0, y0, x1, y1):
    n, h, w, c0 = x0.shape
    assert x1.shape[:3] == (n, h, w)
    if x0.dtype == torch.uint8 or x1.dtype == torch.uint8:
        check(_lib.load().a3d_resize_bilinear_tf1_ex(*_pair_args(x0, y0, x1, y1), _stream()), 'a3d_resize_bilinear_tf1_ex')
        return
    check(_lib.load().a3d_resize_bilinear_tf1_pair(n, h, w, c0, _ptr(x0), y0.shape[1], y0.shape[2], _ptr(y0), x1.shape[3],
                                                   _ptr(x1), y1.shape[1], y1.shape[2], _ptr(y1), _stream()),
          'a3d_resize_bilinear_tf1_pair')


WARP_STRIDE = 12


def _check_pair(who, x0, y0, x1, y1, table):
    if x0.dim() != 4 or y0.dim() != 4 or y0.shape[0] != x0.shape[0] or y0.shape[3] != x0.shape[3]:
        raise ValueError(f'{who}: {tuple(x0.shape)} -> {tuple(y0.shape)}')
    n, h, w, c0 = x0.shape
    if (x1 is None) != (y1 is None):
        raise ValueError(f'{who}: x1 and y1 go together')
    if x1 is not None and (x1.dim() != 4 or tuple(x1.shape[:3]) != (n, h, w) or y1.dim() != 4
                           or y1.shape[0] != n or y1.shape[3] != x1.shape[3]):
        raise ValueError(f'{who}: second tensor {tuple(x1.shape)} -> {tuple(y1.shape)} beside '
                         f'{tuple(x0.shape)}')
    if table is not None and (tuple(table.shape) != (n, WARP_STRIDE) or table.dtype != torch.float32):
        raise ValueError(f'{who}: table {tuple(table.shape)} {table.dtype}, want [{n}, {WARP_STRIDE}] float32')
    for name, t, dtypes in (('x0', x0, (torch.float32, torch.uint8)), ('y0', y0, (torch.float32,)),
                            ('x1', x1, (torch.float32, torch.uint8)), ('y1', y1, (torch.float32,)),
                            ('table', table, (torch.float32,))):
        if t is None:
            continue
        if t.dtype not in dtypes:
            raise ValueError(f'{who}: {name} is {t.dtype}')
        if not t.is_cuda or t.device != x0.device:
            raise ValueError(f'{who}: {name} is on {t.device}, x0 on {x0.device}')
        if not t.is_contiguous():
            raise ValueError(f'{who}: {name} is not contiguous')
    return n, h, w, c0


def warp_bilinear_pair(x0, y0, x1, y1, table):
    if table is None:
        raise ValueError('warp_bilinear_pair: no table')
    _check_pair('warp_bilinear_pair', x0, y0, x1, y1, table)
    check(_lib.load().a3d_warp_bilinear_pair(*_pair_args(x0, y0, x1, y1), _ptr(table), _stream()), 'a3d_warp_bilinear_pair')


def _valid_range(who, x1, min_depth, max_depth):
    if x1 is None:
        raise ValueError(f'{who}: the depth map x1 is required')
    lo, hi = float(min_depth), float(max_depth)
    if not lo <= hi:
        raise ValueError(f'{who}: min_depth {lo}, max_depth {hi}')
    return lo, hi
# ... 812 lines not shown
```

Baseline: 12280.

## Fuse Winograd backward filter and data passes into one chained routine

Adds a combined Winograd backward entry point that transforms x and dz in one kernel, runs the filter-gradient and data-gradient GEMMs as a paired launch, and finishes dw/db reduction and dx output transform (with relu mask or maxpool backward folded in) in a single kernel. It is used for coarse conv2d_3 and conv2d_2 when both Winograd routes apply. This aims to cut kernel launches and intermediate tensor round-trips, and to skip the separate maxpool backward pass. It needs more workspace and adds several new kernel variants, which raises correctness risk.

After: 12460, median of 6. 1.5% higher.

```diff
diff --git a/ann3depth_amd/_lib.py b/ann3depth_amd/_lib.py
--- a/ann3depth_amd/_lib.py
+++ b/ann3depth_amd/_lib.py
@@ -173,6 +173,16 @@
     'a3dwg_conv2d_bwd_filter': (c_int, [_D, _P, _P, _P, _P, _P, c_size_t, _P]),
 }
 
+class WinoBwdPool(ctypes.Structure):
+    _fields_ = [('argmax', c_void_p), ('y', c_void_p), ('ldy', c_int), ('h2', c_int), ('w2', c_int)]
+
+
+WINO_BWD_SIGNATURES = {
+    'a3dwb_sizeof_pool': (c_size_t, []),
+    'a3dwb_conv2d_bwd_ws_bytes': (c_size_t, [_D, c_int, c_int]),
+    'a3dwb_conv2d_bwd': (c_int, [_D, _P, _P, _P, _P, _P, _P, _P, ctypes.POINTER(WinoBwdPool), _P, c_size_t, _P]),
+}
+
 UPSAMPLE_SIGNATURES = {
     'a3du_joint_bilateral_upsample': (c_int, [c_int, c_int, c_int, _P, c_int, c_int, _P, c_int, _P, _P, _P, _P, c_int, c_float,
                                               c_float, _P, _P]),
@@ -210,7 +220,8 @@
                               + list(CRF_VALID_SIGNATURES.items()) + list(FCSP_SIGNATURES.items())
                               + list(CRF_BAND_SIGNATURES.items()) + list(WINO_SIGNATURES.items())
                               + list(UPSAMPLE_SIGNATURES.items()) + list(POSTERIOR_SIGNATURES.items())
-                              + list(WINO_GRAD_SIGNATURES.items()) + list(SLIC_SIGNATURES.items())):
+                              + list(WINO_GRAD_SIGNATURES.items()) + list(SLIC_SIGNATURES.items())
+                              + list(WINO_BWD_SIGNATURES.items())):
         try:
             fn = getattr(lib, name)
         except AttributeError as e:
@@ -220,6 +231,9 @@
     if lib.a3d_sizeof_conv_desc() != ctypes.sizeof(ConvDesc):
         raise A3dError(f'liba3d.so reads a {lib.a3d_sizeof_conv_desc()}-byte a3d_conv_desc, this binding passes '
                        f'{ctypes.sizeof(ConvDesc)} bytes: stale build?')
+    if lib.a3dwb_sizeof_pool() != ctypes.sizeof(WinoBwdPool):
+        raise A3dError(f'liba3d.so reads a {lib.a3dwb_sizeof_pool()}-byte a3dwb_pool, this binding passes '
+                       f'{ctypes.sizeof(WinoBwdPool)} bytes: stale build?')
     _lib = lib
     return lib
 
diff --git a/ann3depth_amd/csrc/a3d_internal.h b/ann3depth_amd/csrc/a3d_internal.h
--- a/ann3depth_amd/csrc/a3d_internal.h
+++ b/ann3depth_amd/csrc/a3d_internal.h
@@ -135,4 +135,14 @@
 a3d_timing_record wino_grad_record(const a3d_conv_desc* d, const WinoGradGeom& g);
 int wino_grad_gemm(IgemmParams& p, const WinoGradGeom& g, hipStream_t st);
 
+struct WinoBwdPool {
+  const uint8_t* argmax;
+  const float* y;
+  int ldy, h2, w2;
+};
+int wino_bwd_transforms(const a3d_conv_desc* d, const float* x, const float* dz, float* Vx, float* Vdz, float* Z, hipStream_t st);
+int wino_bwd_gemm(IgemmParams& pf, const WinoGradGeom& gg, IgemmParams& pd, const WinoGeom& g, hipStream_t st);
+int wino_bwd_finish(const a3d_conv_desc* d, const WinoGradGeom& gg, const float* slabs, const float* bparts, float* dw, float* db,
+                    const float* M, float* dx, const float* mask, const WinoBwdPool* pool, hipStream_t st);
+
 }
diff --git a/ann3depth_amd/csrc/igemm_host.hip b/ann3depth_amd/csrc/igemm_host.hip
--- a/ann3depth_amd/csrc/igemm_host.hip
+++ b/ann3depth_amd/csrc/igemm_host.hip
@@ -2,6 +2,7 @@
 
 #include "../../include/a3d_wino.h"
 #include "../../include/a3d_wino_grad.h"
+#include "../../include/a3d_wino_bwd.h"
 #include "a3d_internal.h"
 #include "igemm.h"
 #include "igemm_cfgs.h"
@@ -306,6 +307,19 @@
   const WinoGeom g = wino_geom(d, bwd);
   return (prepared ? 0 : g.u_bytes) + g.v_bytes + g.m_bytes;
 }
+static IgemmParams wino_product(const WinoGeom& g, const float* V, const float* U, float* M) {
+  a3d_conv_desc e{};
+  e.n = (int)g.T; e.h = e.w = e.ho = e.wo = 1; e.c = g.Kp; e.k = g.Np; e.r = e.s = 1; e.stride = 1; e.ldx = g.Kp; e.ldy = g.Np;
+  GemmProblem gp = fwd_problem(&e);
+  IgemmParams p;
+  fill_common(p, gp);
+  p.A = V; p.B = U; p.C = M;
+  p.npix = gp.M; p.nrsc = gp.K;
+  fill_gather(p, &e, g.Kp, 1, g.Kp);
+  p.ldb = g.Np; p.ldc = g.Np;
+  fill_staging(p, MODE_FWD, (unsigned long long)g.T * g.Kp, (unsigned long long)g.Kp * g.Np, 1, 1);
+  return p;
+}
 static int wino_conv(const a3d_conv_desc* d, bool bwd, const float* src, const float* w, float* out, const float* bias, const float* mask,
                      int act, bool prepared, void* ws, size_t ws_bytes, hipStream_t st) {
   const WinoGeom g = wino_geom(d, bwd);
@@ -325,16 +339,7 @@
   float* M = reinterpret_cast<float*>(base + g.v_bytes);
   rc = wino_input(d, bwd, src, V, st);
   if (rc != A3D_OK) return rc;
-  a3d_conv_desc e{};
-  e.n = (int)g.T; e.h = e.w = e.ho = e.wo = 1; e.c = g.Kp; e.k = g.Np; e.r = e.s = 1; e.stride = 1; e.ldx = g.Kp; e.ldy = g.Np;
-  GemmProblem gp = fwd_problem(&e);
-  IgemmParams p;
-  fill_common(p, gp);
-  p.A = V; p.B = U; p.C = M;
-  p.npix = gp.M; p.nrsc = gp.K;
-  fill_gather(p, &e, g.Kp, 1, g.Kp);
-  p.ldb = g.Np; p.ldc = g.Np;
-  fill_staging(p, MODE_FWD, (unsigned long long)g.T * g.Kp, (unsigned long long)g.Kp * g.Np, 1, 1);
+  IgemmParams p = wino_product(g, V, U, M);
   rc = timed_launch(wino_record(bwd ? MODE_BWD_D : MODE_FWD, g), st, [&] { return wino_gemm(p, g, st); });
   if (rc != A3D_OK) return rc;
   return wino_output(d, bwd, M, out, bias, mask, act, st);
@@ -823,6 +828,20 @@
 
 static bool wino_grad_takes(const a3d_conv_desc* d) { return check_desc(d) == A3D_OK && wino_grad_applicable(d); }
 
+static IgemmParams wino_grad_product(const WinoGradGeom& g, const float* V, const float* Z, float* slabs, float* bparts) {
+  a3d_conv_desc e{};
+  e.n = (int)g.T; e.h = e.w = e.ho = e.wo = 1; e.c = g.Cp; e.k = g.Kp; e.r = e.s = 1; e.stride = 1; e.ldx = g.Cp; e.ldy = g.Kp;
+  GemmProblem gp = bwd_f_problem(&e);
+  IgemmParams p;
+  fill_common(p, gp);
+  p.A = V; p.B = Z; p.C = slabs; p.dbias = bparts;
+  p.npix = gp.K; p.nrsc = gp.M;
+  fill_gather(p, &e, g.Cp, 1, g.Cp);
+  p.ldb = g.Kp; p.ldc = g.Kp;
+  fill_staging(p, MODE_BWD_F, (unsigned long long)g.T * g.Cp, (unsigned long long)g.T * g.Kp, 1, 1);
+  return p;
+}
+
 size_t a3dwg_conv2d_bwd_filter_ws_bytes(const a3d_conv_desc* d) {
   if (!wino_grad_takes(d)) return a3d_conv2d_bwd_filter_ws_bytes(d);
   const WinoGradGeom g = wino_grad_geom(d);
@@ -847,19 +866,87 @@
   if (rc != A3D_OK) return rc;
   rc = wino_dz(d, dz, Z, st);
   if (rc != A3D_OK) return rc;
-  a3d_conv_desc e{};
-  e.n = (int)g.T; e.h = e.w = e.ho = e.wo = 1; e.c = g.Cp; e.k = g.Kp; e.r = e.s = 1; e.stride = 1; e.ldx = g.Cp; e.ldy = g.Kp;
-  GemmProblem gp = bwd_f_problem(&e);
-  IgemmParams p;
-  fill_common(p, gp);
-  p.A = V; p.B = Z; p.C = slabs; p.dbias = db ? bparts : nullptr;
-  p.npix = gp.K; p.nrsc = gp.M;
-  fill_gather(p, &e, g.Cp, 1, g.Cp);
-  p.ldb = g.Kp; p.ldc = g.Kp;
-  fill_staging(p, MODE_BWD_F, (unsigned long long)g.T * g.Cp, (unsigned long long)g.T * g.Kp, 1, 1);
+  IgemmParams p = wino_grad_product(g, V, Z, slabs, db ? bparts : nullptr);
   rc = timed_launch(wino_grad_record(d, g), st, [&] { return wino_grad_gemm(p, g, st); });
   if (rc != A3D_OK) return rc;
   return wino_dw(d, g, slabs, bparts, dw, db, st);
+}
+
+static bool wino_bwd_takes(const a3d_conv_desc* d) {
+  if (!wino_grad_takes(d)) return false;
+  const WinoGeom gx = wino_geom(d, false), gd = wino_geom(d, true);
+  return gx.th <= gd.th && gx.tw <= gd.tw;
+}
+static a3d_conv_desc as_winograd(const a3d_conv_desc* d) {
+  a3d_conv_desc e = *d;
+  e.precision = A3D_PREC_F32_WINOGRAD;
+  return e;
+}
+
+size_t a3dwb_sizeof_pool(void) { return sizeof(a3dwb_pool); }
+
+size_t a3dwb_conv2d_bwd_ws_bytes(const a3d_conv_desc* d, int w_prepared, int pooled) {
+  (void)pooled;
+  if (!wino_bwd_takes(d)) return std::max(a3dwg_conv2d_bwd_filter_ws_bytes(d), a3d_conv2d_bwd_data_ws_bytes(d));
+  const a3d_conv_desc e = as_winograd(d);
+  const WinoGradGeom g = wino_grad_geom(&e);
+  return wino_bytes(&e, true, w_prepared != 0) + g.v_bytes + g.z_bytes + g.slab_bytes + g.bias_bytes;
+}
+
+int a3dwb_conv2d_bwd(const a3d_conv_desc* d, const float* x, const float* dz, const float* w_or_U, float* dw, float* db, float* dx,
+                     const float* relu_mask, const a3dwb_pool* pool, void* ws, size_t ws_bytes, void* stream) {
+  static_assert(sizeof(WinoBwdPool) == sizeof(a3dwb_pool), "WinoBwdPool mirrors a3dwb_pool");
+  if (!wino_bwd_takes(d)) {
+    A3D_CHECK_ARG(!pool, "conv2d_bwd (Winograd): a pool only where the Winograd routes take the descriptor");
+    const int rc = a3dwg_conv2d_bwd_filter(d, x, dz, dw, db, ws, ws_bytes, stream);
+    return rc != A3D_OK ? rc : a3d_conv2d_bwd_data(d, dz, w_or_U, dx, relu_mask, ws, ws_bytes, stream);
+  }
+  A3D_CHECK_ARG(x && dz && w_or_U && dw && dx, "conv2d_bwd (Winograd): null tensor");
+  A3D_CHECK_WS(ws, "conv2d_bwd (Winograd)");
+  A3D_CHECK_ARG(!(pool && relu_mask), "conv2d_bwd (Winograd): relu_mask and pool exclude each other");
+  A3D_CHECK_ARG(!pool || (pool->argmax && pool->y && pool->ldy >= d->c && pool->h2 >= 2 && pool->w2 >= 2 && pool->h2 / 2 == d->h &&
+                          pool->w2 / 2 == d->w),
+                "conv2d_bwd (Winograd): the pool's halved extents must be the layer's input's");
+  const a3d_conv_desc e = as_winograd(d);
+  const bool prepared = (d->hints & A3D_HINT_W_PREPARED) != 0;
+  const WinoGeom g = wino_geom(&e, true);
+  const WinoGradGeom gg = wino_grad_geom(&e);
+  const size_t need = wino_bytes(&e, true, prepared) + gg.v_bytes + gg.z_bytes + gg.slab_bytes + gg.bias_bytes;
+  if (!ws || need > ws_bytes) return set_error(A3D_EWORKSPACE, "conv2d_bwd (Winograd): need %zu workspace bytes", need);
+  A3D_CHECK_ARG(!prepared || aligned16(w_or_U), "conv2d_bwd (Winograd): the prepared filter must be 16-byte aligned");
+  hipStream_t st = static_cast<hipStream_t>(stream);
+  char* base = static_cast<char*>(ws);
+  const float* U = w_or_U;
+  int rc;
+  if (!prepared) {
+    rc = wino_filter(&e, true, w_or_U, reinterpret_cast<float*>(base), st);
+    if (rc != A3D_OK) return rc;
+    U = reinterpret_cast<const float*>(base);
+    base += g.u_bytes;
+  }
+  auto take = [&base](size_t bytes) {
+    float* p = reinterpret_cast<float*>(base);
+    base += bytes;
+    return p;
+  };
+  float *Vdz = take(g.v_bytes), *M = take(g.m_bytes);
+  float *Vx = take(gg.v_bytes), *Z = take(gg.z_bytes), *slabs = take(gg.slab_bytes), *bparts = take(gg.bias_bytes);
+  rc = wino_bwd_transforms(&e, x, dz, Vx, Vdz, Z, st);
+  if (rc != A3D_OK) return rc;
+  IgemmParams pf = wino_grad_product(gg, Vx, Z, slabs, db ? bparts : nullptr);
+  IgemmParams pd = wino_product(g, Vdz, U, M);
+  const a3d_timing_record rf = wino_grad_record(&e, gg), rd = wino_record(MODE_BWD_D, g);
+  if (timing_wanted(rf) || timing_wanted(rd) || tune_int("A3D_WINO_BWD_PAIR", 1) == 0) {
+    rc = timed_launch(rf, st, [&] { return wino_grad_gemm(pf, gg, st); });
+    if (rc != A3D_OK) return rc;
+    rc = timed_launch(rd, st, [&] { return wino_gemm(pd, g, st); });
+  } else {
+    rc = wino_bwd_gemm(pf, gg, pd, g, st);
+  }
+  if (rc != A3D_OK) return rc;
+  WinoBwdPool wp{};
+  if (pool) wp = WinoBwdPool{pool->argmax, pool->y, pool->ldy, pool->h2, pool->w2};
+  return wino_bwd_finish(&e, gg, slabs, bparts, dw, db, M, dx, relu_mask, pool ? &wp : nullptr, st);
 }
 
 static a3d_conv_desc dense_desc(int m, int k, int n) {
diff --git a/ann3depth_amd/csrc/wino.hip b/ann3depth_amd/csrc/wino.hip
--- a/ann3depth_amd/csrc/wino.hip
+++ b/ann3depth_amd/csrc/wino.hip
@@ -37,6 +37,47 @@
 #pragma unroll
       for (int b4 = 0; b4 < 4; ++b4) U[(size_t)(a4 * 4 + b4) * total + i] = u[b4];
     }
+  }
+}
+
+
+template <bool VEC>
+__device__ __forceinline__ void wino_load_window(const float* __restrict__ x, f4 (&d)[4][4], size_t img, int y0, int x0, int h, int w, int c,
+                                                 int ld, int cq) {
+#pragma unroll
+  for (int a = 0; a < 4; ++a)
+#pragma unroll
+    for (int b = 0; b < 4; ++b) {
+      f4 v = f4(0.f);
+      const int yy = y0 + a, xx = x0 + b;
+      if (yy >= 0 && yy < h && xx >= 0 && xx < w) {
+        const float* src = x + ((img * h + yy) * w + xx) * (size_t)ld + cq * 4;
+        if (VEC) {
+          v = *reinterpret_cast<const f4*>(src);
+        } else {
+#pragma unroll
+          for (int e = 0; e < 4; ++e)
+            if (cq * 4 + e < c) v[e] = src[e];
+        }
+      }
+      d[a][b] = v;
+    }
+}
+
+__device__ __forceinline__ void wino_input_store(const f4 (&d)[4][4], float* __restrict__ V, size_t T, size_t t, int Cp, int cq) {
+  f4 r[4][4];
+#pragma unroll
+  for (int b = 0; b < 4; ++b) {
+    r[0][b] = d[0][b] - d[2][b];
+    r[1][b] = d[1][b] + d[2][b];
+    r[2][b] = d[2][b] - d[1][b];
+    r[3][b] = d[1][b] - d[3][b];
+  }
+#pragma unroll
+  for (int a = 0; a < 4; ++a) {
+    const f4 v[4] = {r[a][0] - r[a][2], r[a][1] + r[a][2], r[a][2] - r[a][1], r[a][1] - r[a][3]};
+#pragma unroll
+    for (int b = 0; b < 4; ++b) *reinterpret_cast<f4*>(V + ((size_t)(a * 4 + b) * T + t) * Cp + cq * 4) = v[b];
   }
 }
 
@@ -50,40 +91,22 @@
     const size_t t = i / cqn;
     const int tj = (int)(t % tw), ti = (int)((t / tw) % th);
     const size_t img = t / ((size_t)tw * th);
-    const int y0 = 2 * ti - pad_t, x0 = 2 * tj - pad_l;
     f4 d[4][4];
-#pragma unroll
-    for (int a = 0; a < 4; ++a)
-#pragma unroll
-      for (int b = 0; b < 4; ++b) {
-        f4 v = f4(0.f);
-        const int yy = y0 + a, xx = x0 + b;
-        if (yy >= 0 && yy < h && xx >= 0 && xx < w) {
-          const float* src = x + ((img * h + yy) * w + xx) * (size_t)ld + cq * 4;
-          if (VEC) {
-            v = *reinterpret_cast<const f4*>(src);
-          } else {
-#pragma unroll
-            for (int e = 0; e < 4; ++e)
-              if (cq * 4 + e < c) v[e] = src[e];
-          }
-        }
-        d[a][b] = v;
-      }
-    f4 r[4][4];
-#pragma unroll
-    for (int b = 0; b < 4; ++b) {
-      r[0][b] = d[0][b] - d[2][b];
-      r[1][b] = d[1][b] + d[2][b];
-      r[2][b] = d[2][b] - d[1][b];
-      r[3][b] = d[1][b] - d[3][b];
-    }
-#pragma unroll
-    for (int a = 0; a < 4; ++a) {
-      const f4 v[4] = {r[a][0] - r[a][2], r[a][1] + r[a][2], r[a][2] - r[a][1], r[a][1] - r[a][3]};
-#pragma unroll
-      for (int b = 0; b < 4; ++b) *reinterpret_cast<f4*>(V + ((size_t)(a * 4 + b) * T + t) * Cp + cq * 4) = v[b];
-    }
+    wino_load_window<VEC>(x, d, img, 2 * ti - pad_t, 2 * tj - pad_l, h, w, c, ld, cq);
+    wino_input_store(d, V, T, t, Cp, cq);
+  }
+}
+
+__device__ __forceinline__ void wino_output_rows(const float* __restrict__ M, f4 (&r)[2][4], size_t T, size_t t, int Np, int cq) {
+  f4 m[4][4];
+#pragma unroll
+  for (int a = 0; a < 4; ++a)
+#pragma unroll
+    for (int b = 0; b < 4; ++b) m[a][b] = *reinterpret_cast<const f4*>(M + ((size_t)(a * 4 + b) * T + t) * Np + cq * 4);
+#pragma unroll
+  for (int b = 0; b < 4; ++b) {
+    r[0][b] = (m[0][b] + m[1][b]) + m[2][b];
+    r[1][b] = (m[1][b] - m[2][b]) - m[3][b];
   }
 }
 
@@ -98,17 +121,8 @@
     const size_t t = i / cqn;
     const int tj = (int)(t % tw), ti = (int)((t / tw) % th);
     const size_t img = t / ((size_t)tw * th);
-    f4 m[4][4];
-#pragma unroll
-    for (int a = 0; a < 4; ++a)
-#pragma unroll
-      for (int b = 0; b < 4; ++b) m[a][b] = *reinterpret_cast<const f4*>(M + ((size_t)(a * 4 + b) * T + t) * Np + cq * 4);
     f4 r[2][4];
-#pragma unroll
-    for (int b = 0; b < 4; ++b) {
-      r[0][b] = (m[0][b] + m[1][b]) + m[2][b];
-      r[1][b] = (m[1][b] - m[2][b]) - m[3][b];
-    }
+    wino_output_rows(M, r, T, t, Np, cq);
     f4 bv = f4(0.f);
     if (bias) {
 #pragma unroll
@@ -221,6 +235,14 @@
   return timing_record(mode, A3D_PREC_F32, kBM, kBN, kWavesM, kNWaves, kBK, 4, 4, 0, (int)(16 * g.T), g.N, g.K);
 }
 
+static void wino_gemm_tiles(IgemmParams& p) {
+  p.splitk = 1;
+  p.ktiles_per_split = (p.K + kBK - 1) / kBK;
+  p.tiles_m = (p.M + kBM - 1) / kBM;
+  p.tiles_n = (p.N + kBN - 1) / kBN;
+  p.slab = (size_t)p.M * p.N;
+}
+
 int wino_gemm(IgemmParams& p, const WinoGeom& g, hipStream_t st) {
   using Cfg = IgemmCfg<MODE_FWD, kBM, kBN, kWavesM, kNWaves, kBK, 4, 4>;
   static bool attr_done[64] = {};
@@ -232,17 +254,25 @@
     if (e != hipSuccess) return set_error(A3D_ELAUNCH, "hipFuncSetAttribute: %s", hipGetErrorString(e));
     if (dev >= 0 && dev < 64) attr_done[dev] = true;
   }
-  p.splitk = 1;
-  p.ktiles_per_split = (p.K + kBK - 1) / kBK;
-  p.tiles_m = (p.M + kBM - 1) / kBM;
-  p.tiles_n = (p.N + kBN - 1) / kBN;
-  p.slab = (size_t)p.M * p.N;
+  wino_gemm_tiles(p);
   clear_stale_error();
   hipLaunchKernelGGL(wino_gemm_kernel, dim3((unsigned)(p.tiles_m * p.tiles_n), 16), dim3(Cfg::NT), Cfg::LDS_BYTES, st, p,
                      g.T * (size_t)g.Kp, (size_t)g.Kp * g.Np, g.T * (size_t)g.Np);
   return check_launch("wino_gemm");
 }
 
+
+
+__device__ __forceinline__ void wino_dz_store(const f4 (&y)[2][2], float* __restrict__ Z, size_t T, size_t t, int Kp, int cq) {
+  const f4 r[4][2] = {{y[0][0], y[0][1]}, {y[0][0] + y[1][0], y[0][1] + y[1][1]}, {y[0][0] - y[1][0], y[0][1] - y[1][1]},
+                      {-y[1][0], -y[1][1]}};
+#pragma unroll
+  for (int a = 0; a < 4; ++a) {
+    const f4 z[4] = {r[a][0], r[a][0] + r[a][1], r[a][0] - r[a][1], -r[a][1]};
+#pragma unroll
+    for (int b = 0; b < 4; ++b) *reinterpret_cast<f4*>(Z + ((size_t)(a * 4 + b) * T + t) * Kp + cq * 4) = z[b];
+  }
+}
 
 template <bool VEC>
 __global__ __launch_bounds__(256) void wino_dz_kernel(const float* __restrict__ dz, float* __restrict__ Z, int ho, int wo, int k, int ld,
@@ -273,54 +303,52 @@
         }
         y[a][b] = v;
       }
-    const f4 r[4][2] = {{y[0][0], y[0][1]}, {y[0][0] + y[1][0], y[0][1] + y[1][1]}, {y[0][0] - y[1][0], y[0][1] - y[1][1]},
-                        {-y[1][0], -y[1][1]}};
-#pragma unroll
-    for (int a = 0; a < 4; ++a) {
-      const f4 z[4] = {r[a][0], r[a][0] + r[a][1], r[a][0] - r[a][1], -r[a][1]};
-#pragma unroll
-      for (int b = 0; b < 4; ++b) *reinterpret_cast<f4*>(Z + ((size_t)(a * 4 + b) * T + t) * Kp + cq * 4) = z[b];
-    }
+    wino_dz_store(y, Z, T, t, Kp, cq);
+  }
+}
+
+__device__ __forceinline__ void wino_dw_item(size_t i, const float* __restrict__ slabs, const float* __restrict__ bparts, float* __restrict__ dw,
+                                             float* __restrict__ db, int c, int k, int Cp, int Kp, int splits) {
+  const size_t plane = (size_t)Cp * Kp;
+  const int col = (int)(i % k), row = (int)(i / k);
+  const size_t at = (size_t)row * Kp + col;
+  float m[4][4];
+#pragma unroll
+  for (int xi = 0; xi < 16; ++xi) m[xi / 4][xi % 4] = slabs[(size_t)xi * splits * plane + at];
+  for (int z = 1; z < splits; ++z) {
+    float v[16];
+#pragma unroll
+    for (int xi = 0; xi < 16; ++xi) v[xi] = slabs[((size_t)xi * splits + z) * plane + at];
+#pragma unroll
+    for (int xi = 0; xi < 16; ++xi) m[xi / 4][xi % 4] += v[xi];
+  }
+  float t[3][4];
+#pragma unroll
+  for (int b = 0; b < 4; ++b) {
+    const float hs = (m[1][b] + m[2][b]) * 0.5f;
+    t[0][b] = m[0][b] + hs;
+    t[1][b] = (m[1][b] - m[2][b]) * 0.5f;
+    t[2][b] = hs + m[3][b];
+  }
+#pragma unroll
+  for (int a = 0; a < 3; ++a) {
+    const float hs = (t[a][1] + t[a][2]) * 0.5f;
+    const float g[3] = {t[a][0] + hs, (t[a][1] - t[a][2]) * 0.5f, hs + t[a][3]};
+#pragma unroll
+    for (int b = 0; b < 3; ++b) dw[((size_t)(a * 3 + b) * c + row) * k + col] = g[b];
+  }
+  if (db && row == 0) {
+    float s = bparts[col];
+    for (int z = 1; z < splits; ++z) s += bparts[(size_t)z * Kp + col];
+    db[col] = s;
   }
 }
 
 __global__ __launch_bounds__(256) void wino_dw_kernel(const float* __restrict__ slabs, const float* __restrict__ bparts, float* __restrict__ dw,
                                                       float* __restrict__ db, int c, int k, int Cp, int Kp, int splits) {
-  const size_t total = (size_t)c * k, plane = (size_t)Cp * Kp;
-  for (size_t i = (size_t)blockIdx.x * 256 + threadIdx.x; i < total; i += (size_t)gridDim.x * 256) {
-    const int col = (int)(i % k), row = (int)(i / k);
-    const size_t at = (size_t)row * Kp + col;
-    float m[4][4];
-#pragma unroll
-    for (int xi = 0; xi < 16; ++xi) m[xi / 4][xi % 4] = slabs[(size_t)xi * splits * plane + at];
-    for (int z = 1; z < splits; ++z) {
-      float v[16];
-#pragma unroll
-      for (int xi = 0; xi < 16; ++xi) v[xi] = slabs[((size_t)xi * splits + z) * plane + at];
-#pragma unroll
-      for (int xi = 0; xi < 16; ++xi) m[xi / 4][xi % 4] += v[xi];
-    }
-    float t[3][4];
-#pragma unroll
-    for (int b = 0; b < 4; ++b) {
-      const float hs = (m[1][b] + m[2][b]) * 0.5f;
-      t[0][b] = m[0][b] + hs;
-      t[1][b] = (m[1][b] - m[2][b]) * 0.5f;
-      t[2][b] = hs + m[3][b];
-    }
-#pragma unroll
-    for (int a = 0; a < 3; ++a) {
-      const float hs = (t[a][1] + t[a][2]) * 0.5f;
-      const float g[3] = {t[a][0] + hs, (t[a][1] - t[a][2]) * 0.5f, hs + t[a][3]};
-#pragma unroll
-      for (int b = 0; b < 3; ++b) dw[((size_t)(a * 3 + b) * c + row) * k + col] = g[b];
-    }
-    if (db && row == 0) {
-      float s = bparts[col];
-      for (int z = 1; z < splits; ++z) s += bparts[(size_t)z * Kp + col];
-      db[col] = s;
-    }
-  }
+  const size_t total = (size_t)c * k;
+  for (size_t i = (size_t)blockIdx.x * 256 + threadIdx.x; i < total; i += (size_t)gridDim.x * 256)
+    wino_dw_item(i, slabs, bparts, dw, db, c, k, Cp, Kp, splits);
 }
 
 constexpr int kBiasPlane = 1 * 4 + 1;
@@ -393,6 +421,15 @@
   return r;
 }
 
+static void wino_grad_gemm_tiles(IgemmParams& p, const WinoGradGeom& g) {
+  const int nk = (p.K + kBK - 1) / kBK;
+  p.splitk = g.splits;
+  p.ktiles_per_split = (nk + g.splits - 1) / g.splits;
+  p.tiles_m = (p.M + kBM - 1) / kBM;
+  p.tiles_n = (p.N + kBN - 1) / kBN;
+  p.slab = (size_t)p.M * p.N;
+}
+
 int wino_grad_gemm(IgemmParams& p, const WinoGradGeom& g, hipStream_t st) {
   using Cfg = IgemmCfg<MODE_BWD_F, kBM, kBN, kWavesM, kNWaves, kBK, 4, 4>;
   static bool attr_done[64] = {};
@@ -404,16 +441,244 @@
     if (e != hipSuccess) return set_error(A3D_ELAUNCH, "hipFuncSetAttribute: %s", hipGetErrorString(e));
     if (dev >= 0 && dev < 64) attr_done[dev] = true;
   }
-  const int nk = (p.K + kBK - 1) / kBK;
-  p.splitk = g.splits;
-  p.ktiles_per_split = (nk + g.splits - 1) / g.splits;
-  p.tiles_m = (p.M + kBM - 1) / kBM;
-  p.tiles_n = (p.N + kBN - 1) / kBN;
-  p.slab = (size_t)p.M * p.N;
+  wino_grad_gemm_tiles(p, g);
   clear_stale_error();
   hipLaunchKernelGGL(wino_grad_gemm_kernel, dim3((unsigned)(p.tiles_m * p.tiles_n * p.splitk), 16), dim3(Cfg::NT), Cfg::LDS_BYTES, st, p,
                      g.T * (size_t)g.Cp, g.T * (size_t)g.Kp, (size_t)g.splits * g.Cp * g.Kp);
   return check_launch("wino_grad_gemm");
 }
 
-}
+
+struct WinoBwdXform {
+  const float *x, *dz;
+  float *Vx, *Vdz, *Z;
+  int h, w, c, ldx, xth, xtw, xpt, xpl, Cp;
+  int ho, wo, k, ldy, dth, dtw, dpt, dpl, Kp;
+  size_t Tx, Td, x_items;
+};
+template <bool VEC>
+__global__ __launch_bounds__(256) void wino_bwd_transform_kernel(const WinoBwdXform q) {
+  const int cqx = q.Cp / 4, cqd = q.Kp / 4;
+  const size_t total = q.x_items + q.Td * (size_t)cqd;
+  for (size_t i = (size_t)blockIdx.x * 256 + threadIdx.x; i < total; i += (size_t)gridDim.x * 256) {
+    f4 d[4][4];
+    if (i < q.x_items) {
+      const int cq = (int)(i % cqx);
+      const size_t t = i / cqx;
+      const int tj = (int)(t % q.xtw), ti = (int)((t / q.xtw) % q.xth);
+      const size_t img = t / ((size_t)q.xtw * q.xth);
+      wino_load_window<VEC>(q.x, d, img, 2 * ti - q.xpt, 2 * tj - q.xpl, q.h, q.w, q.c, q.ldx, cq);
+      wino_input_store(d, q.Vx, q.Tx, t, q.Cp, cq);
+      continue;
+    }
+    const size_t j = i - q.x_items;
+    const int cq = (int)(j % cqd);
+    const size_t t = j / cqd;
+    const int tj = (int)(t % q.dtw), ti = (int)((t / q.dtw) % q.dth);
+    const size_t img = t / ((size_t)q.dtw * q.dth);
+    wino_load_window<VEC>(q.dz, d, img, 2 * ti - q.dpt, 2 * tj - q.dpl, q.ho, q.wo, q.k, q.ldy, cq);
+    wino_input_store(d, q.Vdz, q.Td, t, q.Kp, cq);
+    if (ti < q.xth && tj < q.xtw) {
+      f4 y[2][2];
+#pragma unroll
+      for (int a = 0; a < 2; ++a)
+#pragma unroll
+        for (int b = 0; b < 2; ++b) {
+          const f4 lo = q.dpl == 1 ? d[1 + a][1 + b] : d[1 + a][2 + b], hi = q.dpl == 1 ? d[2 + a][1 + b] : d[2 + a][2 + b];
+          y[a][b] = q.dpt == 1 ? lo : hi;
+        }
+      wino_dz_store(y, q.Z, q.Tx, (img * q.xth + ti) * q.xtw + tj, q.Kp, cq);
+    }
+  }
+}
+
+int wino_bwd_transforms(const a3d_conv_desc* d, const float* x, const float* dz, float* Vx, float* Vdz, float* Z, hipStream_t st) {
+  const WinoGeom gx = wino_geom(d, false), gd = wino_geom(d, true);
+  WinoBwdXform q{};
+  q.x = x; q.dz = dz; q.Vx = Vx; q.Vdz = Vdz; q.Z = Z;
+  q.h = d->h; q.w = d->w; q.c = d->c; q.ldx = d->ldx; q.xth = gx.th; q.xtw = gx.tw; q.xpt = d->pad_t; q.xpl = d->pad_l; q.Cp = gx.Kp;
+  q.ho = d->ho; q.wo = d->wo; q.k = d->k; q.ldy = d->ldy; q.dth = gd.th; q.dtw = gd.tw; q.dpt = 2 - d->pad_t; q.dpl = 2 - d->pad_l;
+  q.Kp = gd.Kp;
+  q.Tx = gx.T; q.Td = gd.T; q.x_items = gx.T * (size_t)(gx.Kp / 4);
+  const bool vec = d->c % 4 == 0 && d->ldx % 4 == 0 && aligned16(x) && d->k % 4 == 0 && d->ldy % 4 == 0 && aligned16(dz);
+  const dim3 grid(grid_for(q.x_items + gd.T * (size_t)(gd.Kp / 4), 256, 1u << 20)), block(256);
+  clear_stale_error();
+  if (vec) hipLaunchKernelGGL(wino_bwd_transform_kernel<true>, grid, block, 0, st, q);
+  else hipLaunchKernelGGL(wino_bwd_transform_kernel<false>, grid, block, 0, st, q);
+  return check_launch("wino_bwd_transform");
+}
+
+struct WinoBatch {
+  size_t a, b, c;
+};
+__global__ __launch_bounds__(64 * kNWaves, 2 * kNWaves / 4) void wino_bwd_gemm_kernel(const IgemmParams pf, const WinoBatch bf, const uint32_t gf,
+                                                                                       const IgemmParams pd, const WinoBatch bd, const uint32_t gd) {
+  if (blockIdx.x < 16 * gf) {
+    const uint32_t xi = blockIdx.x / gf;
+    IgemmParams q = pf;
+    q.A = pf.A + (size_t)xi * bf.a;
+    q.B = pf.B + (size_t)xi * bf.b;
+    q.C = pf.C + (size_t)xi * bf.c;
+    if (xi != kBiasPlane) q.dbias = nullptr;
+    igemm_body<MODE_BWD_F, kBM, kBN, kWavesM, kNWaves, kBK, 4, 4>(q, gf, blockIdx.x - xi * gf);
+  } else {
+    const uint32_t id = blockIdx.x - 16 * gf, xi = id / gd;
+    IgemmParams q = pd;
+    q.A = pd.A + (size_t)xi * bd.a;
+    q.B = pd.B + (size_t)xi * bd.b;
+    q.C = pd.C + (size_t)xi * bd.c;
+    igemm_body<MODE_FWD, kBM, kBN, kWavesM, kNWaves, kBK, 4, 4>(q, gd, id - xi * gd);
+  }
+}
+
+int wino_bwd_gemm(IgemmParams& pf, const WinoGradGeom& gg, IgemmParams& pd, const WinoGeom& g, hipStream_t st) {
+  constexpr size_t kLds = std::max(IgemmCfg<MODE_BWD_F, kBM, kBN, kWavesM, kNWaves, kBK, 4, 4>::LDS_BYTES,
+                                   IgemmCfg<MODE_FWD, kBM, kBN, kWavesM, kNWaves, kBK, 4, 4>::LDS_BYTES);
+  static bool attr_done[64] = {};
+  int dev = 0;
+  (void)hipGetDevice(&dev);
+  if (dev < 0 || dev >= 64 || !attr_done[dev]) {
+    hipError_t e = hipFuncSetAttribute(reinterpret_cast<const void*>(wino_bwd_gemm_kernel), hipFuncAttributeMaxDynamicSharedMemorySize, (int)kLds);
+    if (e != hipSuccess) return set_error(A3D_ELAUNCH, "hipFuncSetAttribute: %s", hipGetErrorString(e));
+    if (dev >= 0 && dev < 64) attr_done[dev] = true;
+  }
+  wino_grad_gemm_tiles(pf, gg);
+  wino_gemm_tiles(pd);
+  const uint32_t gf = (uint32_t)(pf.tiles_m * pf.tiles_n * pf.splitk), gd = (uint32_t)(pd.tiles_m * pd.tiles_n);
+  const WinoBatch bf{gg.T * (size_t)gg.Cp, gg.T * (size_t)gg.Kp, (size_t)gg.splits * gg.Cp * gg.Kp};
+  const WinoBatch bd{g.T * (size_t)g.Kp, (size_t)g.Kp * g.Np, g.T * (size_t)g.Np};
+  clear_stale_error();
+  hipLaunchKernelGGL(wino_bwd_gemm_kernel, dim3(16 * (gf + gd)), dim3(64 * kNWaves), kLds, st, pf, bf, gf, pd, bd, gd);
+  return check_launch("wino_bwd_gemm");
+}
+
+struct WinoBwdFinish {
+  const float *slabs, *bparts;
+  float *dw, *db;
+  int c, k, Cp, Kp, splits;
+  const float* M;
+  float* dx;
+  const float* mask;
+  int oh, ow, ncols, ld, th, tw, Np;
+  size_t T, dw_items;
+  const uint8_t* argmax;
+  const float* py;
+  int pldy, h2, w2;
+};
+template <bool VEC, bool POOL>
+__global__ __launch_bounds__(256) void wino_bwd_finish_kernel(const WinoBwdFinish q) {
+  const int cqn = q.Np / 4;
+  const size_t total = q.dw_items + q.T * (size_t)cqn;
+  for (size_t i = (size_t)blockIdx.x * 256 + threadIdx.x; i < total; i += (size_t)gridDim.x * 256) {
+    if (i < q.dw_items) {
+      wino_dw_item(i, q.slabs, q.bparts, q.dw, q.db, q.c, q.k, q.Cp, q.Kp, q.splits);
+      continue;
+    }
+    const size_t j = i - q.dw_items;
+    const int cq = (int)(j % cqn);
+    const size_t t = j / cqn;
+    const int tj = (int)(t % q.tw), ti = (int)((t / q.tw) % q.th);
+    const size_t img = t / ((size_t)q.tw * q.th);
+    f4 r[2][4];
+    wino_output_rows(q.M, r, q.T, t, q.Np, cq);
+#pragma unroll
+    for (int a = 0; a < 2; ++a) {
+      const f4 y2[2] = {(r[a][0] + r[a][1]) + r[a][2], (r[a][1] - r[a][2]) - r[a][3]};
+#pragma unroll
+      for (int b = 0; b < 2; ++b) {
+        const int oy = 2 * ti + a, ox = 2 * tj + b;
+        if (oy >= q.oh || ox >= q.ow) continue;
+        const f4 v = y2[b] + f4(0.f);
+        const size_t win = (img * q.oh + oy) * q.ow + ox;
+        if (!POOL) {
+          const size_t o = win * (size_t)q.ld + cq * 4;
+          if (VEC) {
+            f4 u = v;
+            if (q.mask) {
+              const f4 y = *reinterpret_cast<const f4*>(q.mask + o);
+#pragma unroll
+              for (int e = 0; e < 4; ++e) u[e] = apply_act_grad(v[e], y[e], EPI_RELU, 1.f);
+            }
+            *reinterpret_cast<f4*>(q.dx + o) = u;
+          } else {
+#pragma unroll
+            for (int e = 0; e < 4; ++e)
+              if (cq * 4 + e < q.ncols) q.dx[o + e] = q.mask ? apply_act_grad(v[e], q.mask[o + e], EPI_RELU, 1.f) : v[e];
+          }
+          continue;
+        }
+        const size_t px = (size_t)q.ncols, row = (size_t)q.w2 * px;
+        const size_t base = ((img * q.h2 + 2 * oy) * q.w2 + 2 * ox) * px + cq * 4;
+        const bool cut_r = oy == q.oh - 1 && (q.h2 & 1), cut_c = ox == q.ow - 1 && (q.w2 & 1);
+        if (VEC) {
+          const uint32_t a4 = *reinterpret_cast<const uint32_t*>(q.argmax + win * px + cq * 4);
+          const f4 y4 = *reinterpret_cast<const f4*>(q.py + win * (size_t)q.pldy + cq * 4);
+          const f4 zero = f4(0.f);
+          f4 o[4] = {zero, zero, zero, zero};
+#pragma unroll
+          for (int e = 0; e < 4; ++e) {
+            const uint32_t arg = (a4 >> (8 * e)) & 0xffu;
+            const float g = !(y4[e] > 0.f) ? 0.f : v[e];
+#pragma unroll
+            for (int kk = 0; kk < 4; ++kk) o[kk][e] = arg == (uint32_t)kk ? g : 0.f;
+          }
+          *reinterpret_cast<f4*>(q.dx + base) = o[0];
+          *reinterpret_cast<f4*>(q.dx + base + px) = o[1];
+          *reinterpret_cast<f4*>(q.dx + base + row) = o[2];
+          *reinterpret_cast<f4*>(q.dx + base + row + px) = o[3];
+          if (cut_c) {
+            *reinterpret_cast<f4*>(q.dx + base + 2 * px) = zero;
+            *reinterpret_cast<f4*>(q.dx + base + row + 2 * px) = zero;
+          }
+          if (cut_r) {
+            *reinterpret_cast<f4*>(q.dx + base + 2 * row) = zero;
+            *reinterpret_cast<f4*>(q.dx + base + 2 * row + px) = zero;
+            if (cut_c) *reinterpret_cast<f4*>(q.dx + base + 2 * row + 2 * px) = zero;
+          }
+        } else {
+#pragma unroll
+          for (int e = 0; e < 4; ++e) {
+            if (cq * 4 + e >= q.ncols) continue;
+            const int arg = q.argmax[win * px + cq * 4 + e];
+            const float g = !(q.py[win * (size_t)q.pldy + cq * 4 + e] > 0.f) ? 0.f : v[e];
+            float* dst = q.dx + base + e;
+            dst[0] = arg == 0 ? g : 0.f;
+            dst[px] = arg == 1 ? g : 0.f;
+            dst[row] = arg == 2 ? g : 0.f;
+            dst[row + px] = arg == 3 ? g : 0.f;
+            if (cut_c) dst[2 * px] = dst[row + 2 * px] = 0.f;
+            if (cut_r) {
+              dst[2 * row] = dst[2 * row + px] = 0.f;
+              if (cut_c) dst[2 * row + 2 * px] = 0.f;
+            }
+          }
+        }
+      }
+    }
+  }
+}
+
+int wino_bwd_finish(const a3d_conv_desc* d, const WinoGradGeom& gg, const float* slabs, const float* bparts, float* dw, float* db,
+                    const float* M, float* dx, const float* mask, const WinoBwdPool* pool, hipStream_t st) {
+  const WinoGeom g = wino_geom(d, true);
+  WinoBwdFinish q{};
+  q.slabs = slabs; q.bparts = bparts; q.dw = dw; q.db = db; q.c = d->c; q.k = d->k; q.Cp = gg.Cp; q.Kp = gg.Kp; q.splits = gg.splits;
+  q.M = M; q.dx = dx; q.mask = mask; q.oh = g.oh; q.ow = g.ow; q.ncols = g.N; q.ld = d->ldx; q.th = g.th; q.tw = g.tw; q.Np = g.Np;
+  q.T = g.T; q.dw_items = (size_t)d->c * d->k;
+  bool vec = g.N % 4 == 0 && aligned16(dx);
+  if (pool) {
+    q.argmax = pool->argmax; q.py = pool->y; q.pldy = pool->ldy; q.h2 = pool->h2; q.w2 = pool->w2;
+    vec = vec && pool->ldy % 4 == 0 && aligned16(pool->y) && (reinterpret_cast<uintptr_t>(pool->argmax) & 3) == 0;
+  } else {
+    vec = vec && d->ldx % 4 == 0 && aligned16(mask);
+  }
+  const dim3 grid(grid_for(q.dw_items + g.T * (size_t)(g.Np / 4), 256, 1u << 20)), block(256);
+  clear_stale_error();
+  if (pool && vec) hipLaunchKernelGGL((wino_bwd_finish_kernel<true, true>), grid, block, 0, st, q);
+  else if (pool) hipLaunchKernelGGL((wino_bwd_finish_kernel<false, true>), grid, block, 0, st, q);
+  else if (vec) hipLaunchKernelGGL((wino_bwd_finish_kernel<true, false>), grid, block, 0, st, q);
+  else hipLaunchKernelGGL((wino_bwd_finish_kernel<false, false>), grid, block, 0, st, q);
+  return check_launch("wino_bwd_finish");
+}
+
+}
diff --git a/ann3depth_amd/models.py b/ann3depth_amd/models.py
--- a/ann3depth_amd/models.py
+++ b/ann3depth_amd/models.py
@@ -322,6 +322,7 @@
     WINO_MIN_TILES = 504
     WINO_GRAD_LAYERS = WINO_LAYERS
     WINO_GRAD_MIN_TILES = 504
+    WINO_BWD_CHAIN = True
 
     def _desc(self, name, which):
         d = self.d[name]
@@ -756,6 +757,13 @@
             d, w = self._prepared((name, 'bwd_d', 'fp32w'), self.d_wino[name], w, 'bwd_d')
         ops.conv2d_bwd_data(d, dz, w, dx, relu_mask=relu_mask)
 
+    def _wino_chain(self, name):
+        return self.WINO_BWD_CHAIN and name in self.d_wino and name in self.wino_grad
+
+    def _bwd_wino(self, name, x, dz, dx, relu_mask=None, pool=None):
+        d, w = self._prepared((name, 'bwd_d', 'fp32w'), self.d_wino[name], self._w(name, 'bwd_d'), 'bwd_d')
+        ops.conv2d_bwd_wino(d, x, dz, w, self._g(name + '/kernel'), self._g(name + '/bias'), dx, relu_mask=relu_mask, pool=pool)
+
     def _bwd_filter(self, name, x, dz):
         if name in self.d:
             call = ops.conv2d_bwd_filter_wino if name in self.wino_grad else ops.conv2d_bwd_filter
@@ -806,19 +814,29 @@
         self._bwd_data(n, self.dc4, self.dc3, relu_mask=self.c3)
         self._join()
         dw = self._bwd_filter
+        pooled = self.pooled_fwd == 1 or self.bf16s
         n = 'coarse/conv/conv2d_3'
-        dw(n, self.c2, self.dc3)
-        self._bwd_data(n, self.dc3, self.dc2, relu_mask=self.c2)
+        if self._wino_chain(n):
+            self._bwd_wino(n, self.c2, self.dc3, self.dc2, relu_mask=self.c2)
+        else:
+            dw(n, self.c2, self.dc3)
+            self._bwd_data(n, self.dc3, self.dc2, relu_mask=self.c2)
         n = 'coarse/conv/conv2d_2'
-        dw(n, self.p1, self.dc2)
-        if after_conv2 is not None:
-            after_conv2()
-        self._bwd_data(n, self.dc2, self.dp1)
-        pooled = self.pooled_fwd == 1 or self.bf16s
-        if pooled:
-            ops.maxpool2x2_bwd_idx(self.a1, self.p1, self.dp1, self.dc1, relu_mask=True)
-        else:
-            ops.maxpool2x2_bwd(self.c1, self.dp1, self.dc1, relu_mask=True)
+        if self._wino_chain(n):
+            self._bwd_wino(n, self.p1, self.dc2, self.dc1 if pooled else self.dp1, pool=(self.a1, self.p1) if pooled else None)
+            if after_conv2 is not None:
+                after_conv2()
+            if not pooled:
+                ops.maxpool2x2_bwd(self.c1, self.dp1, self.dc1, relu_mask=True)
+        else:
+            dw(n, self.p1, self.dc2)
+            if after_conv2 is not None:
+                after_conv2()
+            self._bwd_data(n, self.dc2, self.dp1)
+            if pooled:
+                ops.maxpool2x2_bwd_idx(self.a1, self.p1, self.dp1, self.dc1, relu_mask=True)
+            else:
+                ops.maxpool2x2_bwd(self.c1, self.dp1, self.dc1, relu_mask=True)
         n = 'coarse/conv/conv2d_1'
         dw(n, self.p0, self.dc1)
         self._bwd_data(n, self.dc1, self.dp0)
diff --git a/ann3depth_amd/ops.py b/ann3depth_amd/ops.py
--- a/ann3depth_amd/ops.py
+++ b/ann3depth_amd/ops.py
@@ -172,6 +172,19 @@
     check(lib.a3dwg_conv2d_bwd_filter(ctypes.byref(d), _ptr(x), _ptr(dz), _ptr(dw), _ptr(db), ws, n, _stream()),
           'a3dwg_conv2d_bwd_filter')
     return dw, db
+
+
+def conv2d_bwd_wino(d, x, dz, w, dw, db, dx, relu_mask=None, pool=None):
+    lib = _lib.load()
+    prepared = int(bool(d.hints & HINT_W_PREPARED))
+    ws, n = _ws().get(lib.a3dwb_conv2d_bwd_ws_bytes(ctypes.byref(d), prepared, int(pool is not None)), x.device)
+    pp = None
+    if pool is not None:
+        argmax, y = pool
+        pp = ctypes.byref(_lib.WinoBwdPool(_ptr(argmax), _ptr(y), y.shape[-1], dx.shape[1], dx.shape[2]))
+    check(lib.a3dwb_conv2d_bwd(ctypes.byref(d), _ptr(x), _ptr(dz), _ptr(w), _ptr(dw), _ptr(db), _ptr(dx), _ptr(relu_mask), pp,
+                               ws, n, _stream()), 'a3dwb_conv2d_bwd')
+    return dw, db, dx
 
 
 def conv2d_bwd_filter_pooled_supported(d):
diff --git a/include/a3d_wino_bwd.h b/include/a3d_wino_bwd.h
--- /dev/null
+++ b/include/a3d_wino_bwd.h
@@ -0,0 +1,26 @@
+#ifndef A3D_WINO_BWD_H_
+#define A3D_WINO_BWD_H_
+
+#include "a3d.h"
+
+#ifdef __cplusplus
+extern "C" {
+#endif
+
+typedef struct a3dwb_pool {
+  const uint8_t* argmax;
+  const float* y;
+  int ldy;
+  int h2, w2;
+} a3dwb_pool;
+
+size_t a3dwb_sizeof_pool(void);
+
+size_t a3dwb_conv2d_bwd_ws_bytes(const a3d_conv_desc* d, int w_prepared, int pooled);
+int a3dwb_conv2d_bwd(const a3d_conv_desc* d, const float* x, const float* dz, const float* w_or_U, float* dw, float* db, float* dx,
+                     const float* relu_mask, const a3dwb_pool* pool, void* ws, size_t ws_bytes, void* stream);
+
+#ifdef __cplusplus
+}
+#endif
+#endif
```
